# thangvubk/SoftGroup

Hardware: AMD Instinct MI355X
Metric: scans/sec ScanNet-v2-like inference (softgroup_scannet.yaml, full forward_test) (higher is better)
Workload: dtype f32

## Files before the change

### include/softgroup_hip.h

```cpp
#ifndef SOFTGROUP_HIP_H
#define SOFTGROUP_HIP_H

#include <stddef.h>
#include <stdint.h>

#ifdef __cplusplus
extern "C" {
#endif

typedef void *sg_stream_t;

#define SG_OK 0
#define SG_ERR_ARG (-1)
#define SG_ERR_WORKSPACE (-2)
#define SG_ERR_LAUNCH (-3)
#define SG_ERR_UNSUPPORTED (-4)

#define SG_BALLQUERY_MAX_NEIGHBORS 1000
#define SG_OCTREE_NUM_NODES 585
#define SG_OCTREE_NUM_LEAVES 512
#define SG_LISTS_SORTED 1
#define SG_LISTS_RADIUS 2

int sg_version(void);
const char *sg_last_error(void);
int sg_device_info(char *name_host, int name_cap, int *num_cu_host, int *clock_khz_host);

int sg_stream_release(sg_stream_t stream);
int sg_stream_create(sg_stream_t *stream_out);
int sg_stream_destroy(sg_stream_t stream);
int sg_stream_create_priority(sg_stream_t *stream_out, int level);

int sg_voxelize_idx_host(const int64_t *coords_host, int n, int ncol, int mode,
                         int32_t *input_map_host, int32_t *num_voxels_host,
                         int32_t *max_active_host);
int sg_voxelize_idx_fill_host(const int64_t *coords_host, int n, int ncol, int mode,
                              const int32_t *input_map_host, int num_voxels, int max_active,
                              int64_t *out_coords_host, int32_t *out_map_host);
size_t sg_voxelize_idx_workspace_bytes(int n);
int sg_voxelize_idx_build(const int64_t *coords, int n, int ncol, int mode, int32_t *input_map,
                          int32_t *meta, void *ws, size_t ws_bytes, sg_stream_t stream);
int sg_voxelize_idx_fill(const int64_t *coords, int n, int ncol, int mode,
                         const int32_t *input_map, int num_voxels, int max_active,
                         int64_t *out_coords, int32_t *out_map, void *ws, size_t ws_bytes,
                         sg_stream_t stream);

int sg_voxelize_fp(const float *feats, const int32_t *rules, int num_voxels, int max_active,
                   int channels, int average, float *out, sg_stream_t stream);
int sg_voxelize_bp(const float *d_out, const int32_t *rules, int num_voxels, int max_active,
                   int channels, int average, float *d_feats, sg_stream_t stream);

size_t sg_ballquery_workspace_bytes(int n);
int sg_ballquery_build_grid(const float *xyz, const int32_t *batch_idxs, int n, float radius,
                            void *ws, size_t ws_bytes, sg_stream_t stream);
int sg_ballquery_count(const float *xyz, const int32_t *batch_idxs, int n, float radius,
                       int32_t *start_len, int32_t *meta, void *ws, size_t ws_bytes,
                       sg_stream_t stream);
int sg_ballquery_fill(const float *xyz, const int32_t *batch_idxs, int n, float radius,
                      const int32_t *start_len, int32_t *idx, void *ws, size_t ws_bytes,
                      sg_stream_t stream);
size_t sg_scan_workspace_bytes(int n);
int sg_exclusive_scan_startlen(int32_t *start_len, int n, int32_t *meta, void *ws,
                               size_t ws_bytes, sg_stream_t stream);

int sg_octree_build_host(const float *points_host, const float *xyzwhl_host, int num_points,
                         int num_levels, float *boxes_host, int32_t *pt_inds_host,
                         int32_t *pt_start_len_host);
size_t sg_octree_build_workspace_bytes(int n);
int sg_octree_build(const float *points, int n, float *boxes, int32_t *pt_inds, int32_t *pt_start_len,
                    void *ws, size_t ws_bytes, sg_stream_t stream);
size_t sg_pyramid_inverse_map_workspace_bytes(int n_points, int n_voxels, int n_prop);
int sg_pyramid_inverse_map(const int32_t *proposals_idx, int64_t num_pairs, int n_prop,
                           const int32_t *l2p_map, int n_points, int n_voxels, int32_t *out_idx,
                           int32_t *out_offsets, int32_t *n_out_dev, void *ws, size_t ws_bytes,
                           sg_stream_t stream);
int sg_octree_ballquery_count(const float *points, const float *boxes, const int32_t *pt_inds,
                              const int32_t *pt_start_len, int n, float radius,
                              int32_t *start_len, sg_stream_t stream);
int sg_octree_ballquery_fill(const float *points, const float *boxes, const int32_t *pt_inds,
                             const int32_t *pt_start_len, int n, float radius,
                             const int32_t *start_len, int32_t *idx, sg_stream_t stream);

size_t sg_bfs_workspace_bytes(int n, int64_t n_edges);
int sg_bfs_cluster_label(const int32_t *bq_idxs, const int32_t *start_len, int n,
                         int64_t n_edges, int list_flags, const int32_t *seg_of_point,
                         const float *seg_thr, int n_seg, int32_t *n_cluster_host,
                         int32_t *sum_npoint_host, void *ws, size_t ws_bytes, sg_stream_t stream);
int sg_bfs_cluster_emit(const int32_t *bq_idxs, const int32_t *start_len, int n, int64_t n_edges,
                        const int32_t *seg_of_point, const float *seg_thr, int n_cluster,
                        int sum_npoint, int32_t *cluster_idxs, int32_t *cluster_offsets, void *ws,
                        size_t ws_bytes, sg_stream_t stream);

int sg_sec_mean(const float *inp, const int32_t *offsets, int n_seg, int channels, float *out,
                sg_stream_t stream);
int sg_sec_min(const float *inp, const int32_t *offsets, int n_seg, int channels, float *out,
               sg_stream_t stream);
int sg_sec_max(const float *inp, const int32_t *offsets, int n_seg, int channels, float *out,
               sg_stream_t stream);
int sg_global_avg_pool_fp(const float *feats, const int32_t *offsets, int n_seg, int channels,
                          float *out, sg_stream_t stream);
int sg_global_avg_pool_bp(float *d_feats, const int32_t *offsets, const float *d_out, int n_seg,
                          int channels, sg_stream_t stream);

int sg_get_mask_iou_on_cluster(const int32_t *proposals_idx, const int32_t *proposals_offset,
                               const int64_t *instance_labels, const int32_t *instance_pointnum,
                               int n_instance, int n_proposal, float *proposals_iou,
                               sg_stream_t stream);
int sg_get_mask_iou_on_pred(const int32_t *proposals_idx, const int32_t *proposals_offset,
                            const int64_t *instance_labels, const int32_t *instance_pointnum,
                            const float *mask_scores_sigmoid, int n_instance, int n_proposal,
                            float *proposals_iou, sg_stream_t stream);
int sg_get_mask_label(const int32_t *proposals_idx, const int32_t *proposals_offset,
                      const int64_t *instance_labels, const int64_t *instance_cls,
                      const float *proposals_iou, int n_instance, int n_proposal, float iou_thr,
                      float *mask_label, sg_stream_t stream);

size_t sg_spconv_hash_workspace_bytes(int num_rows);
int sg_spconv_subm_rulebook(const int32_t *indices, int num_rows, const int32_t *spatial_shape_host,
                            int32_t *nbr, void *ws, size_t ws_bytes, sg_stream_t stream);
int sg_spconv_down_build(const int32_t *indices, int num_rows, const int32_t *spatial_shape_host,
                         int32_t *in2out, int32_t *meta, void *ws, size_t ws_bytes,
                         sg_stream_t stream);
int sg_spconv_down_fill(const int32_t *indices, int num_rows, const int32_t *in2out,
                        int num_out_rows, int32_t *out_indices, int32_t *child, void *ws,
                        size_t ws_bytes, sg_stream_t stream);
int sg_spconv_inverse_rulebook(const int32_t *indices_fine, const int32_t *in2out, int num_rows,
                               int32_t *inv_nbr, sg_stream_t stream);

#define SG_PLAN_HIST_WORDS 40
size_t sg_spconv_plan_workspace_bytes(int num_out_rows);
int sg_spconv_plan(const int32_t *nbr, int num_out_rows, int kvol, int32_t *order,
                   uint32_t *tile_mask, int32_t *nbr_tiles, void *ws, size_t ws_bytes,
                   sg_stream_t stream);

#define SG_PYRAMID_MAX_LEVELS 10
typedef struct sg_plan_ptrs {
  int32_t *order;
  uint32_t *tile_mask;
  int32_t *nbr_tiles;
} sg_plan_ptrs;
typedef struct sg_pyramid_level {
  int rows;
  int32_t *indices;
  int32_t *nbr;
  sg_plan_ptrs subm;
  int32_t *in2out;
  int32_t *child;
  sg_plan_ptrs down;
  int32_t *inv;
  sg_plan_ptrs up;
} sg_pyramid_level;
size_t sg_spconv_pyramid_workspace_bytes(int num_rows, int n_levels);
int sg_spconv_pyramid_rows(const int32_t *indices, int num_rows, const int32_t *spatial_shape_host,
                           int n_levels, int32_t *rows_dev, void *ws, size_t ws_bytes,
                           sg_stream_t stream);
size_t sg_spconv_pyramid_build_workspace_bytes(const sg_pyramid_level *levels_host, int n_levels);
int sg_spconv_pyramid_build(const int32_t *indices, int num_rows, const int32_t *spatial_shape_host,
                            int n_levels, const sg_pyramid_level *levels_host, void *ws,
                            size_t ws_bytes, void *ws2, size_t ws2_bytes, sg_stream_t stream);

size_t sg_spconv_packed_weight_elems(int kvol, int cin, int cout);
int sg_spconv_pack_weight(const float *w, int cout, int kvol, int cin, int src_is_kio, float *w_k8,
                          sg_stream_t stream);

size_t sg_spconv_conv_workspace_bytes(int num_out_rows, int cout);
int sg_spconv_gather_conv_f32(const float *in, int num_in_rows, const int32_t *nbr,
                              int num_out_rows, int kvol, int cin, int cout, const float *w_k8,
                              const float *post_scale, const float *post_shift,
                              const float *residual, const float *act_scale,
                              const float *act_shift, float *out_act, const int32_t *order,
                              const uint32_t *tile_mask, const int32_t *nbr_tiles, float *out,
                              void *ws, size_t ws_bytes, sg_stream_t stream);

int sg_spconv_set_arithmetic(int mode);

int sg_spconv_set_combine(int mode);

int sg_spconv_set_chain(int mode);
int sg_spconv_chain_stats(int64_t *launches, int64_t *steps);

int sg_spconv_profile(int enable);
int sg_spconv_profile_read(double *total_ms, int *launches);
int sg_spconv_profile_detail(float *ms, int32_t *dims, int cap, int *calls);

typedef struct sg_mlp2 {
  const float *w1, *b1, *bn_scale, *bn_shift, *w2, *b2;
  int out;
} sg_mlp2;
int sg_pointwise_heads(const float *voxel_feats, const void *v2p_map, int v2p_is_int64, int n_points,
                       int channels, const sg_mlp2 *semantic, const sg_mlp2 *offset, float *output_feats,
                       float *semantic_scores, float *pt_offsets, int64_t *semantic_preds,
                       sg_stream_t stream);

size_t sg_spconv_packed_weight_elems_bf16(int kvol, int cin, int cout);
int sg_spconv_pack_weight_bf16(const float *w, int cout, int kvol, int cin, int src_is_kio,
                               uint16_t *w_k8_bf16, sg_stream_t stream);
size_t sg_spconv_conv_bf16_workspace_bytes(int num_out_rows, int cout);
int sg_spconv_gather_conv_bf16(const uint16_t *in, int num_in_rows, const int32_t *nbr, int num_out_rows,
                               int kvol, int cin, int cout, const uint16_t *w_k8_bf16,
                               const int32_t *order, const uint32_t *tile_mask, const int32_t *nbr_tiles,
                               uint16_t *out, void *ws, size_t ws_bytes, sg_stream_t stream);

int sg_spconv_transpose_table(const int32_t *nbr, int num_out_rows, int kvol, int32_t *nbr_t,
                              sg_stream_t stream);
size_t sg_spconv_wgrad_workspace_bytes(int num_out_rows, int kvol, int cin, int cout);
int sg_spconv_wgrad(const void *in, int in_is_bf16, const void *g_out, int g_is_bf16, const int32_t *nbr_t,
                    int num_out_rows, int kvol, int cin, int cout, float *dw_kio, void *ws,
                    size_t ws_bytes, sg_stream_t stream);

typedef struct sg_unet_block {
  int cin, cout;
  const float *bn1_scale, *bn1_shift;
  const float *w1;
  const float *bn2_scale, *bn2_shift;
  const float *w2;
  const float *w_i;
} sg_unet_block;
typedef struct sg_unet_level {
  int planes, n_blocks;
  const sg_unet_block *blocks;
  const sg_unet_block *tail;
  const float *down_bn_scale, *down_bn_shift, *down_w;
  const float *up_bn_scale, *up_bn_shift, *up_w;
} sg_unet_level;
typedef struct sg_unet_desc {
  int n_levels;
  const sg_unet_level *levels;
  int input_cin;
  const float *input_w;
  const float *out_bn_scale, *out_bn_shift;
  int input_cin_packed;
  int arithmetic;
} sg_unet_desc;
size_t sg_unet_arena_bytes(const sg_unet_desc *desc, int num_rows);
int sg_unet_forward(const sg_unet_desc *desc, const float *feats, const int32_t *indices,
                    int num_rows, const int32_t *spatial_shape_host, float *out, void *arena,
                    size_t arena_bytes, sg_stream_t stream);

typedef struct sg_train_bn {
  const float *weight, *bias;
  float *running_mean, *running_var;
  float momentum, eps;
  float *g_weight, *g_bias;
} sg_train_bn;
typedef struct sg_train_conv {
  const float *w;
  float *g_w;
} sg_train_conv;
typedef struct sg_unet_train_block {
  int cin, cout;
  sg_train_bn bn1, bn2;
  sg_train_conv c1, c2, ci;
} sg_unet_train_block;
typedef struct sg_unet_train_level {
  int planes, n_blocks;
  const sg_unet_train_block *blocks, *tail;
  sg_train_bn down_bn, up_bn;
  sg_train_conv down, up;
} sg_unet_train_level;
typedef struct sg_unet_train_desc {
  int n_levels;
  const sg_unet_train_level *levels;
  int input_cin;
  sg_train_conv input;
  sg_train_bn out_bn;
  int arithmetic;
} sg_unet_train_desc;
size_t sg_unet_train_arena_hint(const sg_unet_train_desc *desc, int num_rows);
int sg_unet_train_forward(const sg_unet_train_desc *desc, const float *feats, const int32_t *indices,
                          int num_rows, const int32_t *spatial_shape_host, float *out, void *arena,
                          size_t arena_bytes, size_t *arena_needed, void **tape, sg_stream_t stream);
int sg_unet_train_backward(void *tape, const float *g_out, float *g_feats, sg_stream_t stream);
void sg_unet_train_release(void *tape);

int sg_bn_relu_f32(const float *x, const float *scale, const float *shift, int64_t num_rows,
                   int channels, int relu, float *out, sg_stream_t stream);

int sg_gather_rows_f32(const float *in, const int32_t *index, int64_t num_out_rows, int channels,
                       float *out, sg_stream_t stream);
int sg_gather_rows_i64idx_f32(const float *in, const int64_t *index, int64_t num_out_rows,
                              int channels, float *out, sg_stream_t stream);

int sg_instance_npoint(const int32_t *proposals_idx, const float *mask_scores, int64_t num_pairs,
                       int stride, int n_classes, float mask_thr, int n_prop, int32_t *npoint,
                       sg_stream_t stream);
size_t sg_instance_runs_workspace_bytes(int n_kept, int n_points);
int sg_instance_runs(const int32_t *proposals_idx, const float *mask_scores, int64_t num_pairs,
                     int stride, int n_classes, float mask_thr, const int32_t *inst_of, int n_prop,
                     int n_kept, int n_points, int32_t *starts, int32_t *ends, int64_t *bounds,
                     int64_t runs_capacity, void *ws, size_t ws_bytes, sg_stream_t stream);

int64_t sg_rle_format_bound(int64_t total_runs, int digits);
int sg_rle_format_host(const int64_t *starts_host, const int64_t *lens_host,
                       const int64_t *bounds_host, int n_groups, char *out_host,
                       int64_t out_capacity, int64_t *out_offsets_host);
size_t sg_rle_format_device_workspace_bytes(int64_t run_capacity);
int64_t sg_rle_format_device_text_bytes(int64_t run_capacity, int64_t length);
int sg_rle_format_device(const int32_t *starts, const int32_t *ends, const int64_t *bounds, int n_inst,
                         int64_t run_capacity, int64_t length, uint8_t *text, int64_t text_capacity,
                         int64_t *text_off, void *ws, size_t ws_bytes, sg_stream_t stream);
int sg_rle_format_runs_host(const int32_t *starts_host, const int32_t *ends_host,
                            const int64_t *bounds_host, int n_groups, char *out_host,
                            int64_t out_capacity, int64_t *out_offsets_host);

size_t sg_panoptic_fusion_workspace_bytes(int n_inst, int n_points);
int sg_panoptic_fusion(const uint32_t *bits, int n_inst, int n_points, const int32_t *order,
                       const int32_t *label_id, const int64_t *semantic_preds, int cls_offset,
                       double skip_iou, int semantic_classes, int thing_class_min, uint32_t *out,
                       void *ws, size_t ws_bytes, sg_stream_t stream);

#define SG_NMS_IOU 0
#define SG_NMS_MIN 1
size_t sg_mask_nms_workspace_bytes(int n_inst, int64_t n_points);
int sg_mask_nms(const uint32_t *bits, int n_inst, int64_t n_points, const float *scores, const int32_t *labels,
                double thr, int measure, int class_agnostic, uint8_t *keep, int32_t *n_keep, int32_t *inter_out,
                void *ws, size_t ws_bytes, sg_stream_t stream);
int sg_mask_bits_from_runs(const int32_t *starts, const int32_t *ends, const int64_t *bounds, int64_t n_runs,
                           int n_inst, int64_t n_points, uint32_t *bits, sg_stream_t stream);

typedef struct sg_grouping_cfg {
  int n_points;
  int n_sem_classes;
  int n_seg;
  const int32_t *seg_class;
  const float *seg_thr;
  float score_thr;
  int min_npoint;
  float radius;
  int batch_size;
  float voxel_scale;
  int voxel_shape;
  int feat_channels;
} sg_grouping_cfg;
typedef struct sg_grouping_result {
  int n_selected, n_neighbours, n_proposals, sum_npoint, n_voxels, max_active;
  size_t proposals_idx;
  size_t proposals_offset;
  size_t voxel_coords;
  size_t voxel_offsets;
  size_t voxel_feats;
  size_t point_to_voxel;
  size_t arena_used, arena_needed;
  int deferred_classes;
  int reserved_;
} sg_grouping_result;
int sg_scan_grouping(const sg_grouping_cfg *cfg, const float *scores, const float *pt_offsets,
                     const float *coords_float, const int32_t *batch_idxs, const float *point_feats,
                     void *arena, size_t arena_bytes, sg_grouping_result *result_host,
                     sg_stream_t stream);

typedef struct sg_grouping_pp_cfg {
  sg_grouping_cfg base;
  int with_pyramid, with_octree, lvl_fusion;
  double radius;
  double base_size;
} sg_grouping_pp_cfg;
int sg_scan_grouping_pp(const sg_grouping_pp_cfg *cfg, const float *scores, const float *pt_offsets,
                        const float *coords_float, const int32_t *batch_idxs, const float *point_feats,
                        void *arena, size_t arena_bytes, sg_grouping_result *result_host,
                        sg_stream_t stream);

int sg_host_copy_2d(void *dst, int64_t dst_pitch_bytes, const void *src, int64_t src_pitch_bytes, int64_t rows,
                    int64_t row_bytes);
int sg_host_cast_f64_f32(float *dst, const double *src, int64_t n);
int sg_host_fill_i64_strided(int64_t *dst, int64_t pitch_elems, int64_t rows, int64_t value);
int sg_host_colmax_i64(const int64_t *src, int64_t rows, int64_t cols, int64_t *out_max);

typedef struct sg_instances_cfg {
  int n_proposals, n_classes;
  int score_stride;
  int64_t sum_npoint;
  int n_points;
  float cls_score_thr, mask_score_thr;
  int min_npoint;
} sg_instances_cfg;
typedef struct sg_instances_result {
  int n_kept;
  size_t off_class, off_score, off_text, text_bytes;
  size_t host_needed, arena_used, arena_needed;
  size_t bits;
  size_t label_id;
} sg_instances_result;
int sg_scan_instances(const sg_instances_cfg *cfg, const int32_t *proposals_idx, const float *mask_scores,
                      const float *cls_prob, const float *iou_scores, void *arena, size_t arena_bytes,
                      void *host_out, size_t host_bytes, sg_instances_result *result_host,
                      sg_stream_t stream);

typedef struct sg_linear {
  const float *w, *b;
  int out, in;
} sg_linear;
int sg_softmax_rows(const float *x, int64_t rows, int cols, float *out, sg_stream_t stream);
int sg_mlp_rows(const float *feats, const int32_t *idx, int64_t rows, int channels, const sg_mlp2 *mlp,
                float *out, sg_stream_t stream);
int sg_linear_rows(const float *x, int64_t rows, const sg_linear *lin, float *out, sg_stream_t stream);

#define SG_SCAN_DENSE_MAX 16
typedef struct sg_scan_dense_item {
  int kind;
  const void *ptr;
  size_t bytes;
} sg_scan_dense_item;
typedef struct sg_scan_desc {
  const sg_unet_desc *backbone;
  const sg_unet_desc *tiny;
  sg_mlp2 semantic, offset, mask;
  sg_linear cls, iou;
  int channels;
  int with_coords;
  int semantic_classes, instance_classes;
  sg_grouping_cfg grouping;
  float cls_score_thr, mask_score_thr;
  int min_npoint;
  int want_instances;
  int with_pyramid, with_octree;
  double pp_radius, pp_base_size;
} sg_scan_desc;
typedef struct sg_scan_input {
  int n_points, n_voxels, max_active;
  int batch_size;
  int spatial_shape[3];
  const float *feats;
  int feat_dim;
  const float *coords_float;
  const int32_t *p2v_map;
  const void *v2p_map;
  int v2p_is_int64;
  const void *voxel_coords;
  int voxel_coords_is_int64;
  const int32_t *batch_idxs;
  const int64_t *semantic_labels, *instance_labels;
  int n_dense;
  sg_scan_dense_item dense[SG_SCAN_DENSE_MAX];
} sg_scan_input;
typedef struct sg_scan_result {
  sg_grouping_result grouping;
  sg_instances_result instances;
  size_t grouping_base, instances_base;
  size_t dense_offset[SG_SCAN_DENSE_MAX];
  size_t dense_bytes;
  size_t voxel_feats_in, backbone_out, output_feats, semantic_scores, semantic_prob, pt_offsets,
      semantic_preds, tiny_out, mask_scores, cls_scores, cls_prob, iou_scores;
  size_t arena_used, arena_needed, host_dense_needed, host_inst_needed;
  int stage;
} sg_scan_result;
size_t sg_scan_arena_bytes(const sg_scan_desc *desc, int n_points, int n_voxels);
int sg_scan_forward(const sg_scan_desc *desc, const sg_scan_input *in, void *arena, size_t arena_bytes,
                    void *host_dense, size_t host_dense_bytes, void *host_inst, size_t host_inst_bytes,
                    sg_scan_result *result_host, sg_stream_t stream);

int sg_eval_intersections(const int32_t *run_start, const int64_t *run_off, const int32_t *run_pred,
                          int n_runs, int64_t total_points, const int32_t *gt_slot, int n_pred,
                          int n_slots, int32_t *counts, sg_stream_t stream);

#define SG_EVAL_I32 0
#define SG_EVAL_I64 1
#define SG_EVAL_U32 2
#define SG_EVAL_MAX_CLASSES 1024
#define SG_EVAL_BAD_GT 1
#define SG_EVAL_BAD_PRED 2
#define SG_EVAL_BAD_INST 4

size_t sg_eval_tally_workspace_bytes(int64_t n_points);
int sg_eval_class_tally(const void *pred, int pred_kind, const void *gt, int gt_kind, int64_t n_points,
                        int64_t ignore_label, int panoptic, int n_classes, uint64_t *tallies,
                        const void *inst, int inst_kind, const float *offset_pred, const float *offset_gt,
                        double *offset_sum, uint64_t *offset_count, int32_t *flags, void *ws, size_t ws_bytes,
                        sg_stream_t stream);

size_t sg_eval_panoptic_workspace_bytes(int64_t n_points);
int sg_eval_panoptic_segments(const void *pred, int pred_kind, const void *sem, int sem_kind,
                              const void *inst, int inst_kind, const int64_t *scan_off, int n_scans,
                              int64_t n_points, int64_t ignore_label, int n_classes, int64_t min_points,
                              uint64_t *fp_fn, int64_t *tp_rows, uint64_t *tp_count, int32_t *flags,
                              void *ws, size_t ws_bytes, sg_stream_t stream);

#define SG_INST_BAD_TEXT 1
#define SG_INST_ODD_TOKENS 2
#define SG_INST_RUN_RANGE 4
#define SG_INST_BAD_GT 8
#define SG_INST_OVERFLOW_GT 16
#define SG_INST_OVERFLOW_EX 32
#define SG_INST_NO_EXAMPLES 64
#define SG_INST_MAX_THRESHOLDS 16
#define SG_INST_SECTIONS 16

int64_t sg_inst_rle_run_slots(int64_t text_bytes, int n_masks);
int sg_inst_rle_parse(const uint8_t *text, const int64_t *text_off, const int32_t *mask_pred, int n_masks,
                      int64_t text_bytes, int64_t length, int32_t *run_start, int32_t *run_len, int32_t *run_pred,
                      int64_t run_slots, int32_t *vert_count, int32_t *flags, sg_stream_t stream);

size_t sg_inst_scan_workspace_bytes(int64_t n_points, int n_pred, int64_t run_slots, int n_classes, int gt_cap,
                                    int n_thr, int n_labels, int64_t *section_off);
int sg_inst_scan_update(const int64_t *gts, int64_t n_points, const int32_t *run_start, const int32_t *run_len,
                        const int32_t *run_pred, int64_t run_slots, const int32_t *pred_label,
                        const int32_t *pred_vert, const double *pred_conf, int n_pred, int n_labels, int n_classes,
                        int64_t min_region, const double *thresholds, int n_thr, int gt_cap, uint64_t *ex_key,
                        uint32_t *ex_meta, int64_t ex_cap, int32_t *seg_stats, int64_t *totals, int32_t *flags,
                        void *ws, size_t ws_bytes, sg_stream_t stream);

size_t sg_inst_curves_workspace_bytes(int64_t n_examples, int n_seg);
int sg_inst_curves(const uint64_t *ex_key, const uint32_t *ex_meta, int64_t n_examples, const int32_t *seg_stats,
                   int n_seg, double *ap, double *rc, int32_t *flags, void *ws, size_t ws_bytes,
                   sg_stream_t stream);

#define SG_DET_BAD_COORD 1
#define SG_DET_MAX_THRESHOLDS 16

int sg_det_boxes_runs(const void *coords, int coords_f64, const int64_t *run_start, const int64_t *run_off,
                      const int32_t *run_owner, int64_t n_runs, int64_t total_points, int64_t n_owner,
                      double *boxes, int32_t *flags, sg_stream_t stream);

int sg_det_boxes_labels(const void *coords, int coords_f64, const int64_t *labels, const int64_t *scan_off,
                        const int64_t *owner_off, int n_scans, int64_t n_points, int64_t n_owner, double *boxes,
                        int64_t *count, int64_t *first, int32_t *flags, sg_stream_t stream);

size_t sg_det_match_workspace_bytes(int64_t n_gt, int n_thresholds);
int sg_det_match(const double *det_box, const int32_t *det_group, const int32_t *det_rank, int64_t n_det,
                 const double *gt_box, const int64_t *group_off, int64_t n_gt, const double *thresholds,
                 int n_thresholds, double *ovmax, int64_t *jmax, uint8_t *tp, void *ws, size_t ws_bytes,
                 sg_stream_t stream);

int sg_train_augment(const float *xyz, int64_t n, int has_scale, float scale_factor, const double *m_host,
                     double work_scale, double down, double *xyz_middle, double *work, uint64_t *stats,
                     sg_stream_t stream);
int sg_train_blur(float *grids, float *tmp, int b0, int b1, int b2, int n_grids, sg_stream_t stream);
int sg_train_elastic(double *work, int64_t n, const float *grids, int b0, int b1, int b2, double gran, double mag,
                     uint64_t *stats, sg_stream_t stream);
int sg_train_crop_count(const double *work, int64_t n, double down, const double *min_host,
                        const double *cand_host, int k, uint64_t *counts, sg_stream_t stream);
size_t sg_train_compact_workspace_bytes(int64_t n);
int sg_train_compact(const double *work, const double *xyz_middle, const float *feat, int c, const float *noise,
                     const int64_t *sem, const int64_t *inst, int64_t n, double down, const double *min_host,
                     const double *crop_host, int64_t out_cap, int64_t *coord, double *xyz_middle_out,
                     float *feat_out, int64_t *sem_out, int64_t *inst_out, int32_t *kept, void *ws,
                     size_t ws_bytes, sg_stream_t stream);
int sg_train_gather(const int64_t *idx, int64_t m, const float *xyz, const float *feat, int c, const int64_t *sem,
                    const int64_t *inst, float *xyz_out, float *feat_out, int64_t *sem_out, int64_t *inst_out,
                    sg_stream_t stream);
size_t sg_train_id_set_workspace_bytes(void);
int sg_train_id_set(const int64_t *labels, int64_t n, int64_t ignore, int64_t *out, int cap, void *ws,
                    size_t ws_bytes, sg_stream_t stream);
int sg_train_remap(int64_t *labels, int64_t n, const int64_t *sorted_ids, const int64_t *mapped, int k,
                   sg_stream_t stream);
size_t sg_train_instance_workspace_bytes(int64_t n, int k);
int sg_train_instance_info(const double *xyz_middle, const int64_t *inst, const int64_t *sem, int64_t n, int k,
                           int64_t cls_shift, int32_t *pointnum, int64_t *cls, double *pt_offset, void *ws,
                           size_t ws_bytes, sg_stream_t stream);

int sg_test_x4_minima(const float *xyz, int64_t n, const double *m_host, double scale, uint64_t *stats,
                      sg_stream_t stream);
int sg_test_x4_split(const float *xyz, const float *feat, int c, const int64_t *sem, const int64_t *inst, int64_t n,
                     const double *m_host, double scale, const double *min_host, int64_t *coord,
                     double *xyz_middle, float *feat_out, int64_t *sem_out, int64_t *inst_out, sg_stream_t stream);
int sg_kitti_decode_labels(const int32_t *words, int64_t n, const int32_t *lut, int64_t *sem, int64_t *inst,
                           uint64_t *missing, sg_stream_t stream);

int sg_mask_text_runs(const int32_t *starts, const int32_t *ends, const int64_t *bounds, int64_t n_runs, int n_inst,
                      int64_t length, int first, int count, uint8_t *text, int64_t text_capacity, sg_stream_t stream);
int sg_mask_text_bits(const uint32_t *bits, int n_inst, int64_t length, int first, int count, uint8_t *text,
                      int64_t text_capacity, sg_stream_t stream);
size_t sg_decimal_lines_workspace_bytes(int64_t n);
int sg_decimal_lines(const int64_t *values, int64_t n, const int32_t *nyu_table, int nyu_len, uint8_t *text,
                     int64_t text_capacity, int64_t *meta, void *ws, size_t ws_bytes, sg_stream_t stream);
int sg_panoptic_kitti_words(const uint32_t *words, int64_t n, const int32_t *lut, int lut_len, uint32_t *out,
                            uint64_t *missing, uint64_t *missing_host, sg_stream_t stream);
size_t sg_parse_decimal_lines_workspace_bytes(int64_t nbytes);
int sg_parse_decimal_lines(const uint8_t *text, int64_t nbytes, int64_t *values, int64_t capacity, int64_t *meta,
                           void *ws, size_t ws_bytes, sg_stream_t stream);
int sg_parse_mask_text(const uint8_t *text, int64_t nbytes, uint8_t *flags, uint32_t *bits, int64_t *meta,
                       sg_stream_t stream);

int sg_viz_paint_bits(const uint32_t *bits, int n_inst, int64_t n, const int32_t *priority, const uint8_t *skip,
                      int32_t *label, int32_t *pointnum, sg_stream_t stream);
size_t sg_viz_paint_runs_workspace_bytes(int n_inst, int64_t n);
int sg_viz_paint_runs(const int32_t *starts, const int32_t *ends, const int64_t *bounds, int64_t n_runs, int n_inst,
                      int64_t n, const int32_t *priority, const uint8_t *skip, int32_t *label, int32_t *pointnum,
                      void *ws, size_t ws_bytes, sg_stream_t stream);
int sg_viz_gt_labels(const int64_t *ids, int64_t n, int32_t *label, int32_t *pointnum, sg_stream_t stream);
size_t sg_viz_instance_rank_workspace_bytes(int n_inst);
int sg_viz_instance_rank(const int32_t *pointnum, int n_inst, int32_t *rank, void *ws, size_t ws_bytes,
                         sg_stream_t stream);
#define SG_VIZ_INPUT 0
#define SG_VIZ_CLASS 1
#define SG_VIZ_CLASS_WRAP 2
#define SG_VIZ_INSTANCE 3
int sg_viz_colors(int mode, const float *colors, const int64_t *cls, const int32_t *inst, const int32_t *rank,
                  int n_rank, const uint8_t *table, int k, int64_t n, uint8_t *rgb, int64_t *meta,
                  sg_stream_t stream);
size_t sg_viz_ply_vertices_workspace_bytes(int64_t n);
int sg_viz_ply_vertices(const float *xyz, const float *offset, const uint8_t *rgb, const uint8_t *keep, int64_t n,
                        uint8_t *text, int64_t text_capacity, int64_t *meta, void *ws, size_t ws_bytes,
                        sg_stream_t stream);

size_t sg_loss_reduce_workspace_bytes(void);
int sg_pointwise_loss_fwd(const float *semantic_scores, const int64_t *semantic_labels, const float *weight,
                          int64_t ignore_label, const float *pt_offsets, const float *pt_offset_labels,
                          const int64_t *instance_labels, int64_t n, int c, float *out, void *ws, size_t ws_bytes,
                          sg_stream_t stream);
int sg_pointwise_loss_bwd(const float *semantic_scores, const int64_t *semantic_labels, const float *weight,
                          int64_t ignore_label, const float *pt_offsets, const float *pt_offset_labels,
                          const int64_t *instance_labels, int64_t n, int c, const float *sums,
                          const float *g_semantic, const float *g_offset, float *d_scores, float *d_offsets,
                          sg_stream_t stream);
size_t sg_assign_proposals_workspace_bytes(int n_proposal);
int sg_assign_proposals(const float *ious_on_cluster, const int64_t *instance_cls, int64_t ignore_label,
                        float pos_iou_thr, int match_low_quality, float min_pos_thr, int64_t background_label,
                        int n_proposal, int n_gt, int64_t *labels, void *ws, size_t ws_bytes, sg_stream_t stream);
int sg_proposal_loss_fwd(const float *cls_scores, const float *iou_scores, const int64_t *labels,
                         const float *ious_on_pred, const int64_t *instance_cls, int64_t ignore_label,
                         int n_proposal, int n_gt, int k1, float *gt_iou, float *out, void *ws, size_t ws_bytes,
                         sg_stream_t stream);
int sg_proposal_loss_bwd(const float *cls_scores, const float *iou_scores, const int64_t *labels,
                         const float *gt_iou, const float *sums, const float *g_cls, const float *g_iou,
                         int n_proposal, int k1, float *d_cls_scores, float *d_iou_scores, sg_stream_t stream);
int sg_mask_loss_fwd(const float *mask_scores, const int32_t *instance_batch_idxs, const int64_t *labels,
                     const float *mask_label, int64_t m, int n_proposal, int k1, float *mask_sig, float *out,
                     void *ws, size_t ws_bytes, sg_stream_t stream);
int sg_mask_loss_bwd(const float *mask_scores, const int32_t *instance_batch_idxs, const int64_t *labels,
                     const float *mask_label, const float *sums, const float *g_mask, int64_t m, int n_proposal,
                     int k1, float *d_mask_scores, sg_stream_t stream);

#define SG_OPTIM_ROW_PARAM 0
#define SG_OPTIM_ROW_GRAD 1
#define SG_OPTIM_ROW_STATE0 2
#define SG_OPTIM_ROW_STATE1 3
#define SG_OPTIM_ROW_STEP 4
#define SG_OPTIM_ROW_COUNT 5
#define SG_OPTIM_TABLE_ROWS 6
int sg_optim_chunk_elems(void);
int64_t sg_optim_plan(const int64_t *counts, int n_tensors, int64_t *chunks, int64_t chunk_capacity);
size_t sg_optim_workspace_bytes(void);
int sg_optim_grad_norm(const int64_t *table, int n_tensors, const int64_t *chunks, int64_t n_chunks,
                       const float *grad_scale, float max_norm, float *out, void *ws, size_t ws_bytes,
                       sg_stream_t stream);
int sg_optim_adam_step(const int64_t *table, int n_tensors, const int64_t *chunks, int64_t n_chunks, double lr,
                       double beta1, double beta2, double eps, double weight_decay, int adamw,
                       const float *grad_scale, const float *found_inf, const float *clip_coef, int zero_grad,
                       int32_t *arrive, sg_stream_t stream);
int sg_optim_sgd_step(const int64_t *table, int n_tensors, const int64_t *chunks, int64_t n_chunks, double lr,
                      double momentum, double dampening, double weight_decay, int nesterov, const float *grad_scale,
                      const float *found_inf, const float *clip_coef, int zero_grad, int32_t *arrive,
                      sg_stream_t stream);
int sg_optim_scale_grads(const int64_t *table, int n_tensors, const int64_t *chunks, int64_t n_chunks,
                         const float *coef, sg_stream_t stream);

#ifdef __cplusplus
}
#endif
#endif
```

### softgroup_amd/_lib.py

```python
import ctypes as C
import os

_HERE = os.path.dirname(os.path.abspath(__file__))
LIB_PATH = os.path.join(_HERE, 'lib', os.environ.get('SG_LIB_NAME', 'libsoftgroup_hip.so'))

_lib = None

_vp, _i, _f, _i64, _sz, _d = C.c_void_p, C.c_int, C.c_float, C.c_int64, C.c_size_t, C.c_double
_pi32 = C.POINTER(C.c_int32)

SIGNATURES = {
    'sg_version': (_i, []),
    'sg_last_error': (C.c_char_p, []),
    'sg_device_info': (_i, [C.c_char_p, _i, C.POINTER(_i), C.POINTER(_i)]),
    'sg_stream_release': (_i, [_vp]),
    'sg_host_copy_2d': (_i, [_vp, _i64, _vp, _i64, _i64, _i64]),
    'sg_host_cast_f64_f32': (_i, [_vp, _vp, _i64]),
    'sg_host_fill_i64_strided': (_i, [_vp, _i64, _i64, _i64]),
    'sg_host_colmax_i64': (_i, [_vp, _i64, _i64, _vp]),
    'sg_stream_create': (_i, [_vp]),
    'sg_stream_create_priority': (_i, [_vp, _i]),
    'sg_stream_destroy': (_i, [_vp]),
    'sg_voxelize_idx_host': (_i, [_vp, _i, _i, _i, _vp, _pi32, _pi32]),
    'sg_voxelize_idx_fill_host': (_i, [_vp, _i, _i, _i, _vp, _i, _i, _vp, _vp]),
    'sg_voxelize_idx_workspace_bytes': (_sz, [_i]),
    'sg_voxelize_idx_build': (_i, [_vp, _i, _i, _i, _vp, _vp, _vp, _sz, _vp]),
    'sg_voxelize_idx_fill': (_i, [_vp, _i, _i, _i, _vp, _i, _i, _vp, _vp, _vp, _sz, _vp]),
    'sg_voxelize_fp': (_i, [_vp, _vp, _i, _i, _i, _i, _vp, _vp]),
    'sg_voxelize_bp': (_i, [_vp, _vp, _i, _i, _i, _i, _vp, _vp]),
    'sg_ballquery_workspace_bytes': (_sz, [_i]),
    'sg_ballquery_build_grid': (_i, [_vp, _vp, _i, _f, _vp, _sz, _vp]),
    'sg_ballquery_count': (_i, [_vp, _vp, _i, _f, _vp, _vp, _vp, _sz, _vp]),
    'sg_ballquery_fill': (_i, [_vp, _vp, _i, _f, _vp, _vp, _vp, _sz, _vp]),
    'sg_scan_workspace_bytes': (_sz, [_i]),
    'sg_exclusive_scan_startlen': (_i, [_vp, _i, _vp, _vp, _sz, _vp]),
    'sg_octree_build_host': (_i, [_vp, _vp, _i, _i, _vp, _vp, _vp]),
    'sg_octree_build_workspace_bytes': (_sz, [_i]),
    'sg_octree_build': (_i, [_vp, _i, _vp, _vp, _vp, _vp, _sz, _vp]),
    'sg_pyramid_inverse_map_workspace_bytes': (_sz, [_i, _i, _i]),
    'sg_pyramid_inverse_map': (_i, [_vp, _i64, _i, _vp, _i, _i, _vp, _vp, _vp, _vp, _sz, _vp]),
    'sg_octree_ballquery_count': (_i, [_vp, _vp, _vp, _vp, _i, _f, _vp, _vp]),
    'sg_octree_ballquery_fill': (_i, [_vp, _vp, _vp, _vp, _i, _f, _vp, _vp, _vp]),
    'sg_bfs_workspace_bytes': (_sz, [_i, _i64]),
    'sg_bfs_cluster_label': (_i, [_vp, _vp, _i, _i64, _i, _vp, _vp, _i, _pi32, _pi32, _vp, _sz, _vp]),
    'sg_bfs_cluster_emit': (_i, [_vp, _vp, _i, _i64, _vp, _vp, _i, _i, _vp, _vp, _vp, _sz, _vp]),
    'sg_sec_mean': (_i, [_vp, _vp, _i, _i, _vp, _vp]),
    'sg_sec_min': (_i, [_vp, _vp, _i, _i, _vp, _vp]),
    'sg_sec_max': (_i, [_vp, _vp, _i, _i, _vp, _vp]),
    'sg_global_avg_pool_fp': (_i, [_vp, _vp, _i, _i, _vp, _vp]),
    'sg_global_avg_pool_bp': (_i, [_vp, _vp, _vp, _i, _i, _vp]),
    'sg_get_mask_iou_on_cluster': (_i, [_vp, _vp, _vp, _vp, _i, _i, _vp, _vp]),
    'sg_get_mask_iou_on_pred': (_i, [_vp, _vp, _vp, _vp, _vp, _i, _i, _vp, _vp]),
    'sg_get_mask_label': (_i, [_vp, _vp, _vp, _vp, _vp, _i, _i, _f, _vp, _vp]),
    'sg_spconv_hash_workspace_bytes': (_sz, [_i]),
    'sg_spconv_subm_rulebook': (_i, [_vp, _i, _pi32, _vp, _vp, _sz, _vp]),
    'sg_spconv_pyramid_workspace_bytes': (_sz, [_i, _i]),
    'sg_spconv_pyramid_rows': (_i, [_vp, _i, _pi32, _i, _vp, _vp, _sz, _vp]),
    'sg_spconv_pyramid_build_workspace_bytes': (_sz, [_vp, _i]),
    'sg_spconv_pyramid_build': (_i, [_vp, _i, _pi32, _i, _vp, _vp, _sz, _vp, _sz, _vp]),
    'sg_spconv_down_build': (_i, [_vp, _i, _pi32, _vp, _vp, _vp, _sz, _vp]),
    'sg_spconv_down_fill': (_i, [_vp, _i, _vp, _i, _vp, _vp, _vp, _sz, _vp]),
    'sg_spconv_inverse_rulebook': (_i, [_vp, _vp, _i, _vp, _vp]),
    'sg_spconv_plan_workspace_bytes': (_sz, [_i]),
    'sg_spconv_plan': (_i, [_vp, _i, _i, _vp, _vp, _vp, _vp, _sz, _vp]),
    'sg_spconv_set_arithmetic': (_i, [_i]),
    'sg_spconv_set_combine': (_i, [_i]),
    'sg_spconv_set_chain': (_i, [_i]),
    'sg_spconv_chain_stats': (_i, [_vp, _vp]),
    'sg_spconv_profile': (_i, [_i]),
    'sg_spconv_profile_read': (_i, [_vp, _vp]),
    'sg_spconv_profile_detail': (_i, [_vp, _vp, _i, _vp]),
    'sg_unet_arena_bytes': (_sz, [_vp, _i]),
    'sg_unet_forward': (_i, [_vp, _vp, _vp, _i, _vp, _vp, _vp, _sz, _vp]),
    'sg_unet_train_arena_hint': (_sz, [_vp, _i]),
    'sg_unet_train_forward': (_i, [_vp, _vp, _vp, _i, _vp, _vp, _vp, _sz, _vp, _vp, _vp]),
    'sg_unet_train_backward': (_i, [_vp, _vp, _vp, _vp]),
    'sg_unet_train_release': (None, [_vp]),
    'sg_pointwise_heads': (_i, [_vp, _vp, _i, _i, _i, _vp, _vp, _vp, _vp, _vp, _vp, _vp]),
    'sg_spconv_packed_weight_elems': (_sz, [_i, _i, _i]),
    'sg_spconv_pack_weight': (_i, [_vp, _i, _i, _i, _i, _vp, _vp]),
    'sg_spconv_conv_workspace_bytes': (_sz, [_i, _i]),
    'sg_spconv_gather_conv_f32': (_i, [_vp, _i, _vp, _i, _i, _i, _i, _vp, _vp, _vp, _vp, _vp, _vp,
                                       _vp, _vp, _vp, _vp, _vp, _vp, _sz, _vp]),
    'sg_spconv_packed_weight_elems_bf16': (_sz, [_i, _i, _i]),
    'sg_spconv_pack_weight_bf16': (_i, [_vp, _i, _i, _i, _i, _vp, _vp]),
    'sg_spconv_conv_bf16_workspace_bytes': (_sz, [_i, _i]),
    'sg_spconv_gather_conv_bf16': (_i, [_vp, _i, _vp, _i, _i, _i, _i, _vp, _vp, _vp, _vp, _vp, _vp, _sz,
                                        _vp]),
    'sg_spconv_transpose_table': (_i, [_vp, _i, _i, _vp, _vp]),
    'sg_spconv_wgrad_workspace_bytes': (_sz, [_i, _i, _i, _i]),
    'sg_spconv_wgrad': (_i, [_vp, _i, _vp, _i, _vp, _i, _i, _i, _i, _vp, _vp, _sz, _vp]),
    'sg_instance_npoint': (_i, [_vp, _vp, _i64, _i, _i, _f, _i, _vp, _vp]),
    'sg_instance_runs_workspace_bytes': (_sz, [_i, _i]),
    'sg_instance_runs': (_i, [_vp, _vp, _i64, _i, _i, _f, _vp, _i, _i, _i, _vp, _vp, _vp, _i64, _vp, _sz, _vp]),
    'sg_rle_format_bound': (_i64, [_i64, _i]),
    'sg_rle_format_host': (_i, [_vp, _vp, _vp, _i, _vp, _i64, _vp]),
    'sg_rle_format_device_workspace_bytes': (_sz, [_i64]),
    'sg_rle_format_device_text_bytes': (_i64, [_i64, _i64]),
    'sg_rle_format_device': (_i, [_vp, _vp, _vp, _i, _i64, _i64, _vp, _i64, _vp, _vp, _sz, _vp]),
    'sg_rle_format_runs_host': (_i, [_vp, _vp, _vp, _i, _vp, _i64, _vp]),
    'sg_panoptic_fusion_workspace_bytes': (_sz, [_i, _i]),
    'sg_panoptic_fusion': (_i, [_vp, _i, _i, _vp, _vp, _vp, _i, C.c_double, _i, _i, _vp, _vp, _sz, _vp]),
    'sg_mask_nms_workspace_bytes': (_sz, [_i, _i64]),
    'sg_mask_nms': (_i, [_vp, _i, _i64, _vp, _vp, _d, _i, _i, _vp, _vp, _vp, _vp, _sz, _vp]),
    'sg_mask_bits_from_runs': (_i, [_vp, _vp, _vp, _i64, _i, _i64, _vp, _vp]),
    'sg_scan_grouping': (_i, [_vp, _vp, _vp, _vp, _vp, _vp, _vp, _sz, _vp, _vp]),
    'sg_scan_grouping_pp': (_i, [_vp, _vp, _vp, _vp, _vp, _vp, _vp, _sz, _vp, _vp]),
    'sg_scan_instances': (_i, [_vp, _vp, _vp, _vp, _vp, _vp, _sz, _vp, _sz, _vp, _vp]),
    'sg_softmax_rows': (_i, [_vp, _i64, _i, _vp, _vp]),
    'sg_mlp_rows': (_i, [_vp, _vp, _i64, _i, _vp, _vp, _vp]),
    'sg_linear_rows': (_i, [_vp, _i64, _vp, _vp, _vp]),
    'sg_scan_arena_bytes': (_sz, [_vp, _i, _i]),
    'sg_scan_forward': (_i, [_vp, _vp, _vp, _sz, _vp, _sz, _vp, _sz, _vp, _vp]),
    'sg_eval_intersections': (_i, [_vp, _vp, _vp, _i, _i64, _vp, _i, _i, _vp, _vp]),
    'sg_eval_tally_workspace_bytes': (_sz, [_i64]),
    'sg_eval_class_tally': (_i, [_vp, _i, _vp, _i, _i64, _i64, _i, _i, _vp, _vp, _i, _vp, _vp, _vp, _vp, _vp,
                                 _vp, _sz, _vp]),
    'sg_eval_panoptic_workspace_bytes': (_sz, [_i64]),
    'sg_eval_panoptic_segments': (_i, [_vp, _i, _vp, _i, _vp, _i, _vp, _i, _i64, _i64, _i, _i64, _vp, _vp, _vp,
                                       _vp, _vp, _sz, _vp]),
    'sg_inst_rle_run_slots': (_i64, [_i64, _i]),
    'sg_inst_rle_parse': (_i, [_vp, _vp, _vp, _i, _i64, _i64, _vp, _vp, _vp, _i64, _vp, _vp, _vp]),
    'sg_inst_scan_workspace_bytes': (_sz, [_i64, _i, _i64, _i, _i, _i, _i, _vp]),
    'sg_inst_scan_update': (_i, [_vp, _i64, _vp, _vp, _vp, _i64, _vp, _vp, _vp, _i, _i, _i, _i64, _vp, _i, _i,
                                 _vp, _vp, _i64, _vp, _vp, _vp, _vp, _sz, _vp]),
    'sg_inst_curves_workspace_bytes': (_sz, [_i64, _i]),
    'sg_inst_curves': (_i, [_vp, _vp, _i64, _vp, _i, _vp, _vp, _vp, _vp, _sz, _vp]),
    'sg_det_boxes_runs': (_i, [_vp, _i, _vp, _vp, _vp, _i64, _i64, _i64, _vp, _vp, _vp]),
    'sg_det_boxes_labels': (_i, [_vp, _i, _vp, _vp, _vp, _i, _i64, _i64, _vp, _vp, _vp, _vp, _vp]),
    'sg_det_match_workspace_bytes': (_sz, [_i64, _i]),
    'sg_det_match': (_i, [_vp, _vp, _vp, _i64, _vp, _vp, _i64, _vp, _i, _vp, _vp, _vp, _vp, _sz, _vp]),
    'sg_bn_relu_f32': (_i, [_vp, _vp, _vp, _i64, _i, _i, _vp, _vp]),
    'sg_gather_rows_f32': (_i, [_vp, _vp, _i64, _i, _vp, _vp]),
    'sg_gather_rows_i64idx_f32': (_i, [_vp, _vp, _i64, _i, _vp, _vp]),
    'sg_train_augment': (_i, [_vp, _i64, _i, _f, _vp, C.c_double, C.c_double, _vp, _vp, _vp, _vp]),
    'sg_train_blur': (_i, [_vp, _vp, _i, _i, _i, _i, _vp]),
    'sg_train_elastic': (_i, [_vp, _i64, _vp, _i, _i, _i, C.c_double, C.c_double, _vp, _vp]),
    'sg_train_crop_count': (_i, [_vp, _i64, C.c_double, _vp, _vp, _i, _vp, _vp]),
    'sg_train_compact_workspace_bytes': (_sz, [_i64]),
    'sg_train_compact': (_i, [_vp, _vp, _vp, _i, _vp, _vp, _vp, _i64, C.c_double, _vp, _vp, _i64, _vp, _vp, _vp, _vp,
                              _vp, _vp, _vp, _sz, _vp]),
    'sg_train_gather': (_i, [_vp, _i64, _vp, _vp, _i, _vp, _vp, _vp, _vp, _vp, _vp, _vp]),
    'sg_train_id_set_workspace_bytes': (_sz, []),
    'sg_train_id_set': (_i, [_vp, _i64, _i64, _vp, _i, _vp, _sz, _vp]),
    'sg_train_remap': (_i, [_vp, _i64, _vp, _vp, _i, _vp]),
    'sg_train_instance_workspace_bytes': (_sz, [_i64, _i]),
    'sg_train_instance_info': (_i, [_vp, _vp, _vp, _i64, _i, _i64, _vp, _vp, _vp, _vp, _sz, _vp]),
    'sg_test_x4_minima': (_i, [_vp, _i64, _vp, C.c_double, _vp, _vp]),
    'sg_test_x4_split': (_i, [_vp, _vp, _i, _vp, _vp, _i64, _vp, C.c_double, _vp, _vp, _vp, _vp, _vp, _vp, _vp]),
    'sg_kitti_decode_labels': (_i, [_vp, _i64, _vp, _vp, _vp, _vp, _vp]),
    'sg_mask_text_runs': (_i, [_vp, _vp, _vp, _i64, _i, _i64, _i, _i, _vp, _i64, _vp]),
    'sg_mask_text_bits': (_i, [_vp, _i, _i64, _i, _i, _vp, _i64, _vp]),
    'sg_decimal_lines_workspace_bytes': (_sz, [_i64]),
    'sg_decimal_lines': (_i, [_vp, _i64, _vp, _i, _vp, _i64, _vp, _vp, _sz, _vp]),
    'sg_panoptic_kitti_words': (_i, [_vp, _i64, _vp, _i, _vp, _vp, _vp, _vp]),
    'sg_parse_decimal_lines_workspace_bytes': (_sz, [_i64]),
    'sg_parse_decimal_lines': (_i, [_vp, _i64, _vp, _i64, _vp, _vp, _sz, _vp]),
    'sg_parse_mask_text': (_i, [_vp, _i64, _vp, _vp, _vp, _vp]),
    'sg_viz_paint_bits': (_i, [_vp, _i, _i64, _vp, _vp, _vp, _vp, _vp]),
    'sg_viz_paint_runs_workspace_bytes': (_sz, [_i, _i64]),
    'sg_viz_paint_runs': (_i, [_vp, _vp, _vp, _i64, _i, _i64, _vp, _vp, _vp, _vp, _vp, _sz, _vp]),
    'sg_viz_gt_labels': (_i, [_vp, _i64, _vp, _vp, _vp]),
    'sg_viz_instance_rank_workspace_bytes': (_sz, [_i]),
    'sg_viz_instance_rank': (_i, [_vp, _i, _vp, _vp, _sz, _vp]),
    'sg_viz_colors': (_i, [_i, _vp, _vp, _vp, _vp, _i, _vp, _i, _i64, _vp, _vp, _vp]),
    'sg_viz_ply_vertices_workspace_bytes': (_sz, [_i64]),
    'sg_viz_ply_vertices': (_i, [_vp, _vp, _vp, _vp, _i64, _vp, _i64, _vp, _vp, _sz, _vp]),
    'sg_loss_reduce_workspace_bytes': (_sz, []),
    'sg_pointwise_loss_fwd': (_i, [_vp, _vp, _vp, _i64, _vp, _vp, _vp, _i64, _i, _vp, _vp, _sz, _vp]),
    'sg_pointwise_loss_bwd': (_i, [_vp, _vp, _vp, _i64, _vp, _vp, _vp, _i64, _i, _vp, _vp, _vp, _vp, _vp, _vp]),
    'sg_assign_proposals_workspace_bytes': (_sz, [_i]),
    'sg_assign_proposals': (_i, [_vp, _vp, _i64, _f, _i, _f, _i64, _i, _i, _vp, _vp, _sz, _vp]),
    'sg_proposal_loss_fwd': (_i, [_vp, _vp, _vp, _vp, _vp, _i64, _i, _i, _i, _vp, _vp, _vp, _sz, _vp]),
    'sg_proposal_loss_bwd': (_i, [_vp, _vp, _vp, _vp, _vp, _vp, _vp, _i, _i, _vp, _vp, _vp]),
    'sg_mask_loss_fwd': (_i, [_vp, _vp, _vp, _vp, _i64, _i, _i, _vp, _vp, _vp, _sz, _vp]),
    'sg_mask_loss_bwd': (_i, [_vp, _vp, _vp, _vp, _vp, _vp, _i64, _i, _i, _vp, _vp]),
    'sg_optim_chunk_elems': (_i, []),
    'sg_optim_plan': (_i64, [_vp, _i, _vp, _i64]),
    'sg_optim_workspace_bytes': (_sz, []),
    'sg_optim_grad_norm': (_i, [_vp, _i, _vp, _i64, _vp, _f, _vp, _vp, _sz, _vp]),
    'sg_optim_adam_step': (_i, [_vp, _i, _vp, _i64, _d, _d, _d, _d, _d, _i, _vp, _vp, _vp, _i, _vp, _vp]),
    'sg_optim_sgd_step': (_i, [_vp, _i, _vp, _i64, _d, _d, _d, _d, _i, _vp, _vp, _vp, _i, _vp, _vp]),
    'sg_optim_scale_grads': (_i, [_vp, _i, _vp, _i64, _vp, _vp]),
}


class SoftGroupHipError(RuntimeError):
    pass


def lib():
    global _lib
    if _lib is None:
        import torch
        if not os.path.exists(LIB_PATH):
            raise SoftGroupHipError(
                f'{LIB_PATH} not found: the HIP extension is required (no CPU fallback). '
                'Build it with `python -c "import __graft_entry__ as g; g.build()"`.')
        L = C.CDLL(LIB_PATH)
        for name, (res, args) in SIGNATURES.items():
            fn = getattr(L, name)
            fn.restype = res
            fn.argtypes = args
        _lib = L
    return _lib


def check(rc, what=''):
    if rc != 0:
        msg = lib().sg_last_error()
        raise SoftGroupHipError(f'{what} failed ({rc}): {msg.decode() if msg else ""}')


def ptr(t):
    return None if t is None else t.data_ptr()


_raw_stream = None


def stream():
    global _raw_stream
    import torch
    if _raw_stream is None:
        _raw_stream = getattr(torch._C, '_cuda_getCurrentRawStream', None) or (
            lambda dev: torch.cuda.current_stream(dev).cuda_stream)
    return _raw_stream(torch.cuda.current_device())


def workspace(nbytes, device):
    import torch
    return torch.empty(max(int(nbytes), 256), dtype=torch.uint8, device=device)
```

### softgroup_amd/csrc/ballquery.hip

```cpp
#include "common.h"
#include "scan.h"

namespace sg {

constexpr int32_t kBqEmpty = 0x7f7f7f7f;
constexpr int kBqBuf = 2048;
constexpr int kBqCap = SG_BALLQUERY_MAX_NEIGHBORS;
constexpr int kBqKeep = 64;

struct BqWs {
  int4 *cell;
  int32_t *table;
  int32_t *count;
  int32_t *start;
  int32_t *cursor;
  int32_t *slot_of;
  float4 *sorted;
  int32_t *keep;
  void *scan_ws;
  size_t scan_bytes;
  uint32_t cap;
};

__device__ __forceinline__ uint32_t cell_slot(int b, int cx, int cy, int cz, uint32_t mask) {
  uint64_t h = (static_cast<uint64_t>(static_cast<uint32_t>(b)) << 32) | static_cast<uint32_t>(cx);
  h = mix64(h) ^ ((static_cast<uint64_t>(static_cast<uint32_t>(cy)) << 32) | static_cast<uint32_t>(cz));
  return static_cast<uint32_t>(mix64(h)) & mask;
}

__global__ void __launch_bounds__(256) bq_insert_kernel(const float *__restrict__ xyz,
                                                       const int32_t *__restrict__ batch_idxs,
                                                       int n, double inv_cell, int4 *__restrict__ cell,
                                                       int32_t *table, uint32_t mask, int32_t *count,
                                                       int32_t *__restrict__ slot_of) {
  const int i = blockIdx.x * 256 + threadIdx.x;
  if (i >= n) return;
  int4 c;
  c.x = batch_idxs ? batch_idxs[i] : 0;
  c.y = static_cast<int>(floor(static_cast<double>(xyz[3 * i + 0]) * inv_cell));
  c.z = static_cast<int>(floor(static_cast<double>(xyz[3 * i + 1]) * inv_cell));
  c.w = static_cast<int>(floor(static_cast<double>(xyz[3 * i + 2]) * inv_cell));
  cell[i] = c;
  uint32_t s = cell_slot(c.x, c.y, c.z, c.w, mask);
  while (true) {
    int32_t cur = __hip_atomic_load(&table[s], __ATOMIC_RELAXED, __HIP_MEMORY_SCOPE_AGENT);
    if (cur == kBqEmpty) {
      cur = atomicCAS(&table[s], kBqEmpty, i);
      if (cur == kBqEmpty) break;
    }
    int4 o;
    o.x = batch_idxs ? batch_idxs[cur] : 0;
    o.y = static_cast<int>(floor(static_cast<double>(xyz[3 * cur + 0]) * inv_cell));
    o.z = static_cast<int>(floor(static_cast<double>(xyz[3 * cur + 1]) * inv_cell));
    o.w = static_cast<int>(floor(static_cast<double>(xyz[3 * cur + 2]) * inv_cell));
    if (o.x == c.x && o.y == c.y && o.z == c.z && o.w == c.w) break;
    s = (s + 1) & mask;
  }
  slot_of[i] = static_cast<int32_t>(s);
  atomicAdd(&count[s], 1);
}

__global__ void __launch_bounds__(256) bq_scatter_kernel(const float *__restrict__ xyz, int n,
                                                        const int32_t *__restrict__ slot_of,
                                                        const int32_t *__restrict__ start,
                                                        int32_t *cursor, float4 *__restrict__ sorted) {
  const int i = blockIdx.x * 256 + threadIdx.x;
  if (i >= n) return;
  const int s = slot_of[i];
  const int pos = start[s] + atomicAdd(&cursor[s], 1);
  sorted[pos] = make_float4(xyz[3 * i], xyz[3 * i + 1], xyz[3 * i + 2], __int_as_float(i));
}

__device__ __forceinline__ float dist2(float ox, float oy, float oz, float x, float y, float z) {
  const float dx = __fsub_rn(ox, x), dy = __fsub_rn(oy, y), dz = __fsub_rn(oz, z);
  return __fmaf_rn(dz, dz, __fmaf_rn(dx, dx, __fmul_rn(dy, dy)));
}

struct BqCells {
  int start, excl, incl, total;
};
__device__ __forceinline__ BqCells bq_cells(int my_start, int my_count) {
  BqCells c;
  c.start = my_start;
  c.incl = wave_incl_scan(my_count);
  c.excl = c.incl - my_count;
  c.total = __shfl(c.incl, 63, 64);
  return c;
}
__device__ __forceinline__ int bq_candidate(const BqCells &c, int t) {
  int lo = 0, hi = 26;
#pragma unroll
  for (int it = 0; it < 5; ++it) {
    const int mid = (lo + hi) >> 1;
    const bool right = __shfl(c.incl, mid, 64) <= t;
    lo = right ? mid + 1 : lo;
    hi = right ? hi : mid;
  }
  return __shfl(c.start, lo, 64) + (t - __shfl(c.excl, lo, 64));
}

__device__ __forceinline__ int bq_scan_count(const float4 *__restrict__ sorted, const BqCells &c,
                                             float ox, float oy, float oz, float r2, int limit) {
  int total = 0;
  for (int t0 = 0; t0 < c.total; t0 += 64) {
    const int t = t0 + lane_id();
    const int at = bq_candidate(c, min(t, c.total - 1));
    if (t < c.total) {
      const float4 p = sorted[at];
      total += (dist2(ox, oy, oz, p.x, p.y, p.z) < r2 && __float_as_int(p.w) < limit) ? 1 : 0;
    }
  }
  return wave_sum(total);
}

template <bool FILL>
__global__ void __launch_bounds__(256) bq_query_kernel(const float *__restrict__ xyz, int n,
                                                      float r2, const int4 *__restrict__ cell,
                                                      const int32_t *__restrict__ table,
                                                      const int32_t *__restrict__ count,
                                                      const int32_t *__restrict__ start,
                                                      uint32_t mask, const float4 *__restrict__ sorted,
                                                      int32_t *__restrict__ start_len,
                                                      int32_t *__restrict__ idx_out, int32_t *__restrict__ keep) {
  __shared__ __attribute__((aligned(16))) int32_t buf_all[FILL ? 4 * kBqBuf : 4 * kBqKeep];
  const int wave = threadIdx.x >> 6, lane = threadIdx.x & 63;
  int32_t *buf = buf_all + wave * (FILL ? kBqBuf : kBqKeep);
  for (int i = blockIdx.x * 4 + wave; i < n; i += gridDim.x * 4) {
    if (FILL) {
      const int out_len = start_len[2 * i + 1];
      if (out_len <= kBqKeep) {
        if (lane < out_len) idx_out[static_cast<int64_t>(start_len[2 * i]) + lane] = keep[static_cast<int64_t>(i) * kBqKeep + lane];
        continue;
      }
    }
    const float ox = xyz[3 * i], oy = xyz[3 * i + 1], oz = xyz[3 * i + 2];
    const int4 c = cell[i];
    int my_start = 0, my_count = 0;
    if (lane < 27) {
      const int cx = c.y + lane / 9 - 1, cy = c.z + (lane / 3) % 3 - 1, cz = c.w + lane % 3 - 1;
      uint32_t s = cell_slot(c.x, cx, cy, cz, mask);
      while (true) {
        const int32_t rep = table[s];
        if (rep == kBqEmpty) break;
        const int4 o = cell[rep];
        if (o.x == c.x && o.y == cx && o.z == cy && o.w == cz) {
          my_start = start[s];
          my_count = count[s];
          break;
        }
        s = (s + 1) & mask;
      }
    }
    const BqCells cells = bq_cells(my_start, my_count);
    if (!FILL) {
      int m = 0;
      for (int t0 = 0; t0 < cells.total; t0 += 64) {
        const int t = t0 + lane;
        const int at = bq_candidate(cells, min(t, cells.total - 1));
        bool ok = false;
        int id = 0;
        if (t < cells.total) {
          const float4 p = sorted[at];
          id = __float_as_int(p.w);
          ok = dist2(ox, oy, oz, p.x, p.y, p.z) < r2;
        }
        const uint64_t bal = __ballot(ok);
        const int pos = m + mask_prefix(bal);
        if (ok && pos < kBqKeep) buf[pos] = id;
        m += __popcll(bal);
      }
      if (lane == 0) start_len[2 * i + 1] = min(m, kBqCap);
      if (m <= kBqKeep) {
        __builtin_amdgcn_fence(__ATOMIC_RELEASE, "wavefront");
        __builtin_amdgcn_wave_barrier();
        const int e = lane < m ? buf[lane] : 0x7fffffff;
        int rank = 0;
        for (int j = 0; j < m; ++j) rank += (buf[j] < e);
        if (lane < m) keep[static_cast<int64_t>(i) * kBqKeep + rank] = e;
      }
      __builtin_amdgcn_wave_barrier();
      continue;
    }
    const int out_start = start_len[2 * i], out_len = start_len[2 * i + 1];
    int limit = 0x7fffffff;
    int m = 0;
    for (int attempt = 0; attempt < 2; ++attempt) {
      m = 0;
      for (int t0 = 0; t0 < cells.total; t0 += 64) {
        const int t = t0 + lane;
        const int at = bq_candidate(cells, min(t, cells.total - 1));
        bool ok = false;
        int id = 0;
        if (t < cells.total) {
          const float4 p = sorted[at];
          id = __float_as_int(p.w);
          ok = dist2(ox, oy, oz, p.x, p.y, p.z) < r2 && id < limit;
        }
        const uint64_t bal = __ballot(ok);
        const int pos = m + mask_prefix(bal);
        if (ok && pos < kBqBuf) buf[pos] = id;
        m += __popcll(bal);
      }
      if (m <= kBqBuf) break;
      int lo = 0, hi = n;
      while (lo < hi) {
        const int mid = lo + (hi - lo) / 2;
        const int cmid = bq_scan_count(sorted, cells, ox, oy, oz, r2, mid);
        if (cmid >= out_len) hi = mid; else lo = mid + 1;
      }
      limit = lo;
    }
    __builtin_amdgcn_fence(__ATOMIC_RELEASE, "wavefront");
    __builtin_amdgcn_wave_barrier();
    for (int e0 = 0; e0 < m; e0 += 64) {
      const int ei = e0 + lane;
      const int e = ei < m ? buf[ei] : 0x7fffffff;
      int rank = 0;
      int j = 0;
      for (; j + 4 <= m; j += 4) {
        const int4 q = *reinterpret_cast<const int4 *>(buf + j);
        rank += (q.x < e) + (q.y < e) + (q.z < e) + (q.w < e);
      }
      for (; j < m; ++j) rank += (buf[j] < e);
      if (ei < m && rank < out_len) idx_out[static_cast<int64_t>(out_start) + rank] = e;
    }
    __builtin_amdgcn_wave_barrier();
  }
}

static size_t bq_cap(int n) {
  size_t cap = 1024;
  while (cap < static_cast<size_t>(n) * 2) cap <<= 1;
  return cap;
}

static bool bq_carve(void *ws, size_t ws_bytes, int n, BqWs *w) {
  Workspace a(ws, ws_bytes);
  const size_t nn = static_cast<size_t>(n > 0 ? n : 1);
  w->cap = static_cast<uint32_t>(bq_cap(n));
  w->cell = a.take<int4>(nn);
  w->sorted = a.take<float4>(nn);
  w->table = a.take<int32_t>(w->cap);
  w->count = a.take<int32_t>(w->cap);
  w->start = a.take<int32_t>(w->cap);
  w->cursor = a.take<int32_t>(w->cap);
  w->slot_of = a.take<int32_t>(nn);
  w->scan_bytes = scan_workspace_bytes(w->cap);
  w->scan_ws = a.take<char>(w->scan_bytes);
  w->keep = a.take<int32_t>(nn * kBqKeep);
  return w->scan_ws != nullptr && w->keep != nullptr;
}

}

using namespace sg;

extern "C" {

size_t sg_ballquery_workspace_bytes(int n) {
  const size_t nn = static_cast<size_t>(n > 0 ? n : 1);
  const size_t cap = bq_cap(n);
  return 2 * align_up(nn * 16) + 4 * align_up(cap * 4) + align_up(nn * 4) +
         align_up(scan_workspace_bytes(cap)) + align_up(nn * kBqKeep * 4) + 256;
}

int sg_ballquery_build_grid(const float *xyz, const int32_t *batch_idxs, int n, float radius,
                            void *ws, size_t ws_bytes, sg_stream_t stream_) {
  SG_REQUIRE(n >= 0 && radius > 0.f, "sg_ballquery_build_grid: bad arguments (n=%d r=%g)", n, radius);
  hipStream_t stream = as_stream(stream_);
  BqWs w;
  if (!bq_carve(ws, ws_bytes, n, &w)) {
    set_error("sg_ballquery_build_grid: workspace too small");
    return SG_ERR_WORKSPACE;
  }
  if (n == 0) return SG_OK;
  {
    FillList f;
    f.add(w.table, static_cast<size_t>(w.cap) * 4, 0x7f);
    f.add(w.count, static_cast<size_t>(w.cap) * 4, 0);
    f.add(w.cursor, static_cast<size_t>(w.cap) * 4, 0);
    fill_many(f, stream);
  }
  const double inv_cell = 1.0 / (static_cast<double>(radius) * (1.0 + 1e-6));
  const int grid = (n + 255) / 256;
  bq_insert_kernel<<<grid, 256, 0, stream>>>(xyz, batch_idxs, n, inv_cell, w.cell, w.table,
                                             w.cap - 1, w.count, w.slot_of);
  const int32_t *count = w.count;
  int32_t *start = w.start;
  auto in = [count] __device__(int64_t s) { return count[s]; };
  auto out = [start] __device__(int64_t s, int v) { start[s] = v; };
  int rc = exclusive_scan(in, out, w.cap, nullptr, w.scan_ws, w.scan_bytes, stream);
  if (rc != SG_OK) return rc;
  bq_scatter_kernel<<<grid, 256, 0, stream>>>(xyz, n, w.slot_of, w.start, w.cursor, w.sorted);
  return check_launch("sg_ballquery_build_grid");
}

int sg_ballquery_count(const float *xyz, const int32_t *batch_idxs, int n, float radius,
                       int32_t *start_len, int32_t *meta, void *ws, size_t ws_bytes,
                       sg_stream_t stream_) {
  (void)batch_idxs;
  (void)meta;
  SG_REQUIRE(n >= 0 && radius > 0.f, "sg_ballquery_count: bad arguments");
  BqWs w;
  if (!bq_carve(ws, ws_bytes, n, &w)) {
    set_error("sg_ballquery_count: workspace too small");
    return SG_ERR_WORKSPACE;
  }
  if (n == 0) return SG_OK;
  const float r2 = radius * radius;
  bq_query_kernel<false><<<grid_for(n, 4, 256 * 16), 256, 0, as_stream(stream_)>>>(
      xyz, n, r2, w.cell, w.table, w.count, w.start, w.cap - 1, w.sorted, start_len, nullptr, w.keep);
  return check_launch("sg_ballquery_count");
}

int sg_ballquery_fill(const float *xyz, const int32_t *batch_idxs, int n, float radius,
                      const int32_t *start_len, int32_t *idx, void *ws, size_t ws_bytes,
                      sg_stream_t stream_) {
  (void)batch_idxs;
  SG_REQUIRE(n >= 0 && radius > 0.f, "sg_ballquery_fill: bad arguments");
  BqWs w;
  if (!bq_carve(ws, ws_bytes, n, &w)) {
    set_error("sg_ballquery_fill: workspace too small");
    return SG_ERR_WORKSPACE;
  }
  if (n == 0) return SG_OK;
  const float r2 = radius * radius;
  bq_query_kernel<true><<<grid_for(n, 4, 256 * 16), 256, 0, as_stream(stream_)>>>(
      xyz, n, r2, w.cell, w.table, w.count, w.start, w.cap - 1, w.sorted,
      const_cast<int32_t *>(start_len), idx, w.keep);
  return check_launch("sg_ballquery_fill");
}

}
```

### softgroup_amd/csrc/bfs.hip

```cpp
#include <stdlib.h>

#include <map>
#include <mutex>
#include <utility>

#include "common.h"
#include "scan.h"

namespace sg {

constexpr int kCap = SG_BALLQUERY_MAX_NEIGHBORS;
constexpr int kEmitThreads = 512;
constexpr int kEmitWaves = kEmitThreads / 64;

#define SG_LD(p) __hip_atomic_load((p), __ATOMIC_RELAXED, __HIP_MEMORY_SCOPE_AGENT)
#define SG_ST(p, v) __hip_atomic_store((p), (v), __ATOMIC_RELAXED, __HIP_MEMORY_SCOPE_AGENT)

struct BfsWs {
  int32_t *parent, *lab, *size, *cid, *coff, *owner, *seeds, *ebase, *wcnt, *asym_nodes;
  int4 *label;
  int2 *erec;
  int32_t *counters;
  void *scan_ws;
  size_t scan_bytes;
  int32_t *big_stage[2];
  unsigned long long *big_rec[2];
};

constexpr int kBigFastWgs = 16;
constexpr int kBigSlice = 8192;
constexpr int kBigClusterMin = 16384;
inline bool big_fast_on() {
  const char *e = getenv("SG_BFS_BIG_FAST");
  return !(e && atoi(e) == 0);
}
inline int thin_levels_on() {
  const char *e = getenv("SG_BFS_THIN");
  return e ? atoi(e) : 0;
}
inline bool big_local_on() {
  const char *e = getenv("SG_BFS_BIG_LOCAL");
  return !(e && atoi(e) == 0);
}
inline size_t big_stage_entries(int n) {
  return n > kBigClusterMin && big_fast_on() ? static_cast<size_t>(n) + static_cast<size_t>(kBigFastWgs) * kBigSlice : 0;
}

static bool bfs_carve(void *ws, size_t ws_bytes, int n, int64_t n_edges, BfsWs *w) {
  Workspace a(ws, ws_bytes);
  const size_t nn = static_cast<size_t>(n > 0 ? n : 1);
  w->parent = a.take<int32_t>(nn);
  w->lab = a.take<int32_t>(nn);
  w->label = a.take<int4>(nn);
  w->size = a.take<int32_t>(nn);
  w->cid = a.take<int32_t>(nn);
  w->coff = a.take<int32_t>(nn);
  w->owner = a.take<int32_t>(nn);
  w->seeds = a.take<int32_t>(nn);
  w->ebase = a.take<int32_t>(nn);
  w->wcnt = a.take<int32_t>(nn);
  w->asym_nodes = a.take<int32_t>(nn);
  w->counters = a.take<int32_t>(64);
  w->scan_bytes = scan_workspace_bytes(n);
  w->scan_ws = a.take<char>(w->scan_bytes);
  w->erec = a.take<int2>(static_cast<size_t>(n_edges > 0 ? n_edges : 1));
  bool ok = w->scan_ws != nullptr && w->erec != nullptr;
  const size_t be = big_stage_entries(n);
  for (int i = 0; i < 2; ++i) {
    w->big_stage[i] = be ? a.take<int32_t>(be) : nullptr;
    w->big_rec[i] = be ? a.take<unsigned long long>(be) : nullptr;
    ok = ok && (be == 0 || (w->big_stage[i] != nullptr && w->big_rec[i] != nullptr));
  }
  return ok;
}

__device__ __forceinline__ int uf_find(int32_t *parent, int x) {
  int cur = SG_LD(&parent[x]);
  if (cur != x) {
    int prev = x, next;
    while (cur > (next = SG_LD(&parent[cur]))) {
      SG_ST(&parent[prev], next);
      prev = cur;
      cur = next;
    }
  }
  return cur;
}

__device__ __forceinline__ void uf_union(int32_t *parent, int a, int b) {
  while (a != b) {
    if (a < b) { const int t = a; a = b; b = t; }
    const int old = atomicCAS(&parent[a], a, b);
    if (old == a) return;
    a = uf_find(parent, old);
    b = uf_find(parent, b);
  }
}

__device__ __forceinline__ bool list_has_sorted(const int32_t *__restrict__ lst, int len, int key) {
  int lo = 0, hi = len;
  while (lo < hi) {
    const int mid = (lo + hi) >> 1;
    const int v = lst[mid];
    if (v < key) lo = mid + 1; else hi = mid;
  }
  return lo < len && lst[lo] == key;
}

__global__ void __launch_bounds__(256) bfs_init_kernel(int n, int32_t *parent, int32_t *size,
                                                      int32_t *owner) {
  const int i = blockIdx.x * 256 + threadIdx.x;
  if (i < n) {
    parent[i] = i;
    size[i] = 0;
    owner[i] = 0x7fffffff;
  }
}

constexpr int kSample = 2;
template <int SAMPLE>
__global__ void __launch_bounds__(256) bfs_union_kernel(const int32_t *__restrict__ idx,
                                                       const int32_t *__restrict__ start_len, int n,
                                                       int lists_sorted, int radius_lists,
                                                       int32_t *parent, int32_t *asym_nodes,
                                                       int32_t *counters) {
  const int wave = threadIdx.x >> 6, lane = threadIdx.x & 63;
  for (int u = blockIdx.x * 4 + wave; u < n; u += gridDim.x * 4) {
    const int st = start_len[2 * u], ln_all = start_len[2 * u + 1];
    const int ln = SAMPLE ? min(ln_all, kSample) : ln_all;
    const bool u_capped = ln_all >= kCap;
    bool any_asym = false;
    const int ru = SAMPLE ? -1 : SG_LD(&parent[u]);
    for (int p0 = 0; p0 < ln; p0 += 64) {
      const int p = p0 + lane;
      const int v = p < ln ? idx[st + p] : u;
      bool sym = true;
      if (v != u) {
        const int vst = start_len[2 * v], vln = start_len[2 * v + 1];
        if (!radius_lists || u_capped || vln >= kCap) {
          if (lists_sorted) {
            sym = list_has_sorted(idx + vst, vln, u);
          } else {
            sym = false;
            for (int j = 0; j < vln; ++j)
              if (idx[vst + j] == u) { sym = true; break; }
          }
        }
        if (sym) {
          if (v < u && (SAMPLE || SG_LD(&parent[v]) != ru)) uf_union(parent, uf_find(parent, u), uf_find(parent, v));
        }
      }
      any_asym |= !sym;
    }
    if (!SAMPLE && __any(any_asym)) {
      if (lane == 0) asym_nodes[atomicAdd(&counters[0], 1)] = u;
    }
  }
}

__global__ void __launch_bounds__(256) bfs_hook_min_kernel(const int32_t *__restrict__ idx,
                                                          const int32_t *__restrict__ start_len, int n,
                                                          int lists_sorted, int radius_lists, int32_t *parent) {
  const int u = blockIdx.x * 256 + threadIdx.x;
  if (u >= n) return;
  const int st = start_len[2 * u], ln = start_len[2 * u + 1];
  if (ln == 0 || !lists_sorted) return;
  const int v = idx[st];
  if (v >= u) return;
  if (!radius_lists || ln >= kCap || start_len[2 * v + 1] >= kCap)
    if (!list_has_sorted(idx + start_len[2 * v], start_len[2 * v + 1], u)) return;
  parent[u] = v;
}
__global__ void __launch_bounds__(256) bfs_compress_kernel(int n, int32_t *parent) {
  const int i = blockIdx.x * 256 + threadIdx.x;
  if (i < n) SG_ST(&parent[i], uf_find(parent, i));
}

__global__ void __launch_bounds__(256) bfs_flatten_kernel(int n, int32_t *parent, int32_t *lab) {
  const int i = blockIdx.x * 256 + threadIdx.x;
  if (i >= n) return;
  int r = i;
  while (true) {
    const int p = SG_LD(&parent[r]);
    if (p == r) break;
    r = p;
  }
  lab[i] = r;
}
__global__ void __launch_bounds__(256) bfs_store_root_kernel(int n, const int32_t *__restrict__ lab,
                                                            int32_t *__restrict__ parent) {
  const int i = blockIdx.x * 256 + threadIdx.x;
  if (i < n) parent[i] = lab[i];
}

__global__ void __launch_bounds__(256) bfs_propagate_kernel(const int32_t *__restrict__ idx,
                                                           const int32_t *__restrict__ start_len,
                                                           const int32_t *__restrict__ asym_nodes,
                                                           int n_asym,
                                                           const int32_t *__restrict__ root_of,
                                                           int32_t *lab, int32_t *counters) {
  const int wave = threadIdx.x >> 6, lane = threadIdx.x & 63;
  for (int a = blockIdx.x * 4 + wave; a < n_asym; a += gridDim.x * 4) {
    const int u = asym_nodes[a];
    const int ru = root_of[u];
    const int st = start_len[2 * u], ln = start_len[2 * u + 1];
    for (int p = lane; p < ln; p += 64) {
      const int rv = root_of[idx[st + p]];
      if (rv == ru) continue;
      const int lu = SG_LD(&lab[ru]);
      if (lu < SG_LD(&lab[rv])) {
        if (atomicMin(&lab[rv], lu) > lu) SG_ST(&counters[1], 1);
      }
    }
  }
}

__global__ void __launch_bounds__(256) bfs_label_kernel(int n, const int32_t *__restrict__ root_of,
                                                       const int32_t *__restrict__ lab,
                                                       const int32_t *__restrict__ start_len,
                                                       int4 *__restrict__ node_rec, int32_t *size) {
  const int i = blockIdx.x * 256 + threadIdx.x;
  const bool valid = i < n;
  const int l = valid ? lab[root_of[i]] : -1;
  int slot = 0;
  uint64_t todo = __ballot(valid);
  const int lane = threadIdx.x & 63;
  while (todo) {
    const int leader = __ffsll(static_cast<long long>(todo)) - 1;
    const int ll = __shfl(l, leader, 64);
    const uint64_t same = __ballot(valid && l == ll) & todo;
    int base = 0;
    if (lane == leader) base = atomicAdd(&size[ll], __popcll(same));
    base = __shfl(base, leader, 64);
    if ((same >> lane) & 1ull) slot = base + __popcll(same & ((1ull << lane) - 1ull));
    todo &= ~same;
  }
  if (!valid) return;
  node_rec[i] = make_int4(l, slot, start_len[2 * i], start_len[2 * i + 1]);
}

__global__ void __launch_bounds__(256) bfs_zero_size_kernel(int n, int32_t *size) {
  const int i = blockIdx.x * 256 + threadIdx.x;
  if (i < n) size[i] = 0;
}

__global__ void __launch_bounds__(256) bfs_owner_reset_kernel(int n, const int4 *__restrict__ label,
                                                             const int32_t *__restrict__ size,
                                                             int min_size, const int32_t *gate,
                                                             int32_t *__restrict__ owner) {
  if (SG_LD(gate) == 0) return;
  for (int i = blockIdx.x * 256 + threadIdx.x; i < n; i += gridDim.x * 256)
    if (size[label[i].x] > min_size) owner[i] = 0x7fffffff;
}

__global__ void __launch_bounds__(256) bfs_seed_kernel(int n, const int4 *__restrict__ label,
                                                      const int32_t *__restrict__ size,
                                                      const int32_t *__restrict__ cid,
                                                      const int32_t *__restrict__ coff,
                                                      const int32_t *__restrict__ seg_of_point,
                                                      const float *__restrict__ seg_thr,
                                                      int32_t *__restrict__ seeds,
                                                      int32_t *__restrict__ cluster_offsets) {
  const int i = blockIdx.x * 256 + threadIdx.x;
  if (i == 0) cluster_offsets[0] = 0;
  if (i >= n || label[i].x != i) return;
  const float thr = seg_thr[seg_of_point ? seg_of_point[i] : 0];
  if (static_cast<float>(size[i]) >= thr) {
    seeds[cid[i]] = i;
    cluster_offsets[cid[i] + 1] = coff[i] + size[i];
  }
}

__global__ void __launch_bounds__(256) bfs_edge_rec_kernel(const int32_t *__restrict__ idx,
                                                          const int4 *__restrict__ node_rec,
                                                          const int32_t *__restrict__ cid,
                                                          const int32_t *__restrict__ seeds,
                                                          int n, int n_cluster,
                                                          int2 *__restrict__ erec) {
  const int lane = threadIdx.x & 63;
  for (int v = (blockIdx.x * 256 + threadIdx.x) >> 6; v < n; v += (gridDim.x * 256) >> 6) {
    const int4 rv = node_rec[v];
    const int c = cid[rv.x];
    if (c >= n_cluster || seeds[c] != rv.x) continue;
    for (int p = lane; p < rv.w; p += 64) {
      const int4 rt = node_rec[idx[rv.z + p]];
      erec[rv.z + p] = rt.x == rv.x ? make_int2(min(rt.y, 0xfffe) | (rt.w << 16), rt.z)
                                    : make_int2(0xffff, 0);
    }
  }
}

__device__ __forceinline__ void lds_prefetch_b32(const void *gsrc, unsigned lds_dst) {
  unsigned keep;
  asm volatile("s_mov_b32 %0, m0\n\ts_mov_b32 m0, %2\n\ts_nop 0\n\tglobal_load_lds_dword %1, off\n\t"
               "s_mov_b32 m0, %0"
               : "=&s"(keep) : "v"(gsrc), "s"(lds_dst) : "memory");
}

__device__ __forceinline__ int wg_excl_scan(int v, int *lds, int *total) {
  const int w = threadIdx.x >> 6, l = threadIdx.x & 63;
  const int incl = wave_incl_scan(v);
  if (l == 63) lds[w] = incl;
  __syncthreads();
  int carry = 0, tot = 0;
#pragma unroll
  for (int i = 0; i < kEmitWaves; ++i) {
    const int x = lds[i];
    if (i < w) carry += x;
    tot += x;
  }
  __syncthreads();
  *total = tot;
  return carry + incl - v;
}

constexpr int kOwnCap = 16384;
constexpr int kFrontChunk = 1024;
constexpr int kE2 = 4096;
constexpr int kThinIter = 8;
constexpr int kThinEdges = 64 * kThinIter;
static_assert(kThinEdges <= kFrontChunk, "a thin level's winners must fit the LDS frontier");

__global__ void __launch_bounds__(kEmitThreads) bfs_emit_kernel(
    const int32_t *__restrict__ idx, const int32_t *__restrict__ start_len,
    const int4 *__restrict__ node_rec, const int2 *__restrict__ erec,
    const int32_t *__restrict__ seeds, const int32_t *__restrict__ cluster_offsets, int n_cluster,
    int32_t *owner_g, int32_t *cluster_idxs, int32_t *stats, int skip_above, int only_above,
    const int32_t *gate ,
    int thin_mode ) {
  const bool thin_on = thin_mode != 0, thin_prefetch = thin_mode == 2;
  if (gate != nullptr && SG_LD(gate) == 0) return;
  __shared__ int lds_scan[kEmitWaves];
  __shared__ int own_lds[kOwnCap];
  __shared__ int f_st[2][kFrontChunk], f_ln[2][kFrontChunk];
  __shared__ int f_eb[kFrontChunk], f_wc[kFrontChunk];
  __shared__ unsigned short ebuf[kE2];
  __shared__ int e_st[kE2], e_g[kE2];
  __shared__ unsigned short e_ln[kE2];
  __shared__ int pf_sink[kEmitThreads];
  __shared__ unsigned char thin_map[kThinEdges];
  __shared__ int thin_state[8];
  const int wave = threadIdx.x >> 6, lane = threadIdx.x & 63;
  const unsigned pf_dst = __builtin_amdgcn_readfirstlane(
      static_cast<unsigned>(reinterpret_cast<uintptr_t>(pf_sink + wave * 64)));
  static_assert(sizeof(int2) == 8, "edge records are 8 bytes: 16 per 128-byte line");
  for (int c = blockIdx.x; c < n_cluster; c += gridDim.x) {
    const int seed = seeds[c];
    const int off = cluster_offsets[c];
    const int size = cluster_offsets[c + 1] - off;
    if (size > skip_above || size <= only_above) continue;
    const bool own_in_lds = size <= kOwnCap;
    int32_t *Q = cluster_idxs + 2LL * off;
    if (own_in_lds)
      for (int i = threadIdx.x; i < size; i += kEmitThreads) own_lds[i] = 0x7fffffff;
    __syncthreads();
    if (threadIdx.x == 0) {
      const int4 rec = node_rec[seed];
      SG_ST(&Q[0], c);
      SG_ST(&Q[1], seed);
      if (own_in_lds) own_lds[rec.y] = -1; else SG_ST(&owner_g[seed], -1);
      f_st[0][0] = rec.z;
      f_ln[0][0] = rec.w;
    }
    asm volatile("s_waitcnt vmcnt(0)" ::: "memory");
    __syncthreads();
    auto rec2 = [&](int v) -> int2 { return *reinterpret_cast<const int2 *>(node_rec + v); };
    auto claim = [&](int v, int pos) {
      const int2 ll = rec2(v);
      if (ll.x != seed) return;
      if (own_in_lds) { if (own_lds[ll.y] > pos) atomicMin(&own_lds[ll.y], pos); }
      else if (SG_LD(&owner_g[v]) > pos) atomicMin(&owner_g[v], pos);
    };
    auto owner_of = [&](int v) -> int {
      const int2 ll = rec2(v);
      if (ll.x != seed) return -2;
      return own_in_lds ? own_lds[ll.y] : SG_LD(&owner_g[v]);
    };
    auto mark_done = [&](int v) {
      if (own_in_lds) own_lds[rec2(v).y] = -1; else SG_ST(&owner_g[v], -1);
    };
    int head = 0, tail = 1;
    int n_fast = 0, n_gen = 0, sum_e = 0, max_l = 0;
    int conv_lo = -1;
    auto convert_pending = [&]() {
      if (conv_lo < 0) return;
      for (int o = conv_lo + threadIdx.x; o < tail; o += kEmitThreads)
        SG_ST(&Q[2 * o + 1], idx[SG_LD(&Q[2 * o + 1])]);
      conv_lo = -1;
      asm volatile("s_waitcnt vmcnt(0)" ::: "memory");
      __syncthreads();
    };
    int cur = 0;
    bool in_lds = true;
    bool thin_ok = thin_on;
    while (head < tail) {
      const int L = tail - head;
      if (thin_ok && own_in_lds && in_lds && L <= 64) {
        if (wave == 0) {
          int h = head, t = tail, cu = cur, cl = conv_lo, levels = 0, edges = 0;
          while (true) {
            const int Lw = t - h;
            if (Lw <= 0 || Lw > 64) break;
            const int ln = lane < Lw ? f_ln[cu][lane] : 0;
            const int incl = wave_incl_scan(ln);
            const int E = __builtin_amdgcn_readlane(incl, 63);
            if (E > kThinEdges) break;
            const int eb = incl - ln;
            if (lane < Lw) f_eb[lane] = eb;
            for (int q = 0; q < Lw; ++q) {
              const int ln_q = __builtin_amdgcn_readlane(ln, q), eb_q = __builtin_amdgcn_readlane(eb, q);
              for (int p = lane; p < ln_q; p += 64) thin_map[eb_q + p] = static_cast<unsigned char>(q);
            }
            int2 r[kThinIter];
            int g[kThinIter];
#pragma unroll
            for (int j = 0; j < kThinIter; ++j) {
              const int e = j * 64 + lane;
              g[j] = 0;
              r[j] = make_int2(0xffff, 0);
              if (e < E) {
                const int q = thin_map[e];
                g[j] = f_st[cu][q] + (e - f_eb[q]);
                r[j] = erec[g[j]];
              }
            }
#pragma unroll
            for (int j = 0; j < kThinIter; ++j) {
              const int e = j * 64 + lane;
              const int slot = r[j].x & 0xffff;
              if (e < E && slot != 0xffff) {
                const int cur_owner = own_lds[slot];
                if (cur_owner > e) atomicMin(&own_lds[slot], e);
                if (thin_prefetch && cur_owner >= 0) {
                  const int tl = r[j].x >> 16;
                  const char *first = reinterpret_cast<const char *>(erec + r[j].y);
                  const char *last = reinterpret_cast<const char *>(erec + r[j].y + max(tl, 1) - 1);
                  const uintptr_t l0 = reinterpret_cast<uintptr_t>(first) & ~static_cast<uintptr_t>(127);
                  const int nlines = static_cast<int>(((reinterpret_cast<uintptr_t>(last) & ~static_cast<uintptr_t>(127)) - l0) >> 7) + 1;
                  for (int k = 0; k < 4; ++k)
                    if (k < nlines) lds_prefetch_b32(reinterpret_cast<const void *>(l0 + 128u * k), pf_dst);
                }
              }
            }
            const int nxt = cu ^ 1;
            int t_new = 0;
#pragma unroll
            for (int j = 0; j < kThinIter; ++j) {
              const int e = j * 64 + lane;
              const int slot = r[j].x & 0xffff;
              const bool win = e < E && slot != 0xffff && own_lds[slot] == e;
              const uint64_t bal = __ballot(win);
              if (win) {
                const int oo = t_new + mask_prefix(bal);
                SG_ST(&Q[2 * (t + oo)], c);
                SG_ST(&Q[2 * (t + oo) + 1], g[j]);
                f_st[nxt][oo] = r[j].y;
                f_ln[nxt][oo] = r[j].x >> 16;
                own_lds[slot] = -1;
              }
              t_new += __popcll(bal);
            }
            if (cl < 0 && t_new > 0) cl = t;
            h = t;
            t += t_new;
            cu = nxt;
            ++levels;
            edges += E;
          }
          asm volatile("s_waitcnt vmcnt(0)" ::: "memory");
          if (lane == 0) {
            thin_state[0] = h; thin_state[1] = t; thin_state[2] = cu; thin_state[3] = cl;
            thin_state[4] = levels; thin_state[5] = edges;
          }
        }
        __syncthreads();
        const int levels = thin_state[4];
        head = thin_state[0];
        tail = thin_state[1];
        cur = thin_state[2];
        conv_lo = thin_state[3];
        n_fast += levels;
        sum_e += thin_state[5];
        max_l = max(max_l, L);
        __syncthreads();
        in_lds = true;
        thin_ok = false;
        if (levels > 0) continue;
      }
      thin_ok = thin_on;
      int E = -1;
      if (in_lds && L <= kFrontChunk) {
        int carry = 0;
        for (int b0 = 0; b0 < L; b0 += kEmitThreads) {
          const int q = b0 + threadIdx.x;
          const int ln = q < L ? f_ln[cur][q] : 0;
          int tot;
          const int ex = wg_excl_scan(ln, lds_scan, &tot);
          if (q < L) f_eb[q] = carry + ex;
          carry += tot;
        }
        __syncthreads();
        E = carry;
      }
      if (E >= 0 && E <= kE2) {
        ++n_fast; sum_e += E; max_l = max(max_l, L);
        for (int e = threadIdx.x; e < E; e += kEmitThreads) {
          int lo = 0, hi = L;
          while (hi - lo > 1) {
            const int mid = (lo + hi) >> 1;
            if (f_eb[mid] <= e) lo = mid; else hi = mid;
          }
          const int g = f_st[cur][lo] + (e - f_eb[lo]);
          const int2 r = erec[g];
          const unsigned short slot = static_cast<unsigned short>(r.x & 0xffff);
          ebuf[e] = slot;
          e_g[e] = g;
          e_st[e] = r.y;
          e_ln[e] = static_cast<unsigned short>(r.x >> 16);
          if (slot != 0xffffu) {
            if (own_in_lds) {
              const int cur_owner = own_lds[slot];
              if (cur_owner > e) atomicMin(&own_lds[slot], e);
              if (cur_owner >= 0) {
                const int tl = r.x >> 16;
                const char *first = reinterpret_cast<const char *>(erec + r.y);
                const char *last = reinterpret_cast<const char *>(erec + r.y + max(tl, 1) - 1);
                const uintptr_t l0 = reinterpret_cast<uintptr_t>(first) & ~static_cast<uintptr_t>(127);
                const int nlines = static_cast<int>(((reinterpret_cast<uintptr_t>(last) & ~static_cast<uintptr_t>(127)) - l0) >> 7) + 1;
                for (int j = 0; j < 4; ++j)
                  if (j < nlines) lds_prefetch_b32(reinterpret_cast<const void *>(l0 + 128u * j), pf_dst);
              }
            } else {
              const int v = idx[g];
              if (SG_LD(&owner_g[v]) > e) atomicMin(&owner_g[v], e);
            }
          }
        }
        if (!own_in_lds) asm volatile("s_waitcnt vmcnt(0)" ::: "memory");
        __syncthreads();
        const int nxt = cur ^ 1;
        int t_new = 0;
        for (int b0 = 0; b0 < E; b0 += kEmitThreads) {
          const int e = b0 + threadIdx.x;
          unsigned short slot = 0xffffu;
          bool win = false;
          int v = 0;
          if (e < E) {
            slot = ebuf[e];
            if (slot != 0xffffu) {
              if (own_in_lds) {
                win = own_lds[slot] == e;
              } else {
                v = idx[e_g[e]];
                win = SG_LD(&owner_g[v]) == e;
              }
            }
          }
          int tot;
          const int oo = t_new + wg_excl_scan(win ? 1 : 0, lds_scan, &tot);
          if (win) {
            SG_ST(&Q[2 * (tail + oo)], c);
            SG_ST(&Q[2 * (tail + oo) + 1], e_g[e]);
            if (oo < kFrontChunk) {
              f_st[nxt][oo] = e_st[e];
              f_ln[nxt][oo] = e_ln[e];
            }
            if (own_in_lds) own_lds[slot] = -1; else SG_ST(&owner_g[v], -1);
          }
          t_new += tot;
        }
        if (conv_lo < 0 && t_new > 0) conv_lo = tail;
        if (!own_in_lds) asm volatile("s_waitcnt vmcnt(0)" ::: "memory");
        __syncthreads();
        head = tail;
        tail += t_new;
        cur = nxt;
        in_lds = t_new <= kFrontChunk;
        continue;
      }
      ++n_gen; max_l = max(max_l, L);
      convert_pending();
      auto stage = [&](int ch, int carry_in) -> int {
        const int q0 = ch * kFrontChunk, cnt = min(kFrontChunk, L - q0);
        int carry = carry_in;
        for (int b0 = 0; b0 < cnt; b0 += kEmitThreads) {
          const int q = b0 + threadIdx.x;
          int ln = 0;
          if (q < cnt) {
            const int4 rec = node_rec[SG_LD(&Q[2 * (head + q0 + q) + 1])];
            f_st[0][q] = rec.z;
            ln = rec.w;
            f_ln[0][q] = ln;
          }
          int tot;
          const int ex = wg_excl_scan(ln, lds_scan, &tot);
          if (q < cnt) f_eb[q] = carry + ex;
          carry += tot;
        }
        __syncthreads();
        return carry;
      };
      const int n_chunks = (L + kFrontChunk - 1) / kFrontChunk;
      int carry = 0;
      for (int ch = 0; ch < n_chunks; ++ch) {
        carry = stage(ch, carry);
        const int cnt = min(kFrontChunk, L - ch * kFrontChunk);
        for (int q = wave; q < cnt; q += kEmitWaves) {
          const int st = f_st[0][q], ln = f_ln[0][q], base = f_eb[q];
          for (int p = lane; p < ln; p += 64) claim(idx[st + p], base + p);
        }
        __syncthreads();
      }
      asm volatile("s_waitcnt vmcnt(0)" ::: "memory");
      __syncthreads();
      int appended = 0;
      carry = 0;
      for (int ch = 0; ch < n_chunks; ++ch) {
        carry = stage(ch, carry);
        const int cnt = min(kFrontChunk, L - ch * kFrontChunk);
        for (int q = wave; q < cnt; q += kEmitWaves) {
          const int st = f_st[0][q], ln = f_ln[0][q], base = f_eb[q];
          int wins = 0;
          for (int p0 = 0; p0 < ln; p0 += 64) {
            const int p = p0 + lane;
            wins += __popcll(__ballot(p < ln && owner_of(idx[st + p]) == base + p));
          }
          if (lane == 0) f_wc[q] = wins;
        }
        __syncthreads();
        int chunk_new = 0;
        for (int b0 = 0; b0 < cnt; b0 += kEmitThreads) {
          const int q = b0 + threadIdx.x;
          const int w_ = q < cnt ? f_wc[q] : 0;
          int tot;
          const int ex = wg_excl_scan(w_, lds_scan, &tot);
          if (q < cnt) f_wc[q] = chunk_new + ex;
          chunk_new += tot;
        }
        __syncthreads();
        for (int q = wave; q < cnt; q += kEmitWaves) {
          const int st = f_st[0][q], ln = f_ln[0][q], base = f_eb[q];
          int obase = tail + appended + f_wc[q];
          for (int p0 = 0; p0 < ln; p0 += 64) {
            const int p = p0 + lane;
            int v = 0;
            bool win = false;
            if (p < ln) {
              v = idx[st + p];
              win = owner_of(v) == base + p;
            }
            const uint64_t bal = __ballot(win);
            if (win) {
              const int o = obase + mask_prefix(bal);
              SG_ST(&Q[2 * o], c);
              SG_ST(&Q[2 * o + 1], v);
            }
            obase += __popcll(bal);
          }
        }
        appended += chunk_new;
        __syncthreads();
      }
      asm volatile("s_waitcnt vmcnt(0)" ::: "memory");
      __syncthreads();
      for (int o = tail + threadIdx.x; o < tail + appended; o += kEmitThreads)
        mark_done(SG_LD(&Q[2 * o + 1]));
      const bool keep = own_in_lds && appended <= kFrontChunk;
      if (keep)
        for (int o = threadIdx.x; o < appended; o += kEmitThreads) {
          const int4 rec = node_rec[SG_LD(&Q[2 * (tail + o) + 1])];
          f_st[0][o] = rec.z;
          f_ln[0][o] = rec.w;
        }
      asm volatile("s_waitcnt vmcnt(0)" ::: "memory");
      __syncthreads();
      head = tail;
      tail += appended;
      cur = 0;
      in_lds = keep;
    }
    convert_pending();
    if (stats && threadIdx.x == 0 && c < 256) {
      stats[c * 8 + 0] = size; stats[c * 8 + 1] = n_fast; stats[c * 8 + 2] = n_gen;
      stats[c * 8 + 3] = sum_e; stats[c * 8 + 4] = max_l;
    }
    __syncthreads();
  }
}


constexpr int kBigWgsMax = 256;
constexpr int kBigMin = kOwnCap;
constexpr int kBigNodes = 1024;
constexpr int kBigEdges = 8192;
constexpr int kBigDirectDegree = 32;
static_assert(kBigSlice == kBigEdges && kBigClusterMin == kBigMin && kBfsGiantMin == kBigMin, "staging sizes follow the kernel's constants");
static_assert(kBigNodes <= 65535, "c_j holds node indices of a range as 16-bit");

__device__ __forceinline__ bool big_barrier(int32_t *bar, int &epoch, int32_t *fail, int *lds_flag) {
  asm volatile("s_waitcnt vmcnt(0)" ::: "memory");
  __syncthreads();
  if (threadIdx.x == 0) {
    __hip_atomic_fetch_add(bar, 1, __ATOMIC_RELAXED, __HIP_MEMORY_SCOPE_AGENT);
    const int target = (epoch + 1) * static_cast<int>(gridDim.x);
    unsigned spins = 0;
    int ok = 1;
    while (__hip_atomic_load(bar, __ATOMIC_RELAXED, __HIP_MEMORY_SCOPE_AGENT) < target) {
      __builtin_amdgcn_s_sleep(1);
      if ((++spins & 1023u) == 0u) {
        if (spins > (1u << 24) || __hip_atomic_load(fail, __ATOMIC_RELAXED, __HIP_MEMORY_SCOPE_AGENT)) {
          __hip_atomic_store(fail, 1, __ATOMIC_RELAXED, __HIP_MEMORY_SCOPE_AGENT);
          ok = 0;
          break;
        }
      }
    }
    *lds_flag = ok;
  }
  ++epoch;
  __syncthreads();
  return *lds_flag != 0;
}

__device__ __forceinline__ bool big_flags_barrier(unsigned *flags, unsigned tag, int32_t *fail, int *lds_flag) {
  asm volatile("s_waitcnt vmcnt(0)" ::: "memory");
  __syncthreads();
  const int G = gridDim.x;
  if (threadIdx.x < 64) {
    const int lane = threadIdx.x;
    if (lane == 0) __hip_atomic_store(flags + blockIdx.x, tag, __ATOMIC_RELAXED, __HIP_MEMORY_SCOPE_AGENT);
    int ok = 1;
    for (int w0 = 0; w0 < G && ok; w0 += 64) {
      const int w = w0 + lane;
      unsigned spins = 0;
      while (true) {
        const bool ready = w >= G || __hip_atomic_load(flags + w, __ATOMIC_RELAXED, __HIP_MEMORY_SCOPE_AGENT) >= tag;
        if (__all(ready)) break;
        __builtin_amdgcn_s_sleep(1);
        if ((++spins & 1023u) == 0u &&
            (spins > (1u << 24) || __hip_atomic_load(fail, __ATOMIC_RELAXED, __HIP_MEMORY_SCOPE_AGENT))) {
          __hip_atomic_store(fail, 1, __ATOMIC_RELAXED, __HIP_MEMORY_SCOPE_AGENT);
          ok = 0;
          break;
        }
      }
    }
    if (lane == 0) *lds_flag = ok;
  }
  __syncthreads();
  return *lds_flag != 0;
}

constexpr int kBigRecAt = 64;
constexpr int kBigFlagsAt = kBigRecAt + 8 * kBigWgsMax;
constexpr int kBigSyncWords = kBigFlagsAt + kBigWgsMax;

typedef unsigned long long u64;
__device__ __forceinline__ u64 pack_rec(int z, int w) {
  return static_cast<u64>(static_cast<unsigned>(z)) | (static_cast<u64>(static_cast<unsigned>(w)) << 32);
}

template <bool FAST>
__global__ void __launch_bounds__(kEmitThreads) bfs_emit_big_kernel(
    const int32_t *__restrict__ idx, const int4 *__restrict__ node_rec, const int2 *__restrict__ erec,
    const int32_t *__restrict__ seeds, const int32_t *__restrict__ cluster_offsets, int n_cluster,
    int32_t *owner_g, int32_t *wcnt, int32_t *stage0, int32_t *stage1, u64 *srec0, u64 *srec1, int priv_base,
    int32_t *cluster_idxs, int32_t *sync, bool flag_barrier, bool trace_on, const int32_t *gate) {
  if (gate != nullptr && *gate == 0) return;
  __shared__ int lds_scan[kEmitWaves];
  __shared__ int lds_flag, lds_off;
  __shared__ int node_off[kEmitThreads];
  __shared__ int pre[kBigWgsMax + 1], offs[kBigWgsMax];
  __shared__ int c_st[kBigNodes], c_eb[kBigNodes + 1];
  __shared__ int c_t[kBigEdges];
  __shared__ unsigned short c_j[FAST ? kBigEdges : 1];
  const int wave = threadIdx.x >> 6, lane = threadIdx.x & 63;
  const int G = gridDim.x, b = blockIdx.x;
  int32_t *bar = sync, *fail = sync + 1, *pool = sync + 2;
  unsigned long long *rec = reinterpret_cast<unsigned long long *>(sync + kBigRecAt);
  int epoch = 0;
  unsigned tag = 0;
  unsigned long long ph[6] = {0, 0, 0, 0, 0, 0}, t_prev = 0;
  const bool tracing = trace_on && b == 0 && threadIdx.x == 0;
  auto stamp = [&](int i) {
    if (tracing) {
      const unsigned long long now = __builtin_amdgcn_s_memrealtime();
      ph[i] += now - t_prev;
      t_prev = now;
    }
  };
  for (int c = 0; c < n_cluster; ++c) {
    const int off = cluster_offsets[c];
    const int size = cluster_offsets[c + 1] - off;
    if (size <= kBigMin) continue;
    const int seed = seeds[c];
    int32_t *Q = cluster_idxs + 2LL * off;
    int par = 0;
    ++tag;
    if (threadIdx.x == 0) {
      if (b == 0) {
        SG_ST(&stage0[0], seed);
        if constexpr (FAST) {
          const int4 r = node_rec[seed];
          SG_ST(&srec0[0], pack_rec(r.z, r.w));
        }
        SG_ST(&Q[0], c);
        SG_ST(&Q[1], seed);
        SG_ST(&owner_g[seed], -1);
        SG_ST(&pool[0], 1);
        SG_ST(&pool[1], 0);
      }
      asm volatile("s_waitcnt vmcnt(0)" ::: "memory");
      __hip_atomic_store(&rec[(0 * G + b) * 2], (static_cast<unsigned long long>(tag) << 32), __ATOMIC_RELAXED,
                         __HIP_MEMORY_SCOPE_AGENT);
      __hip_atomic_store(&rec[(0 * G + b) * 2 + 1], (static_cast<unsigned long long>(tag) << 32) | (b == 0 ? 1u : 0u),
                         __ATOMIC_RELAXED, __HIP_MEMORY_SCOPE_AGENT);
    }
    int tail = 0;
    while (true) {
      if (tracing) t_prev = __builtin_amdgcn_s_memrealtime();
      if (wave == 0) {
        int ok = 1;
        for (int w0 = 0; w0 < G; w0 += 64) {
          const int w = w0 + lane;
          unsigned long long a = 0, l = 0;
          unsigned spins = 0;
          while (true) {
            bool ready = true;
            if (w < G) {
              a = __hip_atomic_load(&rec[(par * G + w) * 2], __ATOMIC_RELAXED, __HIP_MEMORY_SCOPE_AGENT);
              l = __hip_atomic_load(&rec[(par * G + w) * 2 + 1], __ATOMIC_RELAXED, __HIP_MEMORY_SCOPE_AGENT);
              ready = (a >> 32) == tag && (l >> 32) == tag;
            }
            if (__all(ready)) break;
            __builtin_amdgcn_s_sleep(1);
            if ((++spins & 1023u) == 0u &&
                (spins > (1u << 24) || __hip_atomic_load(fail, __ATOMIC_RELAXED, __HIP_MEMORY_SCOPE_AGENT))) {
              __hip_atomic_store(fail, 1, __ATOMIC_RELAXED, __HIP_MEMORY_SCOPE_AGENT);
              ok = 0;
              break;
            }
          }
          if (w < G) {
            offs[w] = static_cast<int>(a & 0xffffffffu);
            pre[w + 1] = static_cast<int>(l & 0xffffffffu);
          }
          if (!ok) break;
        }
        if (lane == 0) lds_flag = ok;
      }
      __syncthreads();
      if (!lds_flag) return;
      stamp(0);
      if (threadIdx.x == 0) {
        pre[0] = 0;
        for (int w = 0; w < G; ++w) pre[w + 1] += pre[w];
      }
      __syncthreads();
      const int L = pre[G];
      const int my_pos = pre[b], my_len = pre[b + 1] - pre[b];
      int32_t *cur = par ? stage1 : stage0, *nxt = par ? stage0 : stage1;
      u64 *curr = par ? srec1 : srec0, *nxtr = par ? srec0 : srec1;
      constexpr int kQueueRegs = 4;
      const int q_base = tail + my_pos;
      int qv[kQueueRegs];
#pragma unroll
      for (int k = 0; k < kQueueRegs; ++k) {
        const int i = threadIdx.x + k * kEmitThreads;
        qv[k] = i < my_len ? SG_LD(&cur[offs[b] + i]) : 0;
      }
      for (int i = threadIdx.x + kQueueRegs * kEmitThreads; i < my_len; i += kEmitThreads) {
        SG_ST(&Q[2 * (q_base + i)], c);
        SG_ST(&Q[2 * (q_base + i) + 1], SG_LD(&cur[offs[b] + i]));
      }
      tail += L;
      if (L == 0) {
        if (tracing)
          for (int i = 0; i < 6; ++i) reinterpret_cast<unsigned long long *>(sync + 16)[i] = ph[i];
        break;
      }
      const int lo = static_cast<int>(static_cast<long long>(L) * b / G);
      const int hi = static_cast<int>(static_cast<long long>(L) * (b + 1) / G);
      auto rec_at = [&](int q, int &st, int &ln) {
        int w0 = 0, w1 = G;
        while (w1 - w0 > 1) {
          const int mid = (w0 + w1) >> 1;
          if (pre[mid] <= q) w0 = mid; else w1 = mid;
        }
        const int at = offs[w0] + (q - pre[w0]);
        if constexpr (FAST) {
          const u64 r = SG_LD(&curr[at]);
          st = static_cast<int>(r & 0xffffffffu);
          ln = static_cast<int>(r >> 32);
        } else {
          const int4 r = node_rec[SG_LD(&cur[at])];
          st = r.z;
          ln = r.w;
        }
      };
      const int nn = hi - lo;
      int E = -1;
      if (nn <= kBigNodes) {
        int carry = 0;
        for (int i0 = 0; i0 < nn; i0 += kEmitThreads) {
          const int i = i0 + threadIdx.x;
          int ln = 0;
          if (i < nn) {
            int st;
            rec_at(lo + i, st, ln);
            c_st[i] = st;
          }
          int tot;
          const int ex = wg_excl_scan(ln, lds_scan, &tot);
          if (i < nn) c_eb[i] = carry + ex;
          carry += tot;
        }
        if (threadIdx.x == 0) c_eb[nn] = carry;
        __syncthreads();
        if (carry <= kBigEdges) E = carry;
      }
      auto edge_node = [&](int e) {
        int j0 = 0, j1 = nn;
        while (j1 - j0 > 1) {
          const int mid = (j0 + j1) >> 1;
          if (c_eb[mid] <= e) j0 = mid; else j1 = mid;
        }
        return j0;
      };
      stamp(1);
      if (E >= 0) {
        const bool direct = E <= kBigDirectDegree * nn;
        for (int e = threadIdx.x; e < E; e += kEmitThreads) {
          const int jn = edge_node(e);
          const int p = e - c_eb[jn], g = c_st[jn] + p;
          int t = -1;
          const int ex = erec[g].x, tg = idx[g];
          if ((ex & 0xffff) != 0xffff) {
            t = tg;
            const int pos = ((lo + jn) << 10) | p;
            if (FAST && direct) {
              atomicMin(&owner_g[t], pos);
            } else {
              if (SG_LD(&owner_g[t]) > pos) atomicMin(&owner_g[t], pos);
            }
          }
          c_t[e] = t;
          if constexpr (FAST) c_j[e] = static_cast<unsigned short>(jn);
        }
      } else {
        for (int q = lo + wave; q < hi; q += kEmitWaves) {
          int4 r;
          rec_at(q, r.z, r.w);
          for (int p = lane; p < r.w; p += 64) {
            const int g = r.z + p;
            if ((erec[g].x & 0xffff) == 0xffff) continue;
            const int t = idx[g];
            const int pos = (q << 10) | p;
            if (SG_LD(&owner_g[t]) > pos) atomicMin(&owner_g[t], pos);
          }
        }
      }
      if (b == 0 && threadIdx.x == 0) SG_ST(&pool[par ^ 1], 0);
#pragma unroll
      for (int k = 0; k < kQueueRegs; ++k) {
        const int i = threadIdx.x + k * kEmitThreads;
        if (i < my_len) {
          SG_ST(&Q[2 * (q_base + i)], c);
          SG_ST(&Q[2 * (q_base + i) + 1], qv[k]);
        }
      }
      stamp(2);
      if (flag_barrier) {
        if (!big_flags_barrier(reinterpret_cast<unsigned *>(sync + kBigFlagsAt), tag, fail, &lds_flag)) return;
      } else if (!big_barrier(bar, epoch, fail, &lds_flag)) {
        return;
      }
      stamp(3);
      if (E >= 0) {
        if constexpr (FAST) {
          const int base = priv_base + b * kBigEdges;
          int carry = 0;
          for (int e0 = 0; e0 < E; e0 += kEmitThreads) {
            const int e = e0 + threadIdx.x;
            bool win = false;
            int t = -1;
            int2 er = make_int2(0, 0);
            if (e < E) {
              t = c_t[e];
              if (t >= 0) {
                const int jn = c_j[e];
                const int p = e - c_eb[jn];
                er = erec[c_st[jn] + p];
                win = SG_LD(&owner_g[t]) == (((lo + jn) << 10) | p);
              }
            }
            int tot;
            const int ex = wg_excl_scan(win ? 1 : 0, lds_scan, &tot);
            if (win) {
              SG_ST(&nxt[base + carry + ex], t);
              SG_ST(&nxtr[base + carry + ex], pack_rec(er.y, static_cast<int>(static_cast<unsigned>(er.x) >> 16)));
              SG_ST(&owner_g[t], -1);
            }
            carry += tot;
          }
          asm volatile("s_waitcnt vmcnt(0)" ::: "memory");
          __syncthreads();
          stamp(4);
          if (tracing) ++ph[5];
          ++tag;
          par ^= 1;
          if (threadIdx.x == 0) {
            __hip_atomic_store(&rec[(par * G + b) * 2], (static_cast<unsigned long long>(tag) << 32) | static_cast<unsigned>(base),
                               __ATOMIC_RELAXED, __HIP_MEMORY_SCOPE_AGENT);
            __hip_atomic_store(&rec[(par * G + b) * 2 + 1],
                               (static_cast<unsigned long long>(tag) << 32) | static_cast<unsigned>(carry),
                               __ATOMIC_RELAXED, __HIP_MEMORY_SCOPE_AGENT);
          }
          continue;
        }
        int total = 0;
        for (int e0 = 0; e0 < E; e0 += kEmitThreads) {
          const int e = e0 + threadIdx.x;
          bool win = false;
          if (e < E) {
            const int t = c_t[e];
            if (t >= 0) {
              const int jn = edge_node(e);
              win = SG_LD(&owner_g[t]) == (((lo + jn) << 10) | (e - c_eb[jn]));
            }
            if (!win) c_t[e] = -1;
          }
          total += __popcll(__ballot(win));
        }
        if (lane == 0) lds_scan[wave] = total;
        __syncthreads();
        if (threadIdx.x == 0) {
          int t = 0;
          for (int w = 0; w < kEmitWaves; ++w) t += lds_scan[w];
          lds_off = t > 0 ? __hip_atomic_fetch_add(&pool[par ^ 1], t, __ATOMIC_RELAXED, __HIP_MEMORY_SCOPE_AGENT) : 0;
          lds_scan[0] = t;
        }
        __syncthreads();
        const int region = lds_off, region_len = lds_scan[0];
        __syncthreads();
        int carry = region;
        for (int e0 = 0; e0 < E; e0 += kEmitThreads) {
          const int e = e0 + threadIdx.x;
          const int t = e < E ? c_t[e] : -1;
          int tot;
          const int ex = wg_excl_scan(t >= 0 ? 1 : 0, lds_scan, &tot);
          if (t >= 0) {
            SG_ST(&nxt[carry + ex], t);
            SG_ST(&owner_g[t], -1);
          }
          carry += tot;
        }
        asm volatile("s_waitcnt vmcnt(0)" ::: "memory");
        __syncthreads();
        ++tag;
        par ^= 1;
        if (threadIdx.x == 0) {
          __hip_atomic_store(&rec[(par * G + b) * 2], (static_cast<unsigned long long>(tag) << 32) | static_cast<unsigned>(region),
                             __ATOMIC_RELAXED, __HIP_MEMORY_SCOPE_AGENT);
          __hip_atomic_store(&rec[(par * G + b) * 2 + 1],
                             (static_cast<unsigned long long>(tag) << 32) | static_cast<unsigned>(region_len),
                             __ATOMIC_RELAXED, __HIP_MEMORY_SCOPE_AGENT);
        }
        continue;
      }
      int my_total = 0;
      for (int q = lo + wave; q < hi; q += kEmitWaves) {
        int4 r;
        rec_at(q, r.z, r.w);
        int wins = 0;
        for (int p0 = 0; p0 < r.w; p0 += 64) {
          const int p = p0 + lane;
          bool win = false;
          if (p < r.w) {
            const int g = r.z + p;
            if ((erec[g].x & 0xffff) != 0xffff) win = SG_LD(&owner_g[idx[g]]) == ((q << 10) | p);
          }
          wins += __popcll(__ballot(win));
        }
        if (lane == 0) SG_ST(&wcnt[q], wins);
        my_total += wins;
      }
      if (lane == 0) lds_scan[wave] = my_total;
      asm volatile("s_waitcnt vmcnt(0)" ::: "memory");
      __syncthreads();
      if (threadIdx.x == 0) {
        int t = 0;
        for (int w = 0; w < kEmitWaves; ++w) t += lds_scan[w];
        lds_off = t > 0 ? __hip_atomic_fetch_add(&pool[par ^ 1], t, __ATOMIC_RELAXED, __HIP_MEMORY_SCOPE_AGENT) : 0;
        lds_scan[0] = t;
      }
      __syncthreads();
      const int region = lds_off, region_len = lds_scan[0];
      __syncthreads();
      int carry = region;
      for (int c0 = lo; c0 < hi; c0 += kEmitThreads) {
        const int q_mine = c0 + threadIdx.x;
        const int cnt = q_mine < hi ? SG_LD(&wcnt[q_mine]) : 0;
        int chunk_total;
        const int ex = wg_excl_scan(cnt, lds_scan, &chunk_total);
        node_off[threadIdx.x] = carry + ex;
        __syncthreads();
        const int n_here = min(kEmitThreads, hi - c0);
        for (int jn = wave; jn < n_here; jn += kEmitWaves) {
          const int q = c0 + jn;
          int4 r;
          rec_at(q, r.z, r.w);
          int o = node_off[jn];
          for (int p0 = 0; p0 < r.w; p0 += 64) {
            const int p = p0 + lane;
            bool win = false;
            int t = 0;
            int2 er = make_int2(0, 0);
            if (p < r.w) {
              const int g = r.z + p;
              er = erec[g];
              if ((er.x & 0xffff) != 0xffff) {
                t = idx[g];
                win = SG_LD(&owner_g[t]) == ((q << 10) | p);
              }
            }
            const uint64_t bal = __ballot(win);
            if (win) {
              SG_ST(&nxt[o + mask_prefix(bal)], t);
              if constexpr (FAST)
                SG_ST(&nxtr[o + mask_prefix(bal)], pack_rec(er.y, static_cast<int>(static_cast<unsigned>(er.x) >> 16)));
              SG_ST(&owner_g[t], -1);
            }
            o += __popcll(bal);
          }
        }
        carry += chunk_total;
        __syncthreads();
      }
      asm volatile("s_waitcnt vmcnt(0)" ::: "memory");
      __syncthreads();
      ++tag;
      par ^= 1;
      if (threadIdx.x == 0) {
        __hip_atomic_store(&rec[(par * G + b) * 2], (static_cast<unsigned long long>(tag) << 32) | static_cast<unsigned>(region),
                           __ATOMIC_RELAXED, __HIP_MEMORY_SCOPE_AGENT);
        __hip_atomic_store(&rec[(par * G + b) * 2 + 1],
                           (static_cast<unsigned long long>(tag) << 32) | static_cast<unsigned>(region_len),
                           __ATOMIC_RELAXED, __HIP_MEMORY_SCOPE_AGENT);
      }
    }
    if (!big_barrier(bar, epoch, fail, &lds_flag)) return;
  }
}

constexpr int kLF = 2048;
constexpr int kLE = 8192;
constexpr int kVisWords = 16384;
constexpr int kLevSeg = 2048;
constexpr int kLocalLdsInts = 5 * kLF + 8 + kLE + kLE / 2;
constexpr int kSweepU = 4;

__global__ void __launch_bounds__(kEmitThreads) bfs_emit_big_local_kernel(
    const int32_t *__restrict__ idx, const int4 *__restrict__ node_rec, const int2 *__restrict__ erec,
    const int32_t *__restrict__ seeds, const int32_t *__restrict__ cluster_offsets, int n_cluster,
    int32_t *owner0, int32_t *owner1, int32_t *pool_ids, unsigned long long *pool_rec, unsigned long long *tab,
    int tab_levels, int32_t *cluster_idxs, int32_t *sync, int n, int every, int warm, bool trace_on) {
  typedef unsigned long long u64;
  __shared__ int lds_scan[kEmitWaves];
  __shared__ int lds_flag;
  __shared__ int pre[kBigWgsMax + 1], offs[kBigWgsMax];
  __shared__ int lds_raw[kLocalLdsInts];
  int (*f_st)[kLF] = reinterpret_cast<int (*)[kLF]>(lds_raw);
  unsigned short (*f_ln)[kLF] = reinterpret_cast<unsigned short (*)[kLF]>(lds_raw + 2 * kLF);
  int *f_eb = lds_raw + 3 * kLF;
  int *w_t = f_eb + kLF + 8;
  int *c_t = w_t + kLF;
  unsigned short *c_j = reinterpret_cast<unsigned short *>(c_t + kLE);
  extern __shared__ unsigned vis[];
  const bool use_vis = n <= kVisWords * 32;
  const int vis_words = use_vis ? (n + 31) >> 5 : 0;
  const int wave = threadIdx.x >> 6, lane = threadIdx.x & 63;
  const int G = gridDim.x, b = blockIdx.x;
  int32_t *bar = sync, *fail = sync + 1, *pool_head = sync + 2, *tot = sync + 4;
  int epoch = 0;
  unsigned tagc = 0;
  unsigned long long ph[8] = {0, 0, 0, 0, 0, 0, 0, 0}, t_prev = 0;
  const bool tracing = trace_on && blockIdx.x == 0 && threadIdx.x == 0;
  auto stamp = [&](int i) {
    if (tracing) {
      const unsigned long long now = __builtin_amdgcn_s_memrealtime();
      ph[i] += now - t_prev;
      t_prev = now;
    }
  };
  auto entry = [&](int L, int w) { return tab + (static_cast<size_t>(L) * G + w) * 2; };
  auto publish = [&](int L, unsigned tag, int off, int len) {
    __hip_atomic_store(entry(L, b), (static_cast<u64>(tag) << 32) | static_cast<unsigned>(off), __ATOMIC_RELAXED,
                       __HIP_MEMORY_SCOPE_AGENT);
    __hip_atomic_store(entry(L, b) + 1, (static_cast<u64>(tag) << 32) | static_cast<unsigned>(len), __ATOMIC_RELAXED,
                       __HIP_MEMORY_SCOPE_AGENT);
  };
  auto give_up = [&](int why) {
    if (threadIdx.x == 0) __hip_atomic_store(fail, why, __ATOMIC_RELAXED, __HIP_MEMORY_SCOPE_AGENT);
  };
  for (int c = 0; c < n_cluster; ++c) {
    const int off_c = cluster_offsets[c];
    const int size = cluster_offsets[c + 1] - off_c;
    if (size <= kBigMin) continue;
    const int seed = seeds[c];
    int32_t *Q = cluster_idxs + 2LL * off_c;
    const unsigned tag0 = tagc;
    for (int i = threadIdx.x; i < vis_words; i += kEmitThreads) vis[i] = 0u;
    __syncthreads();
    constexpr int T0 = 1;
    if (threadIdx.x == 0) {
      if (b == 0) {
        const int4 r = node_rec[seed];
        __hip_atomic_store(&pool_rec[0], pack_rec(r.z, r.w), __ATOMIC_RELAXED, __HIP_MEMORY_SCOPE_AGENT);
        SG_ST(&owner0[seed], -1);
        SG_ST(&owner1[seed], -1);
        Q[0] = c;
        Q[1] = seed;
        SG_ST(pool_head, 1);
        SG_ST(&tot[0], 0);
        SG_ST(&tot[1], 0);
        SG_ST(&tot[2], 0);
        SG_ST(&tot[3], 0);
      }
      asm volatile("s_waitcnt vmcnt(0)" ::: "memory");
      publish(0, tag0 + 1, 0, b == 0 ? 1 : 0);
    }
    int cur = 0, nf = 0, L = 0;
    bool pending = false;
    int pend_off = 0;
    bool dead = false;
    while (true) {
      if (L >= tab_levels) { give_up(2); dead = true; break; }
      const unsigned tag = tag0 + static_cast<unsigned>(L) + 1u;
      const bool reb = L < warm || (L % every) == 0;
      const bool next_reb = (L + 1) < warm || ((L + 1) % every) == 0;
      int keybase;
      if (tracing) t_prev = __builtin_amdgcn_s_memrealtime();
      if (reb) {
        if (wave == 0) {
          int ok = 1;
          for (int w0 = 0; w0 < G; w0 += 64) {
            const int w = w0 + lane;
            u64 a = 0, l = 0;
            unsigned spins = 0;
            while (true) {
              bool ready = true;
              if (w < G) {
                a = __hip_atomic_load(entry(L, w), __ATOMIC_RELAXED, __HIP_MEMORY_SCOPE_AGENT);
                l = __hip_atomic_load(entry(L, w) + 1, __ATOMIC_RELAXED, __HIP_MEMORY_SCOPE_AGENT);
                ready = (a >> 32) == tag && (l >> 32) == tag;
              }
              if (__all(ready)) break;
              __builtin_amdgcn_s_sleep(1);
              if ((++spins & 1023u) == 0u &&
                  (spins > (1u << 24) || __hip_atomic_load(fail, __ATOMIC_RELAXED, __HIP_MEMORY_SCOPE_AGENT))) {
                __hip_atomic_store(fail, 1, __ATOMIC_RELAXED, __HIP_MEMORY_SCOPE_AGENT);
                ok = 0;
                break;
              }
            }
            if (w < G) {
              offs[w] = static_cast<int>(a & 0xffffffffu);
              pre[w + 1] = static_cast<int>(l & 0xffffffffu);
            }
            if (!ok) break;
          }
          if (lane == 0) lds_flag = ok;
        }
        __syncthreads();
        if (!lds_flag) return;
        if (threadIdx.x == 0) {
          pre[0] = 0;
          for (int w = 0; w < G; ++w) pre[w + 1] += pre[w];
        }
        __syncthreads();
        const int Ltot = pre[G];
        if (Ltot == 0) break;
        const int lo = static_cast<int>(static_cast<long long>(Ltot) * b / G);
        const int hi = static_cast<int>(static_cast<long long>(Ltot) * (b + 1) / G);
        nf = hi - lo;
        if (nf > kLF) { give_up(3); dead = true; break; }
        for (int i = threadIdx.x; i < nf; i += kEmitThreads) {
          const int q = lo + i;
          int w0 = 0, w1 = G;
          while (w1 - w0 > 1) {
            const int mid = (w0 + w1) >> 1;
            if (pre[mid] <= q) w0 = mid; else w1 = mid;
          }
          const u64 r = __hip_atomic_load(&pool_rec[offs[w0] + (q - pre[w0])], __ATOMIC_RELAXED, __HIP_MEMORY_SCOPE_AGENT);
          f_st[cur][i] = static_cast<int>(r & 0xffffffffu);
          f_ln[cur][i] = static_cast<unsigned short>(r >> 32);
        }
        keybase = lo;
        __syncthreads();
      } else {
        keybase = b << 13;
      }
      stamp(0);
      int E = 0;
      {
        int carry = 0;
        for (int i0 = 0; i0 < nf; i0 += kEmitThreads) {
          const int i = i0 + threadIdx.x;
          const int ln = i < nf ? f_ln[cur][i] : 0;
          int t;
          const int ex = wg_excl_scan(ln, lds_scan, &t);
          if (i < nf) f_eb[i] = carry + ex;
          carry += t;
        }
        if (threadIdx.x == 0) f_eb[nf] = carry;
        __syncthreads();
        E = carry;
      }
      int32_t *own = (L & 1) ? owner1 : owner0;
      auto edge_node = [&](int e) {
        int j0 = 0, j1 = nf;
        while (j1 - j0 > 1) {
          const int mid = (j0 + j1) >> 1;
          if (f_eb[mid] <= e) j0 = mid; else j1 = mid;
        }
        return j0;
      };
      {
        const bool direct = E <= kBigDirectDegree * nf;
        for (int e0 = threadIdx.x; e0 < E; e0 += kSweepU * kEmitThreads) {
          int jn[kSweepU], key[kSweepU], ex[kSweepU], tg[kSweepU], ow[kSweepU];
#pragma unroll
          for (int u = 0; u < kSweepU; ++u) {
            const int e = e0 + u * kEmitThreads;
            jn[u] = 0; key[u] = 0; ex[u] = 0xffff; tg[u] = 0;
            if (e < E) {
              jn[u] = edge_node(e);
              const int p = e - f_eb[jn[u]], g = f_st[cur][jn[u]] + p;
              key[u] = ((keybase + jn[u]) << 10) | p;
              ex[u] = erec[g].x;
              tg[u] = idx[g];
            }
          }
          bool mine_[kSweepU];
#pragma unroll
          for (int u = 0; u < kSweepU; ++u) {
            mine_[u] = (ex[u] & 0xffff) != 0xffff;
            if (use_vis && mine_[u]) mine_[u] = ((vis[tg[u] >> 5] >> (tg[u] & 31)) & 1u) == 0u;
          }
          if (!direct && !use_vis) {
#pragma unroll
            for (int u = 0; u < kSweepU; ++u) ow[u] = mine_[u] ? SG_LD(&own[tg[u]]) : -1;
          }
#pragma unroll
          for (int u = 0; u < kSweepU; ++u) {
            const int e = e0 + u * kEmitThreads;
            const bool mine = mine_[u];
            if (mine && (direct || use_vis || ow[u] > key[u])) atomicMin(&own[tg[u]], key[u]);
            if (e < E && e < kLE) {
              c_t[e] = mine ? tg[u] : -1;
              c_j[e] = static_cast<unsigned short>(jn[u]);
            }
          }
        }
      }
      stamp(1);
      if (pending) {
        if (threadIdx.x == 0) lds_scan[0] = pend_off;
        __syncthreads();
        const int reg = lds_scan[0];
        __syncthreads();
        for (int i = threadIdx.x; i < nf; i += kEmitThreads) {
          SG_ST(&pool_ids[reg + i], w_t[i]);
          __hip_atomic_store(&pool_rec[reg + i], pack_rec(f_st[cur][i], f_ln[cur][i]), __ATOMIC_RELAXED,
                             __HIP_MEMORY_SCOPE_AGENT);
        }
      }
      if (b == 0 && threadIdx.x == 0) SG_ST(&tot[(L + 2) & 3], 0);
      if (trace_on) {
        asm volatile("s_waitcnt vmcnt(0)" ::: "memory");
        stamp(7);
      }
      if (!big_barrier(bar, epoch, fail, &lds_flag)) return;
      if (pending) {
        if (threadIdx.x == 0) publish(L, tag, pend_off, nf);
        pending = false;
      }
      if (!reb) {
        if (threadIdx.x == 0) lds_scan[0] = SG_LD(&tot[L & 3]);
        __syncthreads();
        const int Ltot = lds_scan[0];
        __syncthreads();
        if (Ltot == 0) break;
      }
      stamp(2);
      int cnt = 0;
      {
        const int nxt = cur ^ 1;
        bool over = false;
        for (int e0 = 0; e0 < E; e0 += kSweepU * kEmitThreads) {
          int t[kSweepU], key[kSweepU], ow[kSweepU];
          int2 er[kSweepU];
#pragma unroll
          for (int u = 0; u < kSweepU; ++u) {
            const int e = e0 + u * kEmitThreads + threadIdx.x;
            t[u] = -1; key[u] = 0; ow[u] = -1; er[u] = make_int2(0, 0);
            if (e < E) {
              int jn;
              if (e < kLE) {
                t[u] = c_t[e];
                jn = c_j[e];
              } else {
                jn = edge_node(e);
              }
              const int p = e - f_eb[jn], g = f_st[cur][jn] + p;
              key[u] = ((keybase + jn) << 10) | p;
              if (e >= kLE) {
                er[u] = erec[g];
                t[u] = (er[u].x & 0xffff) != 0xffff ? idx[g] : -1;
              } else if (t[u] >= 0) {
                er[u] = erec[g];
              }
              if (t[u] >= 0) {
                ow[u] = SG_LD(&own[t[u]]);
                if (use_vis) atomicOr(&vis[t[u] >> 5], 1u << (t[u] & 31));
              }
            }
          }
#pragma unroll
          for (int u = 0; u < kSweepU; ++u) {
            if (e0 + u * kEmitThreads >= E) break;
            const bool win = t[u] >= 0 && ow[u] == key[u];
            int tt;
            const int ex = wg_excl_scan(win ? 1 : 0, lds_scan, &tt);
            if (win) {
              const int o = cnt + ex;
              if (o < kLF) {
                f_st[nxt][o] = er[u].y;
                f_ln[nxt][o] = static_cast<unsigned short>(static_cast<unsigned>(er[u].x) >> 16);
                w_t[o] = t[u];
              }
              SG_ST(&owner0[t[u]], -1);
              SG_ST(&owner1[t[u]], -1);
            }
            cnt += tt;
            over = over || cnt > kLF;
          }
        }
        if (over) { give_up(5); dead = true; break; }
      }
      stamp(3);
      if (threadIdx.x == 0) {
        if (cnt > 0) atomicAdd(&tot[(L + 1) & 3], cnt);
        pend_off = cnt > 0 ? __hip_atomic_fetch_add(pool_head, cnt, __ATOMIC_RELAXED, __HIP_MEMORY_SCOPE_AGENT) : 0;
      }
      cur ^= 1;
      nf = cnt;
      ++L;
      pending = true;
      if (next_reb) {
        if (threadIdx.x == 0) lds_scan[0] = pend_off;
        __syncthreads();
        const int reg = lds_scan[0];
        __syncthreads();
        for (int i = threadIdx.x; i < nf; i += kEmitThreads) {
          SG_ST(&pool_ids[reg + i], w_t[i]);
          __hip_atomic_store(&pool_rec[reg + i], pack_rec(f_st[cur][i], f_ln[cur][i]), __ATOMIC_RELAXED,
                             __HIP_MEMORY_SCOPE_AGENT);
        }
        asm volatile("s_waitcnt vmcnt(0)" ::: "memory");
        __syncthreads();
        if (threadIdx.x == 0) publish(L, tag + 1u, reg, nf);
        pending = false;
      }
      stamp(4);
      ph[5] += 1;
      ph[6] += reb ? 1 : 0;
    }
    if (dead) {
      return;
    }
    asm volatile("s_waitcnt vmcnt(0)" ::: "memory");
    if (!big_barrier(bar, epoch, fail, &lds_flag)) return;
    {
      int *lv_dst = c_t;
      int *lv_off = c_t + kLevSeg;
      int *lv_cum = reinterpret_cast<int *>(f_st);
      static_assert(2 * kLevSeg <= kLE && kLevSeg + 1 <= 2 * kLF, "the final copy's tables live in the level caches");
      int base = T0;
      for (int l0 = 1; l0 < L; l0 += kLevSeg) {
        const int nl = min(kLevSeg, L - l0);
        int seg_carry = 0, cum_carry = 0;
        for (int i0 = 0; i0 < nl; i0 += kEmitThreads) {
          const int i = i0 + threadIdx.x;
          int rowtot = 0, mypre = 0, myoff = 0, mylen = 0;
          if (i < nl) {
            for (int w = 0; w < G; ++w) {
              const int len = static_cast<int>(__hip_atomic_load(entry(l0 + i, w) + 1, __ATOMIC_RELAXED, __HIP_MEMORY_SCOPE_AGENT) & 0xffffffffu);
              if (w < b) mypre += len;
              if (w == b) mylen = len;
              rowtot += len;
            }
            myoff = static_cast<int>(__hip_atomic_load(entry(l0 + i, b), __ATOMIC_RELAXED, __HIP_MEMORY_SCOPE_AGENT) & 0xffffffffu);
          }
          int t1, t2;
          const int ex1 = wg_excl_scan(rowtot, lds_scan, &t1);
          const int ex2 = wg_excl_scan(mylen, lds_scan, &t2);
          if (i < nl) {
            lv_dst[i] = base + seg_carry + ex1 + mypre;
            lv_off[i] = myoff;
            lv_cum[i] = cum_carry + ex2;
          }
          seg_carry += t1;
          cum_carry += t2;
        }
        if (threadIdx.x == 0) lv_cum[nl] = cum_carry;
        __syncthreads();
        for (int k = threadIdx.x; k < cum_carry; k += kEmitThreads) {
          int j0 = 0, j1 = nl;
          while (j1 - j0 > 1) {
            const int mid = (j0 + j1) >> 1;
            if (lv_cum[mid] <= k) j0 = mid; else j1 = mid;
          }
          const int r = k - lv_cum[j0];
          const int id = SG_LD(&pool_ids[lv_off[j0] + r]);
          Q[2LL * (lv_dst[j0] + r)] = c;
          Q[2LL * (lv_dst[j0] + r) + 1] = id;
        }
        base += seg_carry;
        __syncthreads();
      }
    }
    tagc = tag0 + static_cast<unsigned>(L) + 2u;
    if (b == 0 && threadIdx.x == 0) {
      sync[8] += L;
      sync[9] += 1;
      if (tracing)
        for (int i = 0; i < 8; ++i) reinterpret_cast<unsigned long long *>(sync + 16)[i] = ph[i];
    }
    asm volatile("s_waitcnt vmcnt(0)" ::: "memory");
    if (!big_barrier(bar, epoch, fail, &lds_flag)) return;
  }
}

struct BfsSide {
  hipStream_t side = nullptr;
  hipEvent_t fork = nullptr, join = nullptr, back = nullptr;
};
static thread_local BfsDefer *t_bfs_defer = nullptr;
static std::mutex g_bfs_mu;
static std::map<std::pair<int, hipStream_t>, BfsSide> g_bfs_side;
static BfsSide *bfs_side(hipStream_t stream) {
  int dev = 0;
  if (hipGetDevice(&dev) != hipSuccess) return nullptr;
  std::lock_guard<std::mutex> g(g_bfs_mu);
  BfsSide &b = g_bfs_side[{dev, stream}];
  if (b.side == nullptr) {
    if (hipStreamCreateWithFlags(&b.side, hipStreamNonBlocking) != hipSuccess ||
        hipEventCreateWithFlags(&b.fork, hipEventDisableTiming) != hipSuccess ||
        hipEventCreateWithFlags(&b.join, hipEventDisableTiming) != hipSuccess ||
        hipEventCreateWithFlags(&b.back, hipEventDisableTiming) != hipSuccess) {
      b = BfsSide();
      return nullptr;
    }
  }
  return &b;
}
void bfs_release_stream(int dev, hipStream_t stream) {
  std::lock_guard<std::mutex> g(g_bfs_mu);
  auto it = g_bfs_side.find({dev, stream});
  if (it == g_bfs_side.end()) return;
  if (it->second.side) {
    hipStreamSynchronize(it->second.side);
    hipStreamDestroy(it->second.side);
    hipEventDestroy(it->second.fork);
    hipEventDestroy(it->second.join);
    hipEventDestroy(it->second.back);
  }
  g_bfs_side.erase(it);
}
struct BfsLabelNote {
  const void *ws = nullptr;
  int max_kept = -1;
};
static thread_local BfsLabelNote t_bfs_note;

void bfs_emit_defer(BfsDefer *d) { t_bfs_defer = d; }
int bfs_emit_join(const BfsDefer &d, hipStream_t stream) {
  if (!d.deferred) return SG_OK;
  BfsSide *side = bfs_side(stream);
  if (side == nullptr || side->side != d.side || hipEventRecord(side->join, side->side) != hipSuccess ||
      hipStreamWaitEvent(stream, side->join, 0) != hipSuccess) {
    set_error("bfs_emit_join: joining the side stream failed");
    return SG_ERR_LAUNCH;
  }
  return SG_OK;
}
int bfs_label_max_kept(const void *ws) { return t_bfs_note.ws == ws ? t_bfs_note.max_kept : -1; }

__global__ void __launch_bounds__(256) bfs_kept_members_kernel(const int32_t *__restrict__ l2p, int n_pts,
                                                              const int4 *__restrict__ label,
                                                              const int32_t *__restrict__ size,
                                                              const float *__restrict__ thr_dev,
                                                              int32_t *__restrict__ out) {
  __shared__ int wsum[4];
  const float thr = thr_dev[0];
  int mine = 0;
  for (int p = blockIdx.x * 256 + threadIdx.x; p < n_pts; p += gridDim.x * 256)
    mine += static_cast<float>(size[label[l2p[p]].x]) >= thr ? 1 : 0;
  const int w = wave_sum(mine);
  if ((threadIdx.x & 63) == 0) wsum[threadIdx.x >> 6] = w;
  __syncthreads();
  if (threadIdx.x == 0) atomicAdd(out, wsum[0] + wsum[1] + wsum[2] + wsum[3]);
}
int bfs_count_kept_members(const void *ws, size_t ws_bytes, int n, int64_t n_edges, const int32_t *l2p, int n_pts,
                           const float *thr_dev, int32_t *out, hipStream_t stream) {
  BfsWs w;
  if (!bfs_carve(const_cast<void *>(ws), ws_bytes, n, n_edges, &w)) {
    set_error("bfs_count_kept_members: workspace too small");
    return SG_ERR_WORKSPACE;
  }
  hipMemsetAsync(out, 0, 4, stream);
  bfs_kept_members_kernel<<<grid_for(n_pts, 256, 1024), 256, 0, stream>>>(l2p, n_pts, w.label, w.size, thr_dev, out);
  return check_launch("bfs_count_kept_members");
}

}

using namespace sg;

extern "C" {

size_t sg_bfs_workspace_bytes(int n, int64_t n_edges) {
  const size_t nn = static_cast<size_t>(n > 0 ? n : 1);
  const size_t ne = static_cast<size_t>(n_edges > 0 ? n_edges : 1);
  const size_t be = big_stage_entries(n);
  return 14 * align_up(nn * 4) + align_up(64 * 4) + align_up(scan_workspace_bytes(n)) +
         align_up(ne * sizeof(int2)) + 2 * (align_up(be * 4) + align_up(be * 8)) + 256;
}

int sg_bfs_cluster_label(const int32_t *bq_idxs, const int32_t *start_len, int n, int64_t n_edges,
                         int list_flags, const int32_t *seg_of_point, const float *seg_thr,
                         int n_seg, int32_t *n_cluster_host, int32_t *sum_npoint_host, void *ws,
                         size_t ws_bytes, sg_stream_t stream_) {
  SG_REQUIRE(n >= 0 && n_seg >= 1 && seg_thr != nullptr, "sg_bfs_cluster_label: bad arguments");
  hipStream_t stream = as_stream(stream_);
  BfsWs w;
  if (!bfs_carve(ws, ws_bytes, n, n_edges, &w)) {
    set_error("sg_bfs_cluster_label: workspace too small");
    return SG_ERR_WORKSPACE;
  }
  *n_cluster_host = 0;
  *sum_npoint_host = 0;
  if (n == 0) return SG_OK;
  const int grid = (n + 255) / 256;
  hipMemsetAsync(w.counters, 0, 64 * 4, stream);
  bfs_init_kernel<<<grid, 256, 0, stream>>>(n, w.parent, w.size, w.owner);
  static const bool one_pass = getenv("SG_BFS_ONE_PASS") != nullptr;
  if (!one_pass) {
    static const bool sample_env = getenv("SG_BFS_SAMPLE") != nullptr;
    if (sample_env || !(list_flags & SG_LISTS_SORTED))
      bfs_union_kernel<1><<<grid_for(n, 4, 256 * 16), 256, 0, stream>>>(bq_idxs, start_len, n,
                                                                      list_flags & SG_LISTS_SORTED,
                                                                      list_flags & SG_LISTS_RADIUS,
                                                                      w.parent, w.asym_nodes, w.counters);
    else
      bfs_hook_min_kernel<<<grid, 256, 0, stream>>>(bq_idxs, start_len, n, list_flags & SG_LISTS_SORTED,
                                                   list_flags & SG_LISTS_RADIUS, w.parent);
    bfs_compress_kernel<<<grid, 256, 0, stream>>>(n, w.parent);
  }
  bfs_union_kernel<0><<<grid_for(n, 4, 256 * 16), 256, 0, stream>>>(bq_idxs, start_len, n,
                                                                  list_flags & SG_LISTS_SORTED,
                                                                  list_flags & SG_LISTS_RADIUS,
                                                                  w.parent, w.asym_nodes, w.counters);
  bfs_flatten_kernel<<<grid, 256, 0, stream>>>(n, w.parent, w.lab);
  bfs_store_root_kernel<<<grid, 256, 0, stream>>>(n, w.lab, w.parent);

  int32_t *host_counters = pinned_words();
  SG_REQUIRE(host_counters != nullptr, "sg_bfs_cluster_label: pinned allocation failed");
  for (int i = 0; i < 5; ++i) host_counters[i] = 0;
  for (int pass = 0; pass < 2; ++pass) {
    if (pass == 1) {
      const int n_asym = host_counters[0];
      while (true) {
        hipMemsetAsync(w.counters + 1, 0, 4, stream);
        bfs_propagate_kernel<<<grid_for(n_asym, 4, 256 * 16), 256, 0, stream>>>(
            bq_idxs, start_len, w.asym_nodes, n_asym, w.parent, w.lab, w.counters);
        host_counters[8] = 0;
        hipMemcpyAsync(host_counters + 8, w.counters + 1, 4, hipMemcpyDeviceToHost, stream);
        if (hipStreamSynchronize(stream) != hipSuccess) return check_launch("bfs propagate");
        if (!host_counters[8]) break;
      }
      bfs_zero_size_kernel<<<grid, 256, 0, stream>>>(n, w.size);
    }
    bfs_label_kernel<<<grid, 256, 0, stream>>>(n, w.parent, w.lab, start_len, w.label, w.size);
    const int4 *label = w.label;
    const int32_t *size = w.size;
    int32_t *cid = w.cid, *coff = w.coff;
    auto keep = [label, size, seg_of_point, seg_thr] __device__(int64_t i) -> int {
      if (label[i].x != static_cast<int32_t>(i)) return 0;
      const float thr = seg_thr[seg_of_point ? seg_of_point[i] : 0];
      return static_cast<float>(size[i]) >= thr ? 1 : 0;
    };
    int32_t *max_kept = w.counters + 4;
    auto keep_size = [keep, size, max_kept] __device__(int64_t i) -> int {
      const int s = keep(i) ? size[i] : 0;
      if (s > kBigMin) atomicMax(max_kept, s);
      return s;
    };
    int rc = exclusive_scan(keep, [cid] __device__(int64_t i, int v) { cid[i] = v; }, n,
                            w.counters + 2, w.scan_ws, w.scan_bytes, stream);
    if (rc != SG_OK) return rc;
    rc = exclusive_scan(keep_size, [coff] __device__(int64_t i, int v) { coff[i] = v; }, n,
                        w.counters + 3, w.scan_ws, w.scan_bytes, stream);
    if (rc != SG_OK) return rc;
    hipMemcpyAsync(host_counters, w.counters, 5 * sizeof(int32_t), hipMemcpyDeviceToHost, stream);
    if (hipStreamSynchronize(stream) != hipSuccess) return check_launch("sg_bfs_cluster_label");
    if (host_counters[0] == 0) break;
    if (pass == 0) hipMemsetAsync(w.counters + 4, 0, 4, stream);
  }
  *n_cluster_host = host_counters[2];
  *sum_npoint_host = host_counters[3];
  t_bfs_note.ws = ws;
  t_bfs_note.max_kept = host_counters[4];
  return check_launch("sg_bfs_cluster_label");
}

int sg_bfs_cluster_emit(const int32_t *bq_idxs, const int32_t *start_len, int n, int64_t n_edges,
                        const int32_t *seg_of_point, const float *seg_thr, int n_cluster,
                        int sum_npoint, int32_t *cluster_idxs, int32_t *cluster_offsets, void *ws,
                        size_t ws_bytes, sg_stream_t stream_) {
  SG_REQUIRE(n >= 0 && n_cluster >= 0 && sum_npoint >= 0, "sg_bfs_cluster_emit: bad arguments");
  hipStream_t stream = as_stream(stream_);
  BfsWs w;
  if (!bfs_carve(ws, ws_bytes, n, n_edges, &w)) {
    set_error("sg_bfs_cluster_emit: workspace too small");
    return SG_ERR_WORKSPACE;
  }
  if (n_cluster == 0 || n == 0) {
    hipMemsetAsync(cluster_offsets, 0, 4, stream);
    return SG_OK;
  }
  bfs_seed_kernel<<<(n + 255) / 256, 256, 0, stream>>>(n, w.label, w.size, w.cid, w.coff,
                                                       seg_of_point, seg_thr, w.seeds,
                                                       cluster_offsets);
  bfs_edge_rec_kernel<<<grid_for(n, 4, 256 * 16), 256, 0, stream>>>(bq_idxs, w.label, w.cid, w.seeds, n,
                                                                     n_cluster, w.erec);
  static const bool want_stats = getenv("SG_BFS_STATS") != nullptr;
  int32_t *stats = nullptr;
  if (want_stats) {
    hipMalloc(&stats, 256 * 8 * 4);
    hipMemsetAsync(stats, 0, 256 * 8 * 4, stream);
  }
  static const bool big_on = !(getenv("SG_BFS_BIG") && atoi(getenv("SG_BFS_BIG")) == 0);
  const bool noted = t_bfs_note.ws == ws && t_bfs_note.max_kept >= 0;
  const bool has_big = big_on && n < (1 << 21) && sum_npoint > kBigMin && (!noted || t_bfs_note.max_kept > kBigMin);
  t_bfs_note.ws = nullptr;
  static const bool side_env = !(getenv("SG_BFS_BIG_SIDE") && atoi(getenv("SG_BFS_BIG_SIDE")) == 0);
  BfsSide *side = has_big && side_env && !want_stats ? bfs_side(stream) : nullptr;
  hipStream_t main_stream = stream;
  BfsDefer *defer = t_bfs_defer;
  t_bfs_defer = nullptr;
  if (defer != nullptr) defer->deferred = false;
  if (side != nullptr) {
    if (hipEventRecord(side->fork, stream) != hipSuccess || hipStreamWaitEvent(side->side, side->fork, 0) != hipSuccess) {
      set_error("sg_bfs_cluster_emit: forking the side stream failed");
      return SG_ERR_LAUNCH;
    }
  }
  bfs_emit_kernel<<<min(n_cluster, 4096), kEmitThreads, 0, stream>>>(
      bq_idxs, start_len, w.label, w.erec, w.seeds, cluster_offsets, n_cluster, w.owner, cluster_idxs,
      stats, big_on && n < (1 << 21) ? kBigMin : 0x7fffffff, -1, nullptr, thin_levels_on());
  if (side != nullptr) stream = side->side;
  if (has_big) {
    static const int big_wgs_env = getenv("SG_BFS_BIG_WGS") ? atoi(getenv("SG_BFS_BIG_WGS")) : 16;
    const int big_wgs = big_wgs_env < 8 ? 8 : big_wgs_env > kBigWgsMax ? kBigWgsMax : big_wgs_env;
    int32_t *sync = w.asym_nodes;
    static const bool flags_on = getenv("SG_BFS_BIG_FLAGS") && atoi(getenv("SG_BFS_BIG_FLAGS")) != 0;
    if (static_cast<size_t>(n) >= static_cast<size_t>(kBigSyncWords)) {
      hipMemsetAsync(sync, 0, kBigSyncWords * 4, stream);
      if (const char *e = getenv("SG_BFS_FORCE_FALLBACK"))
        if (atoi(e) & 1) hipMemsetAsync(sync + 1, 1, 1, stream);
      const int32_t *gate = nullptr;
      if (big_local_on() && big_fast_on() && w.big_stage[0] != nullptr &&
          static_cast<size_t>(n) >= static_cast<size_t>(kBigSyncWords) + 96) {
        const int lw_env = getenv("SG_BFS_BIG_LOCAL_WGS") ? atoi(getenv("SG_BFS_BIG_LOCAL_WGS")) : 16;
        const int lw = lw_env < 8 ? 8 : lw_env > kBigWgsMax ? kBigWgsMax : lw_env;
        const int every_env = getenv("SG_BFS_BIG_LOCAL_EVERY") ? atoi(getenv("SG_BFS_BIG_LOCAL_EVERY")) : 4;
        const int warm_env = getenv("SG_BFS_BIG_LOCAL_WARM") ? atoi(getenv("SG_BFS_BIG_LOCAL_WARM")) : 8;
        const int every = every_env < 1 ? 1 : every_env, warm = warm_env < 1 ? 1 : warm_env;
        const bool novis = getenv("SG_BFS_BIG_LOCAL_NOVIS") && atoi(getenv("SG_BFS_BIG_LOCAL_NOVIS")) != 0;
        int32_t *sync3 = sync + kBigSyncWords;
        const size_t rows = big_stage_entries(n) / (2 * static_cast<size_t>(lw));
        hipMemsetAsync(sync3, 0, 96 * 4, stream);
        hipMemsetAsync(w.big_rec[1], 0, rows * 2 * lw * 8, stream);
        hipMemsetD32Async(reinterpret_cast<hipDeviceptr_t>(w.parent), 0x7fffffff, n, stream);
        if (const char *e = getenv("SG_BFS_FORCE_FALLBACK"))
          if (atoi(e) & 2) hipMemsetAsync(sync3 + 1, 1, 1, stream);
        const size_t vis_bytes = (!novis && n <= kVisWords * 32) ? static_cast<size_t>((n + 31) >> 5) * 4 : 0;
        {
          static std::mutex mu;
          static uint64_t done_mask = 0;
          int dev = 0;
          hipGetDevice(&dev);
          std::lock_guard<std::mutex> g(mu);
          if (dev < 0 || dev >= 64 || !((done_mask >> dev) & 1)) {
            if (hipFuncSetAttribute(reinterpret_cast<const void *>(bfs_emit_big_local_kernel),
                                    hipFuncAttributeMaxDynamicSharedMemorySize, kVisWords * 4) != hipSuccess) {
              (void)hipGetLastError();
              set_error("sg_bfs_cluster_emit: %d bytes of dynamic LDS are not available on this device", kVisWords * 4);
              return SG_ERR_LAUNCH;
            }
            if (dev >= 0 && dev < 64) done_mask |= 1ull << dev;
          }
        }
        bfs_emit_big_local_kernel<<<lw, kEmitThreads, vis_bytes, stream>>>(
            bq_idxs, w.label, w.erec, w.seeds, cluster_offsets, n_cluster, w.owner, w.parent, w.big_stage[0],
            w.big_rec[0], w.big_rec[1], static_cast<int>(rows) - 1, cluster_idxs, sync3, novis ? 0x7fffffff : n, every, warm,
            want_stats);
        gate = sync3 + 1;
        bfs_owner_reset_kernel<<<grid_for(n, 256, 1024), 256, 0, stream>>>(n, w.label, w.size, kBigMin, gate, w.owner);
      }
      if (big_fast_on() && big_wgs <= kBigFastWgs && w.big_stage[0] != nullptr)
        bfs_emit_big_kernel<true><<<big_wgs, kEmitThreads, 0, stream>>>(
            bq_idxs, w.label, w.erec, w.seeds, cluster_offsets, n_cluster, w.owner, w.wcnt, w.big_stage[0],
            w.big_stage[1], w.big_rec[0], w.big_rec[1], n, cluster_idxs, sync, flags_on, want_stats, gate);
      else
        bfs_emit_big_kernel<false><<<big_wgs, kEmitThreads, 0, stream>>>(
            bq_idxs, w.label, w.erec, w.seeds, cluster_offsets, n_cluster, w.owner, w.wcnt, w.parent, w.lab,
            nullptr, nullptr, 0, cluster_idxs, sync, false, false, gate);
      bfs_owner_reset_kernel<<<grid_for(n, 256, 1024), 256, 0, stream>>>(n, w.label, w.size, kBigMin,
                                                                        sync + 1, w.owner);
      bfs_emit_kernel<<<min(n_cluster, 256), kEmitThreads, 0, stream>>>(
          bq_idxs, start_len, w.label, w.erec, w.seeds, cluster_offsets, n_cluster, w.owner,
          cluster_idxs, nullptr, 0x7fffffff, kBigMin, sync + 1, thin_levels_on());
    }
  }
  if (side != nullptr && defer != nullptr) {
    stream = main_stream;
    if (hipEventRecord(side->back, stream) != hipSuccess || hipStreamWaitEvent(side->side, side->back, 0) != hipSuccess) {
      set_error("sg_bfs_cluster_emit: handing the side stream over failed");
      return SG_ERR_LAUNCH;
    }
    defer->deferred = true;
    defer->side = side->side;
  } else if (side != nullptr) {
    stream = main_stream;
    if (hipEventRecord(side->join, side->side) != hipSuccess || hipStreamWaitEvent(stream, side->join, 0) != hipSuccess) {
      set_error("sg_bfs_cluster_emit: joining the side stream failed");
      return SG_ERR_LAUNCH;
    }
  }
  if (want_stats && has_big && big_local_on()) {
    hipStreamSynchronize(stream);
    int32_t h[32];
    hipMemcpy(h, w.asym_nodes + kBigSyncWords, sizeof(h), hipMemcpyDeviceToHost);
    unsigned long long lp[8];
    hipMemcpy(lp, w.asym_nodes + kBigSyncWords + 16, sizeof(lp), hipMemcpyDeviceToHost);
    const double lv = lp[5] ? static_cast<double>(lp[5]) : 1.0;
    fprintf(stderr, "bfs giant clusters, local form: %s (%d); %d clusters, %d levels (%llu re-partition levels); us per level: "
            "re-partition %.2f, edge bases+claim sweep %.2f, pool+drain %.2f, rendezvous %.2f, emit sweep %.2f, totals+publication %.2f\n",
            h[1] ? "gave up" : "completed", h[1], h[9], h[8], lp[6], lp[0] / lv / 100.0, lp[1] / lv / 100.0, lp[7] / lv / 100.0,
            lp[2] / lv / 100.0, lp[3] / lv / 100.0, lp[4] / lv / 100.0);
  }
  if (want_stats && has_big) {
    unsigned long long ph[6];
    hipStreamSynchronize(stream);
    hipMemcpy(ph, w.asym_nodes + 16, sizeof(ph), hipMemcpyDeviceToHost);
    const double lv = ph[5] ? static_cast<double>(ph[5]) : 1.0;
    fprintf(stderr, "bfs giant clusters: %llu cached levels; us per level: wait records %.2f, ranks+queue+staged records %.2f, "
            "claim sweep %.2f, claim rendezvous %.2f, emit sweep+drain %.2f\n", ph[5], ph[0] / lv / 100.0, ph[1] / lv / 100.0,
            ph[2] / lv / 100.0, ph[3] / lv / 100.0, ph[4] / lv / 100.0);
  }
  if (want_stats) {
    int32_t h[256 * 8];
    hipMemcpy(h, stats, sizeof(h), hipMemcpyDeviceToHost);
    hipFree(stats);
    for (int c = 0; c < n_cluster && c < 256; ++c)
      fprintf(stderr, "bfs cluster %d: size %d fast levels %d generic levels %d edges %d max frontier %d\n", c,
              h[c * 8], h[c * 8 + 1], h[c * 8 + 2], h[c * 8 + 3], h[c * 8 + 4]);
  }
  return check_launch("sg_bfs_cluster_emit");
}

}
```

### softgroup_amd/csrc/common.h

```cpp
#pragma once
#include <hip/hip_runtime.h>
#include <stdint.h>
#include <stdio.h>

#include "../../include/softgroup_hip.h"

namespace sg {

constexpr int kWave = 64;

void set_error(const char *fmt, ...);
int32_t *pinned_words();

inline hipStream_t as_stream(sg_stream_t s) { return reinterpret_cast<hipStream_t>(s); }

inline int check_launch(const char *what) {
  hipError_t e = hipGetLastError();
  if (e != hipSuccess) {
    set_error("%s: %s", what, hipGetErrorString(e));
    return SG_ERR_LAUNCH;
  }
  return SG_OK;
}

#define SG_REQUIRE(cond, ...)      \
  do {                             \
    if (!(cond)) {                 \
      sg::set_error(__VA_ARGS__);  \
      return SG_ERR_ARG;           \
    }                              \
  } while (0)

inline size_t align_up(size_t x, size_t a = 256) { return (x + a - 1) / a * a; }

struct Workspace {
  char *base;
  size_t size, off;
  Workspace(void *p, size_t n) : base(static_cast<char *>(p)), size(n), off(0) {}
  template <typename T>
  T *take(size_t count) {
    size_t bytes = align_up(count * sizeof(T));
    if (off + bytes > size) return nullptr;
    T *r = reinterpret_cast<T *>(base + off);
    off += bytes;
    return r;
  }
};

inline int grid_for(int64_t work_items, int block, int max_blocks = 256 * 8) {
  int64_t g = (work_items + block - 1) / block;
  if (g < 1) g = 1;
  if (g > max_blocks) g = max_blocks;
  return static_cast<int>(g);
}

__device__ __forceinline__ int lane_id() { return threadIdx.x & 63; }

__device__ __forceinline__ uint64_t mix64(uint64_t x) {
  x ^= x >> 33;
  x *= 0xff51afd7ed558ccdULL;
  x ^= x >> 33;
  x *= 0xc4ceb9fe1a85ec53ULL;
  return x ^ (x >> 33);
}

__device__ __forceinline__ int mask_prefix(uint64_t m) {
  return __builtin_amdgcn_mbcnt_hi(static_cast<uint32_t>(m >> 32),
                                   __builtin_amdgcn_mbcnt_lo(static_cast<uint32_t>(m), 0u));
}

template <int CTRL, int ROW_MASK = 0xf, int BANK_MASK = 0xf>
__device__ __forceinline__ int dpp_or_zero(int v) {
  return __builtin_amdgcn_update_dpp(0, v, CTRL, ROW_MASK, BANK_MASK, false);
}
__device__ __forceinline__ int wave_incl_scan(int v) {
  v += dpp_or_zero<0x111>(v);
  v += dpp_or_zero<0x112>(v);
  v += dpp_or_zero<0x114>(v);
  v += dpp_or_zero<0x118>(v);
  v += dpp_or_zero<0x142, 0xa>(v);
  v += dpp_or_zero<0x143, 0xc>(v);
  return v;
}
__device__ __forceinline__ int wave_sum(int v) {
  return __builtin_amdgcn_readlane(wave_incl_scan(v), 63);
}
__device__ __forceinline__ int wave_max(int v) {
#pragma unroll
  for (int o = 32; o > 0; o >>= 1) v = max(v, __shfl_xor(v, o, 64));
  return v;
}

constexpr int kFillMax = 16;
struct FillList {
  uint32_t *p[kFillMax];
  size_t words[kFillMax];
  uint32_t pattern[kFillMax];
  int n = 0;
  void add(void *ptr, size_t bytes, int byte) {
    if (bytes == 0 || ptr == nullptr || n >= kFillMax) return;
    p[n] = static_cast<uint32_t *>(ptr);
    words[n] = bytes / 4;
    pattern[n] = 0x01010101u * static_cast<uint32_t>(byte & 0xff);
    ++n;
  }
};
static __global__ void __launch_bounds__(256) fill_many_kernel(FillList f) {
  const int r = blockIdx.y;
  uint32_t *p = f.p[r];
  const size_t w = f.words[r];
  const uint32_t v = f.pattern[r];
  const size_t head = (16 - (reinterpret_cast<uintptr_t>(p) & 15)) / 4 % 4;
  const size_t h = head < w ? head : w;
  const size_t quads = (w - h) / 4;
  uint4 *q = reinterpret_cast<uint4 *>(p + h);
  const uint4 vv = make_uint4(v, v, v, v);
  for (size_t i = blockIdx.x * 256ull + threadIdx.x; i < quads; i += gridDim.x * 256ull) q[i] = vv;
  if (blockIdx.x == 0) {
    if (threadIdx.x < h) p[threadIdx.x] = v;
    const size_t t0 = h + quads * 4;
    if (threadIdx.x < w - t0) p[t0 + threadIdx.x] = v;
  }
}
inline void fill_many(const FillList &f, hipStream_t stream) {
  if (f.n == 0) return;
  size_t mx = 0;
  for (int i = 0; i < f.n; ++i) mx = f.words[i] > mx ? f.words[i] : mx;
  const int gx = grid_for(static_cast<int64_t>(mx / 4 + 1), 256, 1024);
  fill_many_kernel<<<dim3(gx, f.n), 256, 0, stream>>>(f);
}

extern thread_local int t_conv_arith;
void conv_chain_begin(hipStream_t stream);
bool conv_chain_recording();
int conv_chain_end();
void conv_chain_abort();
int conv_chain_concat(const float *a, const float *b, int64_t rows, int ca, int cb, const float *scale,
                      const float *shift, float *out, float *out_act);
int conv_chain_bn_relu(const float *x, const float *scale, const float *shift, int64_t rows, int c, float *out);
int conv_chain_check_abort(const char *who);
int conv_gather_rows(const void *in, int num_in_rows, const int32_t *nbr, int M_out, int K, int Cin, int Cout,
                     const float *w_k8, const float *post_scale, const float *post_shift, const void *residual,
                     const float *act_scale, const float *act_shift, void *out_act, const int32_t *order,
                     const uint32_t *tile_mask, const int32_t *nbr_tiles, void *out, void *ws, size_t ws_bytes,
                     sg_stream_t stream, int in16, int out16, int res16);
int spconv_wgrad_layout(const void *in, int in_bf16, const void *g_out, int g_bf16, const int32_t *nbr_t, int M_out,
                        int K, int Cin, int Cout, float *dw, int out_oki, void *ws, size_t ws_bytes,
                        sg_stream_t stream);
struct PackJob {
  const float *w;
  float *out;
  int cout, kvol, cin, mode;
};
int spconv_pack_weights(const PackJob *jobs, int n, sg_stream_t stream);
size_t octree_stash_bytes(int n);
int octree_ballquery_count_stash(const float *points, const float *boxes, const int32_t *pt_inds,
                                 const int32_t *pt_start_len, int n, float radius, int32_t *start_len, int32_t *stash,
                                 hipStream_t stream);
int octree_ballquery_fill_stash(const float *points, const float *boxes, const int32_t *pt_inds,
                                const int32_t *pt_start_len, int n, float radius, const int32_t *start_len,
                                const int32_t *stash, int32_t *idx, hipStream_t stream);
void conv_release_stream(int dev, hipStream_t stream);
void unet_release_stream(int dev, hipStream_t stream);
void scan_release_stream(int dev, hipStream_t stream);
void bfs_release_stream(int dev, hipStream_t stream);
constexpr int kBfsGiantMin = 16384;
struct BfsDefer {
  bool deferred = false;
  hipStream_t side = nullptr;
};
void bfs_emit_defer(BfsDefer *d);
int bfs_emit_join(const BfsDefer &d, hipStream_t stream);
int bfs_label_max_kept(const void *ws);
int bfs_count_kept_members(const void *ws, size_t ws_bytes, int n, int64_t n_edges, const int32_t *l2p, int n_pts,
                           const float *thr_dev, int32_t *out, hipStream_t stream);

}
```

Before: 420.5.

## Use sub-wave lane groups for ball query and BFS grouping kernels

Adds templated lane-group primitives (scan, ballot, prefix) and lets ball-query counting process two points per wave with 32-lane groups. BFS union, propagate and edge-record kernels pick 8-lane groups when neighbor lists are short on average. The ball-query fill pass gains a separate compact copy kernel for short lists plus a worklist of long ones, and the hash probe reads a stored cell key and a packed start/count range instead of indirecting through the representative. This aims to stop idle lanes when neighbor lists are much shorter than 64, at the cost of extra workspace, an atomic worklist, and more kernel variants.

```diff
diff --git a/include/softgroup_hip.h b/include/softgroup_hip.h
--- a/include/softgroup_hip.h
+++ b/include/softgroup_hip.h
@@ -175,6 +175,8 @@
 int sg_spconv_set_arithmetic(int mode);
 
 int sg_spconv_set_combine(int mode);
+
+int sg_grouping_set_lanes(int lanes);
 
 int sg_spconv_set_chain(int mode);
 int sg_spconv_chain_stats(int64_t *launches, int64_t *steps);
diff --git a/softgroup_amd/_lib.py b/softgroup_amd/_lib.py
--- a/softgroup_amd/_lib.py
+++ b/softgroup_amd/_lib.py
@@ -66,6 +66,7 @@
     'sg_spconv_set_arithmetic': (_i, [_i]),
     'sg_spconv_set_combine': (_i, [_i]),
     'sg_spconv_set_chain': (_i, [_i]),
+    'sg_grouping_set_lanes': (_i, [_i]),
     'sg_spconv_chain_stats': (_i, [_vp, _vp]),
     'sg_spconv_profile': (_i, [_i]),
     'sg_spconv_profile_read': (_i, [_vp, _vp]),
diff --git a/softgroup_amd/csrc/ballquery.hip b/softgroup_amd/csrc/ballquery.hip
--- a/softgroup_amd/csrc/ballquery.hip
+++ b/softgroup_amd/csrc/ballquery.hip
@@ -7,6 +7,12 @@
 constexpr int kBqBuf = 2048;
 constexpr int kBqCap = SG_BALLQUERY_MAX_NEIGHBORS;
 constexpr int kBqKeep = 64;
+constexpr int kBqWideWalk = 192;
+constexpr int kBqDenseMean = 24;
+__device__ __forceinline__ bool bq_dense_lists(const int32_t *__restrict__ start_len, int n) {
+  const int64_t total = static_cast<int64_t>(start_len[2 * static_cast<int64_t>(n) - 2]) + start_len[2 * static_cast<int64_t>(n) - 1];
+  return total > static_cast<int64_t>(kBqDenseMean) * n;
+}
 
 struct BqWs {
   int4 *cell;
@@ -17,6 +23,10 @@
   int32_t *slot_of;
   float4 *sorted;
   int32_t *keep;
+  int4 *key;
+  int2 *range;
+  int32_t *work;
+  int32_t *work_n;
   void *scan_ws;
   size_t scan_bytes;
   uint32_t cap;
@@ -32,7 +42,7 @@
                                                        const int32_t *__restrict__ batch_idxs,
                                                        int n, double inv_cell, int4 *__restrict__ cell,
                                                        int32_t *table, uint32_t mask, int32_t *count,
-                                                       int32_t *__restrict__ slot_of) {
+                                                       int32_t *__restrict__ slot_of, int4 *__restrict__ key) {
   const int i = blockIdx.x * 256 + threadIdx.x;
   if (i >= n) return;
   int4 c;
@@ -46,7 +56,10 @@
     int32_t cur = __hip_atomic_load(&table[s], __ATOMIC_RELAXED, __HIP_MEMORY_SCOPE_AGENT);
     if (cur == kBqEmpty) {
       cur = atomicCAS(&table[s], kBqEmpty, i);
-      if (cur == kBqEmpty) break;
+      if (cur == kBqEmpty) {
+        key[s] = c;
+        break;
+      }
     }
     int4 o;
     o.x = batch_idxs ? batch_idxs[cur] : 0;
@@ -79,24 +92,29 @@
 struct BqCells {
   int start, excl, incl, total;
 };
+template <int G>
 __device__ __forceinline__ BqCells bq_cells(int my_start, int my_count) {
   BqCells c;
   c.start = my_start;
-  c.incl = wave_incl_scan(my_count);
+  c.incl = group_incl_scan<G>(my_count);
   c.excl = c.incl - my_count;
-  c.total = __shfl(c.incl, 63, 64);
+  c.total = __shfl(c.incl, lane_id() | (G - 1), 64);
   return c;
 }
-__device__ __forceinline__ int bq_candidate(const BqCells &c, int t) {
+__device__ __forceinline__ int bq_candidate_from(const BqCells &c, int base, int t) {
   int lo = 0, hi = 26;
 #pragma unroll
   for (int it = 0; it < 5; ++it) {
     const int mid = (lo + hi) >> 1;
-    const bool right = __shfl(c.incl, mid, 64) <= t;
+    const bool right = __shfl(c.incl, base + mid, 64) <= t;
     lo = right ? mid + 1 : lo;
     hi = right ? hi : mid;
   }
-  return __shfl(c.start, lo, 64) + (t - __shfl(c.excl, lo, 64));
+  return __shfl(c.start, base + lo, 64) + (t - __shfl(c.excl, base + lo, 64));
+}
+template <int G>
+__device__ __forceinline__ int bq_candidate(const BqCells &c, int t) {
+  return bq_candidate_from(c, lane_id() & ~(G - 1), t);
 }
 
 __device__ __forceinline__ int bq_scan_count(const float4 *__restrict__ sorted, const BqCells &c,
@@ -104,7 +122,7 @@
   int total = 0;
   for (int t0 = 0; t0 < c.total; t0 += 64) {
     const int t = t0 + lane_id();
-    const int at = bq_candidate(c, min(t, c.total - 1));
+    const int at = bq_candidate<64>(c, min(t, c.total - 1));
     if (t < c.total) {
       const float4 p = sorted[at];
       total += (dist2(ox, oy, oz, p.x, p.y, p.z) < r2 && __float_as_int(p.w) < limit) ? 1 : 0;
@@ -113,20 +131,65 @@
   return wave_sum(total);
 }
 
-template <bool FILL>
+__global__ void __launch_bounds__(256) bq_copy_kernel(int n, const int32_t *__restrict__ start_len,
+                                                     const int32_t *__restrict__ keep,
+                                                     int32_t *__restrict__ idx_out, int32_t *__restrict__ work,
+                                                     int32_t *work_n) {
+  const int lane = threadIdx.x & 63, gl = lane & 7, sub = lane >> 3;
+  if (bq_dense_lists(start_len, n)) return;
+  for (int i0 = ((blockIdx.x * 256 + threadIdx.x) >> 6) * 64; i0 < n; i0 += gridDim.x * 256) {
+    const int mine = i0 + lane;
+    int2 sl = make_int2(0, 0);
+    if (mine < n) sl = *reinterpret_cast<const int2 *>(start_len + 2 * static_cast<int64_t>(mine));
+    const bool append = sl.y > kBqKeep;
+    const uint64_t bal = __ballot(append);
+    if (bal) {
+      const int leader = __ffsll(static_cast<long long>(bal)) - 1;
+      int base = 0;
+      if (lane == leader) base = atomicAdd(work_n, __popcll(bal));
+      base = __shfl(base, leader, 64);
+      const int pos = base + mask_prefix(bal);
+      if (append && pos < n) work[pos] = mine;
+    }
+    const int short_len = append ? 0 : sl.y;
+    int st[8], ln[8], v[8];
+#pragma unroll
+    for (int it = 0; it < 8; ++it) {
+      st[it] = __shfl(sl.x, it * 8 + sub, 64);
+      ln[it] = __shfl(short_len, it * 8 + sub, 64);
+      v[it] = gl < ln[it] ? keep[static_cast<int64_t>(i0 + it * 8 + sub) * kBqKeep + gl] : 0;
+    }
+#pragma unroll
+    for (int it = 0; it < 8; ++it)
+      if (gl < ln[it]) idx_out[static_cast<int64_t>(st[it]) + gl] = v[it];
+#pragma unroll
+    for (int it = 0; it < 8; ++it)
+      for (int p = gl + 8; p < ln[it]; p += 8)
+        idx_out[static_cast<int64_t>(st[it]) + p] = keep[static_cast<int64_t>(i0 + it * 8 + sub) * kBqKeep + p];
+  }
+}
+
+template <bool FILL, int G>
 __global__ void __launch_bounds__(256) bq_query_kernel(const float *__restrict__ xyz, int n,
                                                       float r2, const int4 *__restrict__ cell,
                                                       const int32_t *__restrict__ table,
-                                                      const int32_t *__restrict__ count,
-                                                      const int32_t *__restrict__ start,
+                                                      const int4 *__restrict__ key,
+                                                      const int2 *__restrict__ range,
                                                       uint32_t mask, const float4 *__restrict__ sorted,
                                                       int32_t *__restrict__ start_len,
-                                                      int32_t *__restrict__ idx_out, int32_t *__restrict__ keep) {
-  __shared__ __attribute__((aligned(16))) int32_t buf_all[FILL ? 4 * kBqBuf : 4 * kBqKeep];
-  const int wave = threadIdx.x >> 6, lane = threadIdx.x & 63;
-  int32_t *buf = buf_all + wave * (FILL ? kBqBuf : kBqKeep);
-  for (int i = blockIdx.x * 4 + wave; i < n; i += gridDim.x * 4) {
-    if (FILL) {
+                                                      int32_t *__restrict__ idx_out, int32_t *__restrict__ keep,
+                                                      const int32_t *__restrict__ work, const int32_t *work_n) {
+  static_assert(G == 64 || (!FILL && G == 32), "two points per wave: count pass only");
+  constexpr int kPts = 64 / G;
+  __shared__ __attribute__((aligned(16))) int32_t buf_all[FILL ? 4 * kBqBuf : 4 * kPts * kBqKeep];
+  const int wave = threadIdx.x >> 6, lane = group_lane<G>(), sub = (threadIdx.x & 63) / G;
+  int32_t *buf = buf_all + (FILL ? wave * kBqBuf : (wave * kPts + sub) * kBqKeep);
+  const bool listed = FILL && work != nullptr && !bq_dense_lists(start_len, n);
+  const int n_items = listed ? min(*work_n, n) : n;
+  for (int i0 = (blockIdx.x * 4 + wave) * kPts; i0 < n_items; i0 += gridDim.x * 4 * kPts) {
+    const bool live = G == 64 || i0 + sub < n;
+    const int i = listed ? work[i0] : (live ? i0 + sub : n - 1);
+    if (FILL && !listed) {
       const int out_len = start_len[2 * i + 1];
       if (out_len <= kBqKeep) {
         if (lane < out_len) idx_out[static_cast<int64_t>(start_len[2 * i]) + lane] = keep[static_cast<int64_t>(i) * kBqKeep + lane];
@@ -136,27 +199,60 @@
     const float ox = xyz[3 * i], oy = xyz[3 * i + 1], oz = xyz[3 * i + 2];
     const int4 c = cell[i];
     int my_start = 0, my_count = 0;
-    if (lane < 27) {
+    if (lane < 27 && live) {
       const int cx = c.y + lane / 9 - 1, cy = c.z + (lane / 3) % 3 - 1, cz = c.w + lane % 3 - 1;
       uint32_t s = cell_slot(c.x, cx, cy, cz, mask);
       while (true) {
         const int32_t rep = table[s];
+        const int4 o = key[s];
+        const int2 sc = range[s];
         if (rep == kBqEmpty) break;
-        const int4 o = cell[rep];
         if (o.x == c.x && o.y == cx && o.z == cy && o.w == cz) {
-          my_start = start[s];
-          my_count = count[s];
+          my_start = sc.x;
+          my_count = sc.y;
           break;
         }
         s = (s + 1) & mask;
       }
     }
-    const BqCells cells = bq_cells(my_start, my_count);
+    const BqCells cells = bq_cells<G>(my_start, my_count);
     if (!FILL) {
+      int total_max = cells.total;
+#pragma unroll
+      for (int o = 32; o >= G; o >>= 1) total_max = max(total_max, __shfl_xor(total_max, o, 64));
       int m = 0;
-      for (int t0 = 0; t0 < cells.total; t0 += 64) {
+      if (G == 32 && total_max > kBqWideWalk) {
+        int mh[2];
+#pragma unroll
+        for (int h = 0; h < 2; ++h) {
+          const int src = h * 32, lane64 = threadIdx.x & 63;
+          const float hx = __shfl(ox, src, 64), hy = __shfl(oy, src, 64), hz = __shfl(oz, src, 64);
+          const int htotal = __builtin_amdgcn_readlane(cells.total, src);
+          int32_t *hbuf = buf_all + (wave * kPts + h) * kBqKeep;
+          int mm = 0;
+          for (int t0 = 0; t0 < htotal; t0 += 64) {
+            const int t = t0 + lane64;
+            const int at = bq_candidate_from(cells, src, min(t, htotal - 1));
+            bool ok = false;
+            int id = 0;
+            if (t < htotal) {
+              const float4 p = sorted[at];
+              id = __float_as_int(p.w);
+              ok = dist2(hx, hy, hz, p.x, p.y, p.z) < r2;
+            }
+            const uint64_t bal = __ballot(ok);
+            const int pos = mm + mask_prefix(bal);
+            if (ok && pos < kBqKeep) hbuf[pos] = id;
+            mm += __popcll(bal);
+          }
+          mh[h] = mm;
+        }
+        m = sub ? mh[1] : mh[0];
+        total_max = 0;
+      }
+      for (int t0 = 0; t0 < total_max; t0 += G) {
         const int t = t0 + lane;
-        const int at = bq_candidate(cells, min(t, cells.total - 1));
+        const int at = bq_candidate<G>(cells, min(t, cells.total - 1));
         bool ok = false;
         int id = 0;
         if (t < cells.total) {
@@ -164,19 +260,21 @@
           id = __float_as_int(p.w);
           ok = dist2(ox, oy, oz, p.x, p.y, p.z) < r2;
         }
-        const uint64_t bal = __ballot(ok);
-        const int pos = m + mask_prefix(bal);
+        const uint64_t bal = group_ballot<G>(ok);
+        const int pos = m + group_mask_prefix<G>(bal);
         if (ok && pos < kBqKeep) buf[pos] = id;
         m += __popcll(bal);
       }
-      if (lane == 0) start_len[2 * i + 1] = min(m, kBqCap);
-      if (m <= kBqKeep) {
-        __builtin_amdgcn_fence(__ATOMIC_RELEASE, "wavefront");
-        __builtin_amdgcn_wave_barrier();
-        const int e = lane < m ? buf[lane] : 0x7fffffff;
+      if (lane == 0 && live) start_len[2 * i + 1] = min(m, kBqCap);
+      __builtin_amdgcn_fence(__ATOMIC_RELEASE, "wavefront");
+      __builtin_amdgcn_wave_barrier();
+      const int ms = m <= kBqKeep && live ? m : 0;
+      for (int e0 = 0; e0 < ms; e0 += G) {
+        const int ei = e0 + lane;
+        const int e = ei < ms ? buf[ei] : 0x7fffffff;
         int rank = 0;
-        for (int j = 0; j < m; ++j) rank += (buf[j] < e);
-        if (lane < m) keep[static_cast<int64_t>(i) * kBqKeep + rank] = e;
+        for (int j = 0; j < ms; ++j) rank += (buf[j] < e);
+        if (ei < ms) keep[static_cast<int64_t>(i) * kBqKeep + rank] = e;
       }
       __builtin_amdgcn_wave_barrier();
       continue;
@@ -188,7 +286,7 @@
       m = 0;
       for (int t0 = 0; t0 < cells.total; t0 += 64) {
         const int t = t0 + lane;
-        const int at = bq_candidate(cells, min(t, cells.total - 1));
+        const int at = bq_candidate<64>(cells, min(t, cells.total - 1));
         bool ok = false;
         int id = 0;
         if (t < cells.total) {
@@ -248,7 +346,12 @@
   w->scan_bytes = scan_workspace_bytes(w->cap);
   w->scan_ws = a.take<char>(w->scan_bytes);
   w->keep = a.take<int32_t>(nn * kBqKeep);
-  return w->scan_ws != nullptr && w->keep != nullptr;
+  w->key = a.take<int4>(w->cap);
+  w->range = a.take<int2>(w->cap);
+  w->work = a.take<int32_t>(nn);
+  w->work_n = a.take<int32_t>(64);
+  return w->scan_ws != nullptr && w->keep != nullptr && w->key != nullptr && w->range != nullptr &&
+         w->work != nullptr && w->work_n != nullptr;
 }
 
 }
@@ -261,7 +364,8 @@
   const size_t nn = static_cast<size_t>(n > 0 ? n : 1);
   const size_t cap = bq_cap(n);
   return 2 * align_up(nn * 16) + 4 * align_up(cap * 4) + align_up(nn * 4) +
-         align_up(scan_workspace_bytes(cap)) + align_up(nn * kBqKeep * 4) + 256;
+         align_up(scan_workspace_bytes(cap)) + align_up(nn * kBqKeep * 4) + align_up(cap * 16) +
+         align_up(cap * 8) + align_up(nn * 4) + align_up(64 * 4) + 256;
 }
 
 int sg_ballquery_build_grid(const float *xyz, const int32_t *batch_idxs, int n, float radius,
@@ -279,16 +383,21 @@
     f.add(w.table, static_cast<size_t>(w.cap) * 4, 0x7f);
     f.add(w.count, static_cast<size_t>(w.cap) * 4, 0);
     f.add(w.cursor, static_cast<size_t>(w.cap) * 4, 0);
+    f.add(w.work_n, 64 * 4, 0);
     fill_many(f, stream);
   }
   const double inv_cell = 1.0 / (static_cast<double>(radius) * (1.0 + 1e-6));
   const int grid = (n + 255) / 256;
   bq_insert_kernel<<<grid, 256, 0, stream>>>(xyz, batch_idxs, n, inv_cell, w.cell, w.table,
-                                             w.cap - 1, w.count, w.slot_of);
+                                             w.cap - 1, w.count, w.slot_of, w.key);
   const int32_t *count = w.count;
   int32_t *start = w.start;
   auto in = [count] __device__(int64_t s) { return count[s]; };
-  auto out = [start] __device__(int64_t s, int v) { start[s] = v; };
+  int2 *range = w.range;
+  auto out = [start, count, range] __device__(int64_t s, int v) {
+    start[s] = v;
+    range[s] = make_int2(v, count[s]);
+  };
   int rc = exclusive_scan(in, out, w.cap, nullptr, w.scan_ws, w.scan_bytes, stream);
   if (rc != SG_OK) return rc;
   bq_scatter_kernel<<<grid, 256, 0, stream>>>(xyz, n, w.slot_of, w.start, w.cursor, w.sorted);
@@ -308,8 +417,12 @@
   }
   if (n == 0) return SG_OK;
   const float r2 = radius * radius;
-  bq_query_kernel<false><<<grid_for(n, 4, 256 * 16), 256, 0, as_stream(stream_)>>>(
-      xyz, n, r2, w.cell, w.table, w.count, w.start, w.cap - 1, w.sorted, start_len, nullptr, w.keep);
+  if (grouping_lanes_forced() == 64)
+    bq_query_kernel<false, 64><<<grid_for(n, 4, 256 * 16), 256, 0, as_stream(stream_)>>>(
+        xyz, n, r2, w.cell, w.table, w.key, w.range, w.cap - 1, w.sorted, start_len, nullptr, w.keep, nullptr, nullptr);
+  else
+    bq_query_kernel<false, 32><<<grid_for((static_cast<int64_t>(n) + 1) / 2, 4, 256 * 16), 256, 0, as_stream(stream_)>>>(
+        xyz, n, r2, w.cell, w.table, w.key, w.range, w.cap - 1, w.sorted, start_len, nullptr, w.keep, nullptr, nullptr);
   return check_launch("sg_ballquery_count");
 }
 
@@ -325,9 +438,18 @@
   }
   if (n == 0) return SG_OK;
   const float r2 = radius * radius;
-  bq_query_kernel<true><<<grid_for(n, 4, 256 * 16), 256, 0, as_stream(stream_)>>>(
-      xyz, n, r2, w.cell, w.table, w.count, w.start, w.cap - 1, w.sorted,
-      const_cast<int32_t *>(start_len), idx, w.keep);
+  hipStream_t stream = as_stream(stream_);
+  if (grouping_lanes_forced() == 64) {
+    bq_query_kernel<true, 64><<<grid_for(n, 4, 256 * 16), 256, 0, stream>>>(
+        xyz, n, r2, w.cell, w.table, w.key, w.range, w.cap - 1, w.sorted, const_cast<int32_t *>(start_len), idx,
+        w.keep, nullptr, nullptr);
+  } else {
+    bq_copy_kernel<<<grid_for((static_cast<int64_t>(n) + 63) / 64, 4, 256 * 16), 256, 0, stream>>>(
+        n, start_len, w.keep, idx, w.work, w.work_n);
+    bq_query_kernel<true, 64><<<grid_for(n, 4, 256 * 16), 256, 0, stream>>>(
+        xyz, n, r2, w.cell, w.table, w.key, w.range, w.cap - 1, w.sorted, const_cast<int32_t *>(start_len), idx,
+        w.keep, w.work, w.work_n);
+  }
   return check_launch("sg_ballquery_fill");
 }
 
diff --git a/softgroup_amd/csrc/bfs.hip b/softgroup_amd/csrc/bfs.hip
--- a/softgroup_amd/csrc/bfs.hip
+++ b/softgroup_amd/csrc/bfs.hip
@@ -1,5 +1,6 @@
 #include <stdlib.h>
 
+#include <atomic>
 #include <map>
 #include <mutex>
 #include <utility>
@@ -118,20 +119,23 @@
 }
 
 constexpr int kSample = 2;
-template <int SAMPLE>
+template <int SAMPLE, int G>
 __global__ void __launch_bounds__(256) bfs_union_kernel(const int32_t *__restrict__ idx,
                                                        const int32_t *__restrict__ start_len, int n,
                                                        int lists_sorted, int radius_lists,
                                                        int32_t *parent, int32_t *asym_nodes,
                                                        int32_t *counters) {
-  const int wave = threadIdx.x >> 6, lane = threadIdx.x & 63;
-  for (int u = blockIdx.x * 4 + wave; u < n; u += gridDim.x * 4) {
-    const int st = start_len[2 * u], ln_all = start_len[2 * u + 1];
+  constexpr int kNodes = 64 / G;
+  const int wave = threadIdx.x >> 6, lane = group_lane<G>(), sub = (threadIdx.x & 63) / G;
+  for (int u0 = (blockIdx.x * 4 + wave) * kNodes; u0 < n; u0 += gridDim.x * 4 * kNodes) {
+    const int u = u0 + sub;
+    const bool live = G == 64 || u < n;
+    const int st = live ? start_len[2 * u] : 0, ln_all = live ? start_len[2 * u + 1] : 0;
     const int ln = SAMPLE ? min(ln_all, kSample) : ln_all;
     const bool u_capped = ln_all >= kCap;
     bool any_asym = false;
-    const int ru = SAMPLE ? -1 : SG_LD(&parent[u]);
-    for (int p0 = 0; p0 < ln; p0 += 64) {
+    const int ru = SAMPLE || !live ? -1 : SG_LD(&parent[u]);
+    for (int p0 = 0; p0 < ln; p0 += G) {
       const int p = p0 + lane;
       const int v = p < ln ? idx[st + p] : u;
       bool sym = true;
@@ -152,7 +156,7 @@
       }
       any_asym |= !sym;
     }
-    if (!SAMPLE && __any(any_asym)) {
+    if (!SAMPLE && group_any<G>(any_asym)) {
       if (lane == 0) asym_nodes[atomicAdd(&counters[0], 1)] = u;
     }
   }
@@ -193,18 +197,19 @@
   if (i < n) parent[i] = lab[i];
 }
 
+template <int G>
 __global__ void __launch_bounds__(256) bfs_propagate_kernel(const int32_t *__restrict__ idx,
                                                            const int32_t *__restrict__ start_len,
                                                            const int32_t *__restrict__ asym_nodes,
                                                            int n_asym,
                                                            const int32_t *__restrict__ root_of,
                                                            int32_t *lab, int32_t *counters) {
-  const int wave = threadIdx.x >> 6, lane = threadIdx.x & 63;
-  for (int a = blockIdx.x * 4 + wave; a < n_asym; a += gridDim.x * 4) {
+  const int lane = group_lane<G>();
+  for (int a = (blockIdx.x * 256 + threadIdx.x) / G; a < n_asym; a += (gridDim.x * 256) / G) {
     const int u = asym_nodes[a];
     const int ru = root_of[u];
     const int st = start_len[2 * u], ln = start_len[2 * u + 1];
-    for (int p = lane; p < ln; p += 64) {
+    for (int p = lane; p < ln; p += G) {
       const int rv = root_of[idx[st + p]];
       if (rv == ru) continue;
       const int lu = SG_LD(&lab[ru]);
@@ -222,19 +227,24 @@
   const int i = blockIdx.x * 256 + threadIdx.x;
   const bool valid = i < n;
   const int l = valid ? lab[root_of[i]] : -1;
-  int slot = 0;
+  int rank = 0, peers = 0, my_leader = threadIdx.x & 63;
   uint64_t todo = __ballot(valid);
   const int lane = threadIdx.x & 63;
   while (todo) {
     const int leader = __ffsll(static_cast<long long>(todo)) - 1;
     const int ll = __shfl(l, leader, 64);
     const uint64_t same = __ballot(valid && l == ll) & todo;
-    int base = 0;
-    if (lane == leader) base = atomicAdd(&size[ll], __popcll(same));
-    base = __shfl(base, leader, 64);
-    if ((same >> lane) & 1ull) slot = base + __popcll(same & ((1ull << lane) - 1ull));
+    if ((same >> lane) & 1ull) {
+      my_leader = leader;
+      peers = __popcll(same);
+      rank = __popcll(same & ((1ull << lane) - 1ull));
+    }
     todo &= ~same;
   }
+  int base = 0;
+  if (valid && lane == my_leader) base = atomicAdd(&size[l], peers);
+  base = __shfl(base, my_leader, 64);
+  const int slot = base + rank;
   if (!valid) return;
   node_rec[i] = make_int4(l, slot, start_len[2 * i], start_len[2 * i + 1]);
 }
@@ -271,18 +281,19 @@
   }
 }
 
+template <int G>
 __global__ void __launch_bounds__(256) bfs_edge_rec_kernel(const int32_t *__restrict__ idx,
                                                           const int4 *__restrict__ node_rec,
                                                           const int32_t *__restrict__ cid,
                                                           const int32_t *__restrict__ seeds,
                                                           int n, int n_cluster,
                                                           int2 *__restrict__ erec) {
-  const int lane = threadIdx.x & 63;
-  for (int v = (blockIdx.x * 256 + threadIdx.x) >> 6; v < n; v += (gridDim.x * 256) >> 6) {
+  const int lane = group_lane<G>();
+  for (int v = (blockIdx.x * 256 + threadIdx.x) / G; v < n; v += (gridDim.x * 256) / G) {
     const int4 rv = node_rec[v];
     const int c = cid[rv.x];
     if (c >= n_cluster || seeds[c] != rv.x) continue;
-    for (int p = lane; p < rv.w; p += 64) {
+    for (int p = lane; p < rv.w; p += G) {
       const int4 rt = node_rec[idx[rv.z + p]];
       erec[rv.z + p] = rt.x == rv.x ? make_int2(min(rt.y, 0xfffe) | (rt.w << 16), rt.z)
                                     : make_int2(0xffff, 0);
@@ -1625,11 +1636,71 @@
   return check_launch("bfs_count_kept_members");
 }
 
+static std::atomic<int> g_group_lanes{-1};
+static bool lanes_value_ok(int v) { return v == 0 || v == 8 || v == 16 || v == 32 || v == 64; }
+int grouping_lanes_forced() {
+  int v = g_group_lanes.load(std::memory_order_relaxed);
+  if (v >= 0) return v;
+  const char *e = getenv("SG_GROUP_LANES");
+  const int from_env = e && lanes_value_ok(atoi(e)) ? atoi(e) : 0;
+  int expected = -1;
+  g_group_lanes.compare_exchange_strong(expected, from_env, std::memory_order_relaxed);
+  return g_group_lanes.load(std::memory_order_relaxed);
+}
+constexpr int kNarrowMean = 16;
+constexpr int kNarrowMeanUnion = 5;
+static int lanes_auto(int64_t n_edges, int n, int narrow_mean) {
+  const int f = grouping_lanes_forced();
+  if (f) return f;
+  return n > 0 && n_edges <= static_cast<int64_t>(narrow_mean) * n ? 8 : 64;
+}
+int grouping_lanes_for(int64_t n_edges, int n) { return lanes_auto(n_edges, n, kNarrowMean); }
+static int lanes_grid(int n, int G) { return grid_for((static_cast<int64_t>(n) * G + 63) / 64, 4, 256 * 16); }
+
+template <int SAMPLE>
+static void launch_union(int G, hipStream_t stream, const int32_t *idx, const int32_t *start_len, int n, int sorted,
+                         int radius, int32_t *parent, int32_t *asym_nodes, int32_t *counters) {
+  const int grid = lanes_grid(n, G);
+  switch (G) {
+    case 8: bfs_union_kernel<SAMPLE, 8><<<grid, 256, 0, stream>>>(idx, start_len, n, sorted, radius, parent, asym_nodes, counters); break;
+    case 16: bfs_union_kernel<SAMPLE, 16><<<grid, 256, 0, stream>>>(idx, start_len, n, sorted, radius, parent, asym_nodes, counters); break;
+    case 32: bfs_union_kernel<SAMPLE, 32><<<grid, 256, 0, stream>>>(idx, start_len, n, sorted, radius, parent, asym_nodes, counters); break;
+    default: bfs_union_kernel<SAMPLE, 64><<<grid, 256, 0, stream>>>(idx, start_len, n, sorted, radius, parent, asym_nodes, counters); break;
+  }
+}
+static void launch_propagate(int G, hipStream_t stream, const int32_t *idx, const int32_t *start_len,
+                             const int32_t *asym_nodes, int n_asym, const int32_t *root_of, int32_t *lab,
+                             int32_t *counters) {
+  const int grid = lanes_grid(n_asym, G);
+  switch (G) {
+    case 8: bfs_propagate_kernel<8><<<grid, 256, 0, stream>>>(idx, start_len, asym_nodes, n_asym, root_of, lab, counters); break;
+    case 16: bfs_propagate_kernel<16><<<grid, 256, 0, stream>>>(idx, start_len, asym_nodes, n_asym, root_of, lab, counters); break;
+    case 32: bfs_propagate_kernel<32><<<grid, 256, 0, stream>>>(idx, start_len, asym_nodes, n_asym, root_of, lab, counters); break;
+    default: bfs_propagate_kernel<64><<<grid, 256, 0, stream>>>(idx, start_len, asym_nodes, n_asym, root_of, lab, counters); break;
+  }
+}
+static void launch_edge_rec(int G, hipStream_t stream, const int32_t *idx, const int4 *node_rec, const int32_t *cid,
+                            const int32_t *seeds, int n, int n_cluster, int2 *erec) {
+  const int grid = lanes_grid(n, G);
+  switch (G) {
+    case 8: bfs_edge_rec_kernel<8><<<grid, 256, 0, stream>>>(idx, node_rec, cid, seeds, n, n_cluster, erec); break;
+    case 16: bfs_edge_rec_kernel<16><<<grid, 256, 0, stream>>>(idx, node_rec, cid, seeds, n, n_cluster, erec); break;
+    case 32: bfs_edge_rec_kernel<32><<<grid, 256, 0, stream>>>(idx, node_rec, cid, seeds, n, n_cluster, erec); break;
+    default: bfs_edge_rec_kernel<64><<<grid, 256, 0, stream>>>(idx, node_rec, cid, seeds, n, n_cluster, erec); break;
+  }
+}
+
 }
 
 using namespace sg;
 
 extern "C" {
+
+int sg_grouping_set_lanes(int lanes) {
+  SG_REQUIRE(lanes_value_ok(lanes), "sg_grouping_set_lanes: lanes must be 0, 8, 16, 32 or 64");
+  grouping_lanes_forced();
+  return g_group_lanes.exchange(lanes, std::memory_order_relaxed);
+}
 
 size_t sg_bfs_workspace_bytes(int n, int64_t n_edges) {
   const size_t nn = static_cast<size_t>(n > 0 ? n : 1);
@@ -1654,25 +1725,23 @@
   *sum_npoint_host = 0;
   if (n == 0) return SG_OK;
   const int grid = (n + 255) / 256;
+  const int lanes_union = lanes_auto(n_edges, n, kNarrowMeanUnion);
+  const int lanes = lanes_auto(n_edges, n, kNarrowMean);
   hipMemsetAsync(w.counters, 0, 64 * 4, stream);
   bfs_init_kernel<<<grid, 256, 0, stream>>>(n, w.parent, w.size, w.owner);
   static const bool one_pass = getenv("SG_BFS_ONE_PASS") != nullptr;
   if (!one_pass) {
     static const bool sample_env = getenv("SG_BFS_SAMPLE") != nullptr;
     if (sample_env || !(list_flags & SG_LISTS_SORTED))
-      bfs_union_kernel<1><<<grid_for(n, 4, 256 * 16), 256, 0, stream>>>(bq_idxs, start_len, n,
-                                                                      list_flags & SG_LISTS_SORTED,
-                                                                      list_flags & SG_LISTS_RADIUS,
-                                                                      w.parent, w.asym_nodes, w.counters);
+      launch_union<1>(lanes_union, stream, bq_idxs, start_len, n, list_flags & SG_LISTS_SORTED,
+                      list_flags & SG_LISTS_RADIUS, w.parent, w.asym_nodes, w.counters);
     else
       bfs_hook_min_kernel<<<grid, 256, 0, stream>>>(bq_idxs, start_len, n, list_flags & SG_LISTS_SORTED,
                                                    list_flags & SG_LISTS_RADIUS, w.parent);
     bfs_compress_kernel<<<grid, 256, 0, stream>>>(n, w.parent);
   }
-  bfs_union_kernel<0><<<grid_for(n, 4, 256 * 16), 256, 0, stream>>>(bq_idxs, start_len, n,
-                                                                  list_flags & SG_LISTS_SORTED,
-                                                                  list_flags & SG_LISTS_RADIUS,
-                                                                  w.parent, w.asym_nodes, w.counters);
+  launch_union<0>(lanes_union, stream, bq_idxs, start_len, n, list_flags & SG_LISTS_SORTED,
+                  list_flags & SG_LISTS_RADIUS, w.parent, w.asym_nodes, w.counters);
   bfs_flatten_kernel<<<grid, 256, 0, stream>>>(n, w.parent, w.lab);
   bfs_store_root_kernel<<<grid, 256, 0, stream>>>(n, w.lab, w.parent);
 
@@ -1684,8 +1753,7 @@
       const int n_asym = host_counters[0];
       while (true) {
         hipMemsetAsync(w.counters + 1, 0, 4, stream);
-        bfs_propagate_kernel<<<grid_for(n_asym, 4, 256 * 16), 256, 0, stream>>>(
-            bq_idxs, start_len, w.asym_nodes, n_asym, w.parent, w.lab, w.counters);
+        launch_propagate(lanes, stream, bq_idxs, start_len, w.asym_nodes, n_asym, w.parent, w.lab, w.counters);
         host_counters[8] = 0;
         hipMemcpyAsync(host_counters + 8, w.counters + 1, 4, hipMemcpyDeviceToHost, stream);
         if (hipStreamSynchronize(stream) != hipSuccess) return check_launch("bfs propagate");
@@ -1744,8 +1812,7 @@
   bfs_seed_kernel<<<(n + 255) / 256, 256, 0, stream>>>(n, w.label, w.size, w.cid, w.coff,
                                                        seg_of_point, seg_thr, w.seeds,
                                                        cluster_offsets);
-  bfs_edge_rec_kernel<<<grid_for(n, 4, 256 * 16), 256, 0, stream>>>(bq_idxs, w.label, w.cid, w.seeds, n,
-                                                                     n_cluster, w.erec);
+  launch_edge_rec(grouping_lanes_for(n_edges, n), stream, bq_idxs, w.label, w.cid, w.seeds, n, n_cluster, w.erec);
   static const bool want_stats = getenv("SG_BFS_STATS") != nullptr;
   int32_t *stats = nullptr;
   if (want_stats) {
diff --git a/softgroup_amd/csrc/common.h b/softgroup_amd/csrc/common.h
--- a/softgroup_amd/csrc/common.h
+++ b/softgroup_amd/csrc/common.h
@@ -90,6 +90,47 @@
   for (int o = 32; o > 0; o >>= 1) v = max(v, __shfl_xor(v, o, 64));
   return v;
 }
+
+template <int G>
+__device__ __forceinline__ int group_lane() { return static_cast<int>(threadIdx.x) & (G - 1); }
+template <int G>
+__device__ __forceinline__ uint64_t group_mask() { return G == 64 ? ~0ull : ((1ull << (G & 63)) - 1ull); }
+template <int G>
+__device__ __forceinline__ uint64_t group_ballot(bool p) {
+  const uint64_t b = __ballot(p);
+  if (G == 64) return b;
+  return (b >> (lane_id() & ~(G - 1))) & group_mask<G>();
+}
+template <int G>
+__device__ __forceinline__ bool group_any(bool p) { return group_ballot<G>(p) != 0ull; }
+template <int G>
+__device__ __forceinline__ int group_mask_prefix(uint64_t m) {
+  if (G == 64) return mask_prefix(m);
+  return __popcll(m & ((1ull << group_lane<G>()) - 1ull));
+}
+template <int G>
+__device__ __forceinline__ int group_incl_scan(int v) {
+  static_assert(G == 8 || G == 16 || G == 32 || G == 64, "lane groups are 8, 16, 32 or 64 lanes");
+  if (G == 8) {
+    const int gl = group_lane<8>();
+    int t = dpp_or_zero<0x111>(v);
+    v += gl >= 1 ? t : 0;
+    t = dpp_or_zero<0x112>(v);
+    v += gl >= 2 ? t : 0;
+    t = dpp_or_zero<0x114>(v);
+    v += gl >= 4 ? t : 0;
+    return v;
+  }
+  v += dpp_or_zero<0x111>(v);
+  v += dpp_or_zero<0x112>(v);
+  v += dpp_or_zero<0x114>(v);
+  v += dpp_or_zero<0x118>(v);
+  if (G >= 32) v += dpp_or_zero<0x142, 0xa>(v);
+  if (G == 64) v += dpp_or_zero<0x143, 0xc>(v);
+  return v;
+}
+int grouping_lanes_for(int64_t n_edges, int n);
+int grouping_lanes_forced();
 
 constexpr int kFillMax = 16;
 struct FillList {
```

Result: faster. 434.9, median of 6 (+3.4%).
